# Geo3DSmart/PDANet

Hardware: AMD Instinct MI355X
Metric: scenes/sec (16384-pt ONCE, PDA-SSD forward+backward) (higher is better)
Workload: dtype f32; 1 GPU; once16k_b2_detector_fwd_bwd_adam; scenes_per_gpu=2, global_batch=2, parallelism=dp1, world_size_seen=1, cpu_affinity=GPU-local NUMA node of 0000:a7:00.0: 128 CPUs, full=False, graph_tail=False, graph_head=True

## Files before the change

include/pda_train.h:

```cpp
#ifndef PDA_TRAIN_H
#define PDA_TRAIN_H
#include "pda_pointnet2.h"

#ifdef __cplusplus
extern "C" {
#endif

int pda_grad_norm(const float *g, int64_t n, float *norm_out, float *scratch1024, pda_stream_t stream);
int pda_adam_onecycle_step(float *p, const float *g, float *m, float *v, int64_t n, float lr,
                           float beta1, float beta2, float eps, float wd, int step,
                           const float *total_norm, float max_norm, pda_stream_t stream);

int64_t pda_bn_relu_scratch_bytes(int c);
int pda_bn_relu_fwd(const float *x, const float *gamma, const float *beta, float *running_mean,
                    float *running_var, float *y, float *mean_invstd, void *scratch, int64_t rows, int c,
                    float eps, float momentum, pda_stream_t stream);
int pda_bn_relu_bwd(const float *x, const float *grad_y, const float *gamma, const float *beta,
                    const float *mean_invstd, float *grad_x, float *grad_gamma, float *grad_beta,
                    void *scratch, int64_t rows, int c, pda_stream_t stream);
int pda_bn_relu_fwd_mixed(const void *x, int x_is_bf16, const float *gamma, const float *beta, float *running_mean,
                          float *running_var, void *y, int y_is_bf16, float *mean_invstd, void *scratch,
                          int64_t rows, int c, float eps, float momentum, pda_stream_t stream);
int pda_bn_relu_bwd_mixed(const void *x, int x_is_bf16, const void *grad_y, int grad_y_is_bf16, const float *gamma,
                          const float *beta, const float *mean_invstd, void *grad_x, float *grad_gamma,
                          float *grad_beta, void *scratch, int64_t rows, int c, pda_stream_t stream);
int pda_bn_relu_max_pool_fwd(const void *x, int x_is_bf16, const float *gamma, const float *beta, float *running_mean,
                             float *running_var, float *out, uint8_t *arg, float *mean_invstd, void *scratch,
                             int64_t groups, int ns, int c, float eps, float momentum, pda_stream_t stream);
int pda_bn_relu_max_pool_bwd(const void *x, int x_is_bf16, const float *grad_out, const uint8_t *arg,
                             const float *gamma, const float *beta, const float *mean_invstd, void *grad_x,
                             float *grad_gamma, float *grad_beta, void *scratch, int64_t groups, int ns, int c,
                             pda_stream_t stream);

int64_t pda_layer_norm_scratch_bytes(int d);
int pda_layer_norm_fwd(const float *x, const float *residual, const float *gamma, const float *beta,
                       float *sum_out, float *y, float *mean_rstd, int64_t rows, int d, float eps,
                       pda_stream_t stream);
int pda_layer_norm_bwd(const float *x, const float *grad_y, const float *grad_y2, const float *gamma,
                       const float *mean_rstd, float *grad_x, float *grad_gamma, float *grad_beta,
                       void *scratch, int64_t rows, int d, pda_stream_t stream);
int pda_layer_norm_fwd_mixed(const void *x, int x_is_bf16, const float *residual, const float *gamma,
                             const float *beta, float *sum_out, float *y, uint16_t *y_bf16, float *mean_rstd,
                             int64_t rows, int d, float eps, pda_stream_t stream);
int pda_layer_norm_bwd_mixed(const float *x, const float *grad_y, const void *grad_y2, int grad_y2_is_bf16,
                             const float *gamma, const float *mean_rstd, float *grad_x, uint16_t *grad_x_bf16,
                             float *grad_gamma, float *grad_beta, void *scratch, int64_t rows, int d,
                             pda_stream_t stream);

int64_t pda_linear_wgrad_scratch_bytes(int64_t tokens, int in_features, int out_features);
int pda_linear_wgrad_form(int64_t tokens, int in_features, int out_features);
int pda_linear_wgrad(const float *x, const float *grad_out, float *grad_weight, float *grad_bias,
                     void *scratch, int64_t tokens, int in_features, int out_features, pda_stream_t stream);
int pda_linear_wgrad_bn(const float *x, const float *grad_out, float *grad_weight, float *grad_bias, void *scratch,
                        int64_t tokens, int in_features, int out_features, const float *x_mean_invstd,
                        const float *x_gamma, const float *x_beta, pda_stream_t stream);

int64_t pda_gemm_split_bn_tiles(int64_t tokens);
int pda_gemm_split_bn(const float *x, const void *wf, float *y, int64_t tokens, int k, int n_out,
                      const float *in_mean_invstd, const float *in_gamma, const float *in_beta, int stats_mode,
                      double *partial, pda_stream_t stream);
int pda_gemm_split_maxpool(const float *x, const void *wf, const float *bias, float *out, int64_t tokens, int k, int n_out,
                           int ns, int relu, pda_stream_t stream);
int pda_gemm_split_gather(const float *point_rows, const float *xyz, const float *new_xyz, const int32_t *idx,
                          const float *w1, int ldw1, const float *bias1, const void *wf, const float *bias2, float *y,
                          int b, int n, int m, int ns, int k, int n_out, int relu, pda_stream_t stream);
int pda_bn_stats_fwd(const float *x, float *running_mean, float *running_var, float *mean_invstd, void *scratch,
                     int64_t rows, int c, float eps, float momentum, pda_stream_t stream);
int pda_bn_finalize_fwd(const double *partial, int nblocks, int c, int64_t count, float eps, float momentum,
                        float *mean_invstd, float *running_mean, float *running_var, pda_stream_t stream);
int pda_bn_relu_max_pool_apply(const float *x, const float *gamma, const float *beta, const float *mean_invstd,
                               float *out, uint8_t *arg, int64_t groups, int ns, int c, pda_stream_t stream);

int64_t pda_colsum_scratch_bytes(int cols);
int pda_colsum_bf16(const uint16_t *g, float *out, void *scratch, int64_t rows, int cols, pda_stream_t stream);

int pda_assemble_tokens(const float *rppe, const float *dscale, const float *feats, const int32_t *idx,
                        const float *glob, float *out, int b, int n, int m, int nsample, int c,
                        pda_stream_t stream);
int pda_assemble_tokens_grad(const float *grad_out, const float *dscale, const float *feats, const int32_t *idx,
                             float *grad_rppe, float *grad_dscale, float *grad_feats, float *grad_glob,
                             int b, int n, int m, int nsample, int c, pda_stream_t stream);

int pda_add_max_pool(const float *a, const float *b, float *out, uint8_t *arg, int64_t groups, int seq, int d,
                     pda_stream_t stream);
int pda_max_pool_scatter(const float *grad_out, const uint8_t *arg, float *grad_x, int64_t groups, int seq,
                         int d, pda_stream_t stream);
int pda_add_max_pool_bf16(const float *a, const uint16_t *b, float *out, uint8_t *arg, int64_t groups, int seq,
                          int d, pda_stream_t stream);
int pda_max_pool_scatter_bf16(const float *grad_out, const uint8_t *arg, float *grad_x, uint16_t *grad_x_bf16,
                              int64_t groups, int seq, int d, pda_stream_t stream);

int pda_bn_relu_fwd_weighted(const float *x, const float *gamma, const float *beta, float *running_mean,
                             float *running_var, float *y, float *mean_invstd, void *scratch, int64_t rows, int c,
                             float eps, float momentum, const float *row_weight, int64_t count, pda_stream_t stream);
int pda_bn_relu_bwd_weighted(const float *x, const float *grad_y, const float *gamma, const float *beta,
                             const float *mean_invstd, float *grad_x, float *grad_gamma, float *grad_beta,
                             void *scratch, int64_t rows, int c, const float *row_weight, int64_t count,
                             pda_stream_t stream);

int pda_ragged_plan(const int32_t *idx, int32_t *cnt, int32_t *off, int32_t *rowmap, float *row_weight, int64_t groups,
                    int nsample, pda_stream_t stream);
int pda_assemble_tokens_ragged(const float *rppe, const float *dscale, const float *feats, const int32_t *idx,
                               const float *glob, const int32_t *rowmap, const int32_t *off, float *out,
                               int64_t max_tokens, int b, int n, int m, int nsample, int c, int rppe_compact,
                               pda_stream_t stream);
int pda_assemble_tokens_ragged_grad(const float *grad_out, const float *dscale, const float *feats,
                                    const int32_t *idx, const int32_t *cnt, const int32_t *off, const int32_t *rowmap,
                                    float *grad_rppe, float *grad_dscale, float *grad_feats, float *grad_glob,
                                    int64_t max_tokens, int b, int n, int m, int nsample, int c, int rppe_compact,
                                    pda_stream_t stream);
int pda_add_max_pool_ragged(const float *a, const float *b, const int32_t *cnt, const int32_t *off, float *out,
                            uint8_t *arg, int64_t groups, int d, pda_stream_t stream);
int pda_max_pool_scatter_ragged(const float *grad_out, const uint8_t *arg, const int32_t *rowmap,
                                const int32_t *off, float *grad_x, int64_t max_tokens, int64_t groups, int nsample,
                                int d, pda_stream_t stream);
int pda_group_attention_ragged_fwd(const float *qkv, const int32_t *cnt, const int32_t *off, float *out, float *lse,
                                   int64_t tokens, int64_t num_groups, int seq, int heads, int head_dim,
                                   pda_stream_t stream);
int pda_group_attention_ragged_bwd(const float *qkv, const float *grad_out, const float *lse, const int32_t *cnt,
                                   const int32_t *off, float *grad_qkv, int64_t tokens, int64_t num_groups, int seq,
                                   int heads, int head_dim, pda_stream_t stream);

int pda_densitynet_param_count(void);
int64_t pda_densitynet_scratch_bytes(void);
int pda_densitynet_fwd(const float *x, const float *params, float *y, float *stats, void *scratch,
                       float *running_mean1, float *running_var1, float *running_mean2, float *running_var2,
                       float *running_mean3, float *running_var3, int64_t n, float eps, float momentum,
                       pda_stream_t stream);
int pda_densitynet_bwd(const float *x, const float *grad_y, const float *params, const float *stats,
                       float *grad_params, void *scratch, int64_t n, float eps, pda_stream_t stream);
int pda_densitynet_fwd_unique(const float *x, const float *params, float *y, float *stats, void *scratch,
                              float *running_mean1, float *running_var1, float *running_mean2, float *running_var2,
                              float *running_mean3, float *running_var3, int64_t n, const int32_t *rowmap,
                              const float *row_weight, const int32_t *n_unique, int nsample, float eps, float momentum,
                              pda_stream_t stream);
int pda_densitynet_bwd_unique(const float *x, const float *grad_y, const float *params, const float *stats,
                              float *grad_params, void *scratch, int64_t n, const int32_t *rowmap,
                              const float *row_weight, const int32_t *n_unique, int nsample, float eps,
                              pda_stream_t stream);
#define PDA_DENSITYNET_MAX_SCALES 4
typedef struct pda_densitynet_scale {
    const float *x, *grad_y, *params;
    float *y, *stats;
    void *scratch;
    float *running[6];
    float *grad_params;
    int64_t n;
    const int32_t *rowmap;
    const float *row_weight;
    const int32_t *n_unique;
    int nsample;
    float eps, momentum;
} pda_densitynet_scale_t;
int pda_densitynet_fwd_multi(const pda_densitynet_scale_t *scales, int nscales, pda_stream_t stream);
int pda_densitynet_bwd_multi(const pda_densitynet_scale_t *scales, int nscales, pda_stream_t stream);

int pda_densitynet_eval_param_count(void);
int pda_densitynet_eval(const float *x, const float *folded, float *y, int64_t n, pda_stream_t stream);

int pda_pda_geometry(const float *xyz, const float *new_xyz, const int32_t *idx, float *rppe, float *dscale,
                     int b, int n, int m, int nsample, float radius, pda_stream_t stream);

int pda_points_in_boxes(const float *boxes, const float *pts, int32_t *box_idx_of_points, int b, int t,
                        int m, pda_stream_t stream);
int pda_assign_point_targets(const float *gt_boxes, const int32_t *in_box, const int32_t *in_ext, int64_t *labels,
                             int64_t *box_idx, float *gt_of_points, int b, int n, int t, int mode, int single_class,
                             pda_stream_t stream);
int pda_head_assign_targets(const float *points, int point_stride, int point_offset, const float *gt_boxes, const float *extra_width,
                            int64_t *labels, int64_t *box_idx, float *gt_of_points, float *box_labels, const float *mean_size,
                            int bins, int b, int n, int t, int mode, int single_class, pda_stream_t stream);
int pda_sa_gaussian_mask(const float *coords, int stride, int offset, const float *gt_of_points, const int64_t *labels,
                         float *out, int64_t points, pda_stream_t stream);

int pda_boxes_overlap_bev(const float *boxes_a, const float *boxes_b, float *ans_overlap, int num_a,
                          int num_b, pda_stream_t stream);
int pda_boxes_iou_bev(const float *boxes_a, const float *boxes_b, float *ans_iou, int num_a, int num_b,
                      pda_stream_t stream);
int64_t pda_nms_mask_words(int n);
int pda_nms_bev(const float *boxes, const int32_t *num_valid, int64_t *keep, int32_t *num_keep,
                uint64_t *mask_scratch, int b, int n, float thresh, int normal, pda_stream_t stream);

int pda_head_cls_loss(const float *preds, int row_stride, int col0, int num_class, const int64_t *labels, const float *soft,
                      int64_t n, float scale, float *out2, float *grad, pda_stream_t stream);
int pda_head_centerness(const float *centers, const float *gt, const int64_t *labels, float *out, int64_t n, pda_stream_t stream);
int pda_head_box_loss(const float *preds, const float *labels, const int64_t *cls_labels, const float *code_weights, float beta,
                      int bins, float dir_weight, float box_weight, int64_t n, float *out4, float *grad, pda_stream_t stream);
int pda_head_vote_loss(int mode, const float *origin, const float *offsets, const int64_t *key, const float *gt, int b, int boxes,
                       int num_class, float weight, int64_t n, float *out1, float *grad, pda_stream_t stream);
int pda_head_corner_loss(const float *box_preds, const float *centers, const float *cls_preds, int num_class, const float *gt,
                         const int64_t *cls_labels, const float *mean_size, int bins, float weight, int64_t n, float *out1,
                         float *grad_box, float *grad_centers, pda_stream_t stream);

int64_t pda_sa_small_train_workspace_bytes(void);
int pda_sa_small_train_supported(int c, int nsample, int c1, int c2, int c3, int64_t tokens);
int pda_sa_small_train_fwd(const float *xyz, const float *new_xyz, const float *feat_pm, const int32_t *idx,
                           const float *w1, const float *w2, const float *w3, const float *const *gamma,
                           const float *const *beta, float *const *running_mean, float *const *running_var,
                           const float *eps, const float *momentum, void *workspace, float *out, float *zmax,
                           uint8_t *arg, int b, int n, int m, int c, int nsample, int c1, int c2, int c3,
                           pda_stream_t stream);
int pda_sa_small_train_bwd(const float *xyz, const float *new_xyz, const float *feat_pm, const int32_t *idx,
                           const float *grad_out, const float *zmax, const uint8_t *arg, void *workspace, float *dz2,
                           float *dz1, float *dw1, float *dw2, float *dw3, float *const *dgamma, float *const *dbeta,
                           int b, int n, int m, int c, int nsample, int c1, int c2, int c3, pda_stream_t stream);

int64_t pda_sa_xyz_grad_scratch_bytes(int c1);
int pda_sa_point_gather(const float *point_rows, const float *xyz, const float *new_xyz, const int32_t *idx, const float *w,
                        int ldw, const float *bias, int relu, float *z, int b, int n, int m, int nsample, int c1,
                        pda_stream_t stream);
int pda_sa_xyz_grad(const float *grad_z1, const float *xyz, const float *new_xyz, const int32_t *idx, const float *w, int ldw,
                    float *dw, int lddw, float *grad_new_xyz, void *scratch, int b, int n, int m, int nsample, int c1,
                    pda_stream_t stream);

int64_t pda_input_stage_workspace_bytes(int batch, int64_t n_cap);
int pda_input_stage(const float *points, const int64_t *offsets, int64_t n_total, int batch, int c, int64_t n_cap,
                    const float *range6, int num_points, const int32_t *pick, const int32_t *perm1, const int32_t *perm2,
                    uint64_t seed, int shuffle, float *out_points, int32_t *info, void *workspace, pda_stream_t stream);
int pda_input_boxes(const float *boxes, const int64_t *box_offsets, int64_t m_total, int batch, int box_dim, int max_gt,
                    const float *range6, int min_num_corners, float *gt_boxes, int32_t *info, pda_stream_t stream);

int64_t pda_augment_workspace_bytes(int batch, int64_t n_cap, int k);
int pda_augment(const float *points, const int64_t *offsets, int64_t n_total, int batch, int c, int64_t n_cap,
                const float *boxes, const int64_t *box_offsets, int64_t m_total, const float *db_points,
                const int64_t *db_offsets, int64_t db_n_points, const float *db_boxes, const double *db_centre,
                const int32_t *db_class, int n_obj, const int32_t *cand, const int32_t *cand_group, const double *cand_dz,
                int k, const int32_t *flip, const double *angle, const float *scale, const float *remove_extra_width,
                int64_t paste_cap, float *out_points, int64_t out_cap, int64_t *out_offsets, float *out_boxes,
                int64_t out_box_cap, int64_t *out_box_offsets, int32_t *info, void *workspace, pda_stream_t stream);

int pda_augment_paste(const float *points, const int64_t *offsets, int64_t n_total, int batch, int c, int64_t n_cap,
                      const float *boxes, const int64_t *box_offsets, int64_t m_total, const float *db_points,
                      const int64_t *db_offsets, int64_t db_n_points, const float *db_boxes, const double *db_centre,
                      const int32_t *db_class, int n_obj, const int32_t *cand, const int32_t *cand_group,
                      const double *cand_dz, int k, const float *remove_extra_width, int64_t paste_cap, float *out_points,
                      int64_t out_cap, int64_t *out_offsets, float *out_boxes, int64_t out_box_cap,
                      int64_t *out_box_offsets, int32_t *info, void *workspace, pda_stream_t stream);

int64_t pda_augment_steps_workspace_bytes(int batch, int64_t n_cap, int box_slots, int n_ops);
int pda_augment_steps(const float *points, const int64_t *offsets, int64_t n_total, int batch, int c, int64_t n_cap,
                      const float *boxes, const int64_t *box_offsets, int64_t m_total, const int32_t *ops, int n_ops,
                      const double *scene_draws, const double *box_draws, int draw_cap, int box_slots,
                      const int32_t *info_in, float *out_points, int64_t out_cap, int64_t *out_offsets, float *out_boxes,
                      int64_t out_box_cap, int64_t *out_box_offsets, int32_t *info, void *workspace, pda_stream_t stream);

typedef struct pda_once_frames {
    const double *gt_boxes;
    const int32_t *gt_name;
    const int64_t *gt_offsets;
    const float *pred_boxes, *pred_score;
    const int32_t *pred_name;
    const int64_t *pred_start;
    const int32_t *pred_count;
    const int64_t *iou_start;
    int64_t n_gt_total, pred_cap, iou_cap;
    int n_frames, max_gt, max_pred;
} pda_once_frames_t;

int64_t pda_once_eval_workspace_bytes(int n_frames, int64_t n_gt_total, int n_tasks);
int pda_once_eval_iou(const pda_once_frames_t *frames, int with_heading, double *iou, int32_t *status,
                      pda_stream_t stream);
int pda_once_eval_accumulate(const pda_once_frames_t *frames, const double *iou, const uint8_t *accept, int n_classes,
                             int n_names, const double *iou_thr, int difficulty_mode, int64_t *num_valid_gt,
                             int32_t *status, void *workspace, pda_stream_t stream);
int pda_once_eval_match(const pda_once_frames_t *frames, const double *iou, const uint8_t *accept, int n_classes,
                        int n_names, const double *iou_thr, int difficulty_mode, int num_pr_points,
                        const float *sorted_scores, const int64_t *num_valid_gt, double *thresholds,
                        int64_t *n_thresholds, int64_t *counts, int32_t *status, void *workspace, pda_stream_t stream);


typedef struct pda_kitti_frames {
    const float *gt_bbox, *gt_loc;
    const double *gt_dims, *gt_ry, *gt_alpha, *gt_trunc, *gt_occ;
    const int32_t *gt_name;
    const int64_t *gt_offsets;
    const float *dt_bbox, *dt_box, *dt_alpha, *dt_score;
    const int32_t *dt_name;
    const int64_t *dt_start;
    const int32_t *dt_count;
    const int64_t *ov_start;
    const int32_t *frame_mode;
    int64_t n_gt_total, det_cap, ov_cap;
    int n_frames, max_gt, max_det;
} pda_kitti_frames_t;

int64_t pda_kitti_eval_workspace_bytes(int n_frames, int64_t n_gt_total, int64_t det_cap, int n_classes);
int pda_kitti_eval_overlaps(const pda_kitti_frames_t *frames, double *overlaps, int32_t *status, pda_stream_t stream);
int pda_kitti_eval_first_pass(const pda_kitti_frames_t *frames, const double *overlaps, int n_classes, int n_names,
                              const int8_t *gt_class, const uint8_t *dt_class, const uint8_t *dontcare,
                              const double *min_overlaps, int8_t *gt_flags, int8_t *dt_flags, int64_t *num_valid_gt,
                              int32_t *status, void *workspace, pda_stream_t stream);
int pda_kitti_eval_match(const pda_kitti_frames_t *frames, const double *overlaps, int n_classes, int n_names,
                         const int8_t *gt_class, const uint8_t *dt_class, const uint8_t *dontcare,
                         const double *min_overlaps, int compute_aos, const int8_t *gt_flags, const int8_t *dt_flags,
                         const float *sorted_scores, const int64_t *num_valid_gt, double *thresholds,
                         int64_t *n_thresholds, int64_t *counts, double *similarity, int32_t *status, void *workspace,
                         pda_stream_t stream);
int pda_kitti_eval_predictions(const float *boxes, int64_t n, int stride, int rows_per_frame, const int32_t *frame_idx,
                               const float *calib, const int32_t *image_shape, int n_frames, float *cam, float *bbox,
                               float *alpha, int32_t *status, pda_stream_t stream);

int pda_recall_record(const float *pred_boxes, const int32_t *num_pred, const float *gt_boxes, int gt_cols,
                      const float *thresh, int n_thresh, int64_t *counters, float *max_iou, int b, int k, int t,
                      pda_stream_t stream);

int64_t pda_kitti_fov_filter_workspace_bytes(int batch, int64_t n_cap);
int pda_kitti_fov_filter(const float *points, const int64_t *offsets, int64_t n_total, int batch, int c, int64_t n_cap,
                         const float *calib, const int32_t *image_shape, float *out_points, int64_t out_cap,
                         int64_t *out_offsets, int32_t *info, void *workspace, pda_stream_t stream);
int64_t pda_gt_extract_workspace_bytes(int batch, int64_t n_cap, int64_t m_total);
int pda_gt_extract_count(const float *points, const int64_t *offsets, int64_t n_total, int batch, int c, int64_t n_cap,
                         const float *boxes, const int64_t *box_offsets, int64_t m_total, int32_t *counts, int32_t *info,
                         void *workspace, pda_stream_t stream);
int pda_gt_extract_write(const float *points, const int64_t *offsets, int64_t n_total, int batch, int c, int64_t n_cap,
                         const float *boxes, const int64_t *box_offsets, int64_t m_total, const double *centre,
                         const int64_t *obj_offsets, float *obj_points, int64_t out_cap, int32_t *info, void *workspace,
                         pda_stream_t stream);

#ifdef __cplusplus
}
#endif
#endif
```

pdanet_amd/_lib.py:

```python
import ctypes
import os

_HERE = os.path.dirname(os.path.abspath(__file__))
LIB_PATH = os.environ.get("PDA_LIB_PATH") or os.path.join(_HERE, "libpda_pointnet2.so")
ABI_VERSION = 20


class DensityNetScale(ctypes.Structure):
    _fields_ = [("x", ctypes.c_void_p), ("grad_y", ctypes.c_void_p), ("params", ctypes.c_void_p), ("y", ctypes.c_void_p),
                ("stats", ctypes.c_void_p), ("scratch", ctypes.c_void_p), ("running", ctypes.c_void_p * 6),
                ("grad_params", ctypes.c_void_p), ("n", ctypes.c_int64), ("rowmap", ctypes.c_void_p),
                ("row_weight", ctypes.c_void_p), ("n_unique", ctypes.c_void_p), ("nsample", ctypes.c_int),
                ("eps", ctypes.c_float), ("momentum", ctypes.c_float)]


class OnceFrames(ctypes.Structure):
    _fields_ = [("gt_boxes", ctypes.c_void_p), ("gt_name", ctypes.c_void_p), ("gt_offsets", ctypes.c_void_p),
                ("pred_boxes", ctypes.c_void_p), ("pred_score", ctypes.c_void_p), ("pred_name", ctypes.c_void_p),
                ("pred_start", ctypes.c_void_p), ("pred_count", ctypes.c_void_p), ("iou_start", ctypes.c_void_p),
                ("n_gt_total", ctypes.c_int64), ("pred_cap", ctypes.c_int64), ("iou_cap", ctypes.c_int64),
                ("n_frames", ctypes.c_int), ("max_gt", ctypes.c_int), ("max_pred", ctypes.c_int)]


class KittiFrames(ctypes.Structure):
    _fields_ = [(n, ctypes.c_void_p) for n in ("gt_bbox", "gt_loc", "gt_dims", "gt_ry", "gt_alpha", "gt_trunc", "gt_occ",
                                               "gt_name", "gt_offsets", "dt_bbox", "dt_box", "dt_alpha", "dt_score",
                                               "dt_name", "dt_start", "dt_count", "ov_start", "frame_mode")] + \
               [("n_gt_total", ctypes.c_int64), ("det_cap", ctypes.c_int64), ("ov_cap", ctypes.c_int64),
                ("n_frames", ctypes.c_int), ("max_gt", ctypes.c_int), ("max_det", ctypes.c_int)]


PARAM_EPOCH = [0]
WEIGHT_EPOCH = [0]

_vp = ctypes.c_void_p
_i = ctypes.c_int
_f = ctypes.c_float

SIGNATURES = {
    "pda_furthest_point_sampling": [_vp, _vp, _vp, _i, _i, _i, _vp],
    "pda_furthest_point_sampling_with_dist": [_vp, _vp, _vp, _i, _i, _i, _vp],
    "pda_gather_points": [_vp, _vp, _vp, _i, _i, _i, _i, _vp],
    "pda_gather_points_grad": [_vp, _vp, _vp, _i, _i, _i, _i, _vp],
    "pda_ball_query": [_vp, _vp, _vp, _i, _i, _i, _f, _i, _vp],
    "pda_ball_query_dilated": [_vp, _vp, _vp, _i, _i, _i, _f, _f, _i, _vp],
    "pda_ellipsoid_query": [_vp, _vp, _vp, _i, _i, _i, _f, _f, _f, _i, _vp],
    "pda_ball_query_cells_scratch_bytes": [_i, _i],
    "pda_ball_query_cells": [_vp, _vp, ctypes.POINTER(_vp), _i, _i, _i, _i, ctypes.POINTER(_f), ctypes.POINTER(ctypes.c_int32),
                             _vp, ctypes.c_int64, _vp],
    "pda_ball_query_multi": [_vp, _vp, ctypes.POINTER(_vp), _i, _i, _i, _i,
                             ctypes.POINTER(_f), ctypes.POINTER(ctypes.c_int32), _vp],
    "pda_group_points": [_vp, _vp, _vp, _i, _i, _i, _i, _i, _vp],
    "pda_group_points_grad": [_vp, _vp, _vp, _i, _i, _i, _i, _i, _vp],
    "pda_group_rows": [_vp, _vp, _vp, _i, _i, _i, ctypes.c_int64, _vp],
    "pda_group_rows_grad": [_vp, _vp, _vp, _i, _i, _i, ctypes.c_int64, _vp],
    "pda_three_nn": [_vp, _vp, _vp, _vp, _i, _i, _i, _vp],
    "pda_three_interpolate": [_vp, _vp, _vp, _vp, _i, _i, _i, _i, _vp],
    "pda_three_interpolate_grad": [_vp, _vp, _vp, _vp, _i, _i, _i, _i, _vp],
    "pda_chamfer_forward": [_vp, _vp, _vp, _vp, _vp, _vp, _i, _i, _i, _vp],
    "pda_chamfer_backward": [_vp, _vp, _vp, _vp, _vp, _vp, _vp, _vp, _i, _i, _i, _vp],
    "pda_group_attention_fwd": [_vp, _vp, _vp, ctypes.c_int64, _i, _i, _i, _vp],
    "pda_group_attention_bwd": [_vp, _vp, _vp, _vp, ctypes.c_int64, _i, _i, _i, _vp],
    "pda_group_attention_fwd_bf16": [_vp, _vp, _vp, ctypes.c_int64, _i, _i, _i, _vp],
    "pda_group_attention_bwd_bf16": [_vp, _vp, _vp, _vp, ctypes.c_int64, _i, _i, _i, _vp],
    "pda_sa_mlp_maxpool": [_vp, _vp, _vp, _vp, _vp, _i, _i, _i, _i, _i, ctypes.POINTER(ctypes.c_int32),
                           ctypes.POINTER(_vp), ctypes.POINTER(_vp), ctypes.POINTER(_vp), _vp],
    "pda_linear_cols_packed_size": [_i, _i],
    "pda_linear_cols_pack": [_vp, _vp, _i, _i, _i, _i, _vp],
    "pda_linear_cols": [_vp, _vp, _vp, ctypes.c_int64, _i, _i, _vp],
    "pda_sa_gather_linear": [_vp, _vp, _vp, _vp, _vp, _vp, _i, _i, _i, _i, _i, _i, _vp],
    "pda_linear_split_packed_bytes": [_i, _i],
    "pda_linear_split_pack": [_vp, _vp, _i, _i, _i, _vp],
    "pda_linear_split_pack_both": [_vp, _vp, _vp, _i, _i, _vp],
    "pda_linear_split": [_vp, _vp, _vp, _vp, ctypes.c_int64, _i, _i, _i, _vp],
    "pda_gemm_split": [_vp, _vp, _vp, _vp, ctypes.c_int64, _i, _i, _i, _i, _vp],
    "pda_sa_mlp_packed_size": [_i, _i, _i],
    "pda_sa_mlp_pack_weights": [_vp, _vp, _i, _i, _i, _vp],
    "pda_grad_norm": [_vp, ctypes.c_int64, _vp, _vp, _vp],
    "pda_bn_relu_scratch_bytes": [_i],
    "pda_bn_relu_fwd": [_vp, _vp, _vp, _vp, _vp, _vp, _vp, _vp, ctypes.c_int64, _i, _f, _f, _vp],
    "pda_bn_relu_bwd": [_vp, _vp, _vp, _vp, _vp, _vp, _vp, _vp, _vp, ctypes.c_int64, _i, _vp],    "pda_bn_relu_fwd_mixed": [_vp, _i, _vp, _vp, _vp, _vp, _vp, _i, _vp, _vp, ctypes.c_int64, _i, _f, _f, _vp],
    "pda_bn_relu_bwd_mixed": [_vp, _i, _vp, _i, _vp, _vp, _vp, _vp, _vp, _vp, _vp, ctypes.c_int64, _i, _vp],
    "pda_bn_relu_max_pool_fwd": [_vp, _i, _vp, _vp, _vp, _vp, _vp, _vp, _vp, _vp, ctypes.c_int64, _i, _i, _f, _f, _vp],
    "pda_bn_relu_max_pool_bwd": [_vp, _i, _vp, _vp, _vp, _vp, _vp, _vp, _vp, _vp, _vp, ctypes.c_int64, _i, _i, _vp],

    "pda_layer_norm_scratch_bytes": [_i],
    "pda_layer_norm_fwd": [_vp, _vp, _vp, _vp, _vp, _vp, _vp, ctypes.c_int64, _i, _f, _vp],
    "pda_layer_norm_bwd": [_vp, _vp, _vp, _vp, _vp, _vp, _vp, _vp, _vp, ctypes.c_int64, _i, _vp],
    "pda_layer_norm_fwd_mixed": [_vp, _i, _vp, _vp, _vp, _vp, _vp, _vp, _vp, ctypes.c_int64, _i, _f, _vp],
    "pda_layer_norm_bwd_mixed": [_vp, _vp, _vp, _i, _vp, _vp, _vp, _vp, _vp, _vp, _vp, ctypes.c_int64, _i, _vp],
    "pda_linear_wgrad_scratch_bytes": [ctypes.c_int64, _i, _i],
    "pda_linear_wgrad_form": [ctypes.c_int64, _i, _i],
    "pda_linear_wgrad": [_vp, _vp, _vp, _vp, _vp, ctypes.c_int64, _i, _i, _vp],
    "pda_linear_wgrad_bn": [_vp, _vp, _vp, _vp, _vp, ctypes.c_int64, _i, _i, _vp, _vp, _vp, _vp],
    "pda_gemm_split_bn_tiles": [ctypes.c_int64],
    "pda_gemm_split_bn": [_vp, _vp, _vp, ctypes.c_int64, _i, _i, _vp, _vp, _vp, _i, _vp, _vp],
    "pda_gemm_split_maxpool": [_vp, _vp, _vp, _vp, ctypes.c_int64, _i, _i, _i, _i, _vp],
    "pda_gemm_split_gather": [_vp, _vp, _vp, _vp, _vp, _i, _vp, _vp, _vp, _vp, _i, _i, _i, _i, _i, _i, _i, _vp],
    "pda_bn_stats_fwd": [_vp, _vp, _vp, _vp, _vp, ctypes.c_int64, _i, _f, _f, _vp],
    "pda_bn_finalize_fwd": [_vp, _i, _i, ctypes.c_int64, _f, _f, _vp, _vp, _vp, _vp],
    "pda_bn_relu_max_pool_apply": [_vp, _vp, _vp, _vp, _vp, _vp, ctypes.c_int64, _i, _i, _vp],
    "pda_colsum_scratch_bytes": [_i],
    "pda_colsum_bf16": [_vp, _vp, _vp, ctypes.c_int64, _i, _vp],
    "pda_assemble_tokens": [_vp, _vp, _vp, _vp, _vp, _vp, _i, _i, _i, _i, _i, _vp],
    "pda_assemble_tokens_grad": [_vp, _vp, _vp, _vp, _vp, _vp, _vp, _vp, _i, _i, _i, _i, _i, _vp],
    "pda_add_max_pool": [_vp, _vp, _vp, _vp, ctypes.c_int64, _i, _i, _vp],
    "pda_max_pool_scatter": [_vp, _vp, _vp, ctypes.c_int64, _i, _i, _vp],
    "pda_add_max_pool_bf16": [_vp, _vp, _vp, _vp, ctypes.c_int64, _i, _i, _vp],
    "pda_max_pool_scatter_bf16": [_vp, _vp, _vp, _vp, ctypes.c_int64, _i, _i, _vp],
    "pda_ragged_plan": [_vp, _vp, _vp, _vp, _vp, ctypes.c_int64, _i, _vp],
    "pda_assemble_tokens_ragged": [_vp, _vp, _vp, _vp, _vp, _vp, _vp, _vp, ctypes.c_int64, _i, _i, _i, _i, _i, _i, _vp],
    "pda_assemble_tokens_ragged_grad": [_vp, _vp, _vp, _vp, _vp, _vp, _vp, _vp, _vp, _vp, _vp, ctypes.c_int64, _i, _i, _i, _i, _i, _i, _vp],
    "pda_bn_relu_fwd_weighted": [_vp, _vp, _vp, _vp, _vp, _vp, _vp, _vp, ctypes.c_int64, _i, _f, _f, _vp, ctypes.c_int64, _vp],
    "pda_bn_relu_bwd_weighted": [_vp, _vp, _vp, _vp, _vp, _vp, _vp, _vp, _vp, ctypes.c_int64, _i, _vp, ctypes.c_int64, _vp],
    "pda_add_max_pool_ragged": [_vp, _vp, _vp, _vp, _vp, _vp, ctypes.c_int64, _i, _vp],
    "pda_max_pool_scatter_ragged": [_vp, _vp, _vp, _vp, _vp, ctypes.c_int64, ctypes.c_int64, _i, _i, _vp],
    "pda_group_attention_ragged_fwd": [_vp, _vp, _vp, _vp, _vp, ctypes.c_int64, ctypes.c_int64, _i, _i, _i, _vp],
    "pda_group_attention_ragged_bwd": [_vp, _vp, _vp, _vp, _vp, _vp, ctypes.c_int64, ctypes.c_int64, _i, _i, _i, _vp],
    "pda_densitynet_param_count": [],
    "pda_densitynet_eval_param_count": [],
    "pda_densitynet_scratch_bytes": [],
    "pda_densitynet_fwd": [_vp, _vp, _vp, _vp, _vp, _vp, _vp, _vp, _vp, _vp, _vp, ctypes.c_int64, _f, _f, _vp],
    "pda_densitynet_bwd": [_vp, _vp, _vp, _vp, _vp, _vp, ctypes.c_int64, _f, _vp],
    "pda_densitynet_eval": [_vp, _vp, _vp, ctypes.c_int64, _vp],
    "pda_densitynet_fwd_multi": [_vp, _i, _vp],
    "pda_densitynet_bwd_multi": [_vp, _i, _vp],
    "pda_densitynet_fwd_unique": [_vp, _vp, _vp, _vp, _vp, _vp, _vp, _vp, _vp, _vp, _vp, ctypes.c_int64, _vp, _vp, _vp, _i, _f, _f, _vp],
    "pda_densitynet_bwd_unique": [_vp, _vp, _vp, _vp, _vp, _vp, ctypes.c_int64, _vp, _vp, _vp, _i, _f, _vp],
    "pda_pda_geometry": [_vp, _vp, _vp, _vp, _vp, _i, _i, _i, _i, _f, _vp],
    "pda_points_in_boxes": [_vp, _vp, _vp, _i, _i, _i, _vp],
    "pda_assign_point_targets": [_vp, _vp, _vp, _vp, _vp, _vp, _i, _i, _i, _i, _i, _vp],
    "pda_sa_gaussian_mask": [_vp, _i, _i, _vp, _vp, _vp, ctypes.c_int64, _vp],
    "pda_head_assign_targets": [_vp, _i, _i, _vp, ctypes.POINTER(ctypes.c_float), _vp, _vp, _vp, _vp, _vp, _i, _i, _i, _i, _i, _i, _vp],
    "pda_head_cls_loss": [_vp, _i, _i, _i, _vp, _vp, ctypes.c_int64, _f, _vp, _vp, _vp],
    "pda_head_centerness": [_vp, _vp, _vp, _vp, ctypes.c_int64, _vp],
    "pda_head_box_loss": [_vp, _vp, _vp, _vp, _f, _i, _f, _f, ctypes.c_int64, _vp, _vp, _vp],
    "pda_head_vote_loss": [_i, _vp, _vp, _vp, _vp, _i, _i, _i, _f, ctypes.c_int64, _vp, _vp, _vp],
    "pda_head_corner_loss": [_vp, _vp, _vp, _i, _vp, _vp, _vp, _i, _f, ctypes.c_int64, _vp, _vp, _vp, _vp],
    "pda_boxes_overlap_bev": [_vp, _vp, _vp, _i, _i, _vp],
    "pda_boxes_iou_bev": [_vp, _vp, _vp, _i, _i, _vp],
    "pda_nms_mask_words": [_i],
    "pda_nms_bev": [_vp, _vp, _vp, _vp, _vp, _i, _i, _f, _i, _vp],
    "pda_sa_small_train_workspace_bytes": [],
    "pda_sa_small_train_supported": [_i, _i, _i, _i, _i, ctypes.c_int64],
    "pda_sa_small_train_fwd": [_vp] * 7 + [ctypes.POINTER(_vp)] * 4 + [ctypes.POINTER(_f)] * 2 + [_vp] * 4 + [_i] * 8 + [_vp],
    "pda_sa_small_train_bwd": [_vp] * 13 + [ctypes.POINTER(_vp)] * 2 + [_i] * 8 + [_vp],
    "pda_sa_xyz_grad_scratch_bytes": [_i],
    "pda_sa_point_gather": [_vp, _vp, _vp, _vp, _vp, _i, _vp, _i, _vp, _i, _i, _i, _i, _i, _vp],
    "pda_sa_xyz_grad": [_vp, _vp, _vp, _vp, _vp, _i, _vp, _i, _vp, _vp, _i, _i, _i, _i, _i, _vp],
    "pda_adam_onecycle_step": [_vp, _vp, _vp, _vp, ctypes.c_int64, _f, _f, _f, _f, _f, _i, _vp, _f, _vp],
    "pda_input_stage_workspace_bytes": [_i, ctypes.c_int64],
    "pda_input_stage": [_vp, _vp, ctypes.c_int64, _i, _i, ctypes.c_int64, ctypes.POINTER(_f), _i, _vp, _vp, _vp,
                        ctypes.c_uint64, _i, _vp, _vp, _vp, _vp],
    "pda_input_boxes": [_vp, _vp, ctypes.c_int64, _i, _i, _i, ctypes.POINTER(_f), _i, _vp, _vp, _vp],
    "pda_augment_workspace_bytes": [_i, ctypes.c_int64, _i],
    "pda_augment": [_vp, _vp, ctypes.c_int64, _i, _i, ctypes.c_int64, _vp, _vp, ctypes.c_int64, _vp, _vp, ctypes.c_int64, _vp,
                    _vp, _vp, _i, _vp, _vp, _vp, _i, _vp, _vp, _vp, ctypes.POINTER(_f), ctypes.c_int64, _vp, ctypes.c_int64,
                    _vp, _vp, ctypes.c_int64, _vp, _vp, _vp, _vp],
    "pda_augment_paste": [_vp, _vp, ctypes.c_int64, _i, _i, ctypes.c_int64, _vp, _vp, ctypes.c_int64, _vp, _vp, ctypes.c_int64, _vp,
                          _vp, _vp, _i, _vp, _vp, _vp, _i, ctypes.POINTER(_f), ctypes.c_int64, _vp, ctypes.c_int64, _vp, _vp,
                          ctypes.c_int64, _vp, _vp, _vp, _vp],
    "pda_augment_steps_workspace_bytes": [_i, ctypes.c_int64, _i, _i],
    "pda_augment_steps": [_vp, _vp, ctypes.c_int64, _i, _i, ctypes.c_int64, _vp, _vp, ctypes.c_int64,
                          ctypes.POINTER(ctypes.c_int32), _i, _vp, _vp, _i, _i, _vp, _vp, ctypes.c_int64, _vp, _vp,
                          ctypes.c_int64, _vp, _vp, _vp, _vp],
    "pda_once_eval_workspace_bytes": [_i, ctypes.c_int64, _i],
    "pda_once_eval_iou": [ctypes.POINTER(OnceFrames), _i, _vp, _vp, _vp],
    "pda_once_eval_accumulate": [ctypes.POINTER(OnceFrames), _vp, _vp, _i, _i, ctypes.POINTER(ctypes.c_double), _i, _vp, _vp,
                                 _vp, _vp],
    "pda_once_eval_match": [ctypes.POINTER(OnceFrames), _vp, _vp, _i, _i, ctypes.POINTER(ctypes.c_double), _i, _i, _vp, _vp,
                            _vp, _vp, _vp, _vp, _vp, _vp],
    "pda_kitti_eval_workspace_bytes": [_i, ctypes.c_int64, ctypes.c_int64, _i],
    "pda_kitti_eval_overlaps": [ctypes.POINTER(KittiFrames), _vp, _vp, _vp],
    "pda_kitti_eval_first_pass": [ctypes.POINTER(KittiFrames), _vp, _i, _i, _vp, _vp, _vp, ctypes.POINTER(ctypes.c_double),
                                  _vp, _vp, _vp, _vp, _vp, _vp],
    "pda_kitti_eval_match": [ctypes.POINTER(KittiFrames), _vp, _i, _i, _vp, _vp, _vp, ctypes.POINTER(ctypes.c_double), _i,
                             _vp, _vp, _vp, _vp, _vp, _vp, _vp, _vp, _vp, _vp, _vp],
    "pda_kitti_eval_predictions": [_vp, ctypes.c_int64, _i, _i, _vp, _vp, _vp, _i, _vp, _vp, _vp, _vp, _vp],
    "pda_recall_record": [_vp, _vp, _vp, _i, ctypes.POINTER(_f), _i, _vp, _vp, _i, _i, _i, _vp],
    "pda_kitti_fov_filter_workspace_bytes": [_i, ctypes.c_int64],
    "pda_kitti_fov_filter": [_vp, _vp, ctypes.c_int64, _i, _i, ctypes.c_int64, _vp, _vp, _vp, ctypes.c_int64, _vp, _vp, _vp, _vp],
    "pda_gt_extract_workspace_bytes": [_i, ctypes.c_int64, ctypes.c_int64],
    "pda_gt_extract_count": [_vp, _vp, ctypes.c_int64, _i, _i, ctypes.c_int64, _vp, _vp, ctypes.c_int64, _vp, _vp, _vp, _vp],
    "pda_gt_extract_write": [_vp, _vp, ctypes.c_int64, _i, _i, ctypes.c_int64, _vp, _vp, ctypes.c_int64, _vp, _vp, _vp,
                             ctypes.c_int64, _vp, _vp, _vp],
    "pda_stack_ball_query": [_vp, _vp, _vp, _vp, _vp, _i, _i, _f, _i, _vp],
    "pda_stack_group_points": [_vp, _vp, _vp, _vp, _vp, _i, _i, _i, _i, _vp],
    "pda_stack_group_points_grad": [_vp, _vp, _vp, _vp, _vp, _i, _i, _i, _i, _i, _vp],
    "pda_stack_furthest_point_sampling": [_vp, _vp, _vp, _vp, _vp, _i, _vp],
    "pda_stack_three_nn": [_vp, _vp, _vp, _vp, _vp, _vp, _i, _i, _vp],
    "pda_stack_three_interpolate": [_vp, _vp, _vp, _vp, _i, _i, _vp],
    "pda_stack_three_interpolate_grad": [_vp, _vp, _vp, _vp, _i, _i, _vp],
}
INFO_SYMBOLS = ["pda_abi_version", "pda_last_error", "pda_fp_contract_mode", "pda_opt_n_threads",
                "pda_fps_coop_timeouts", "pda_debug_fps_spin_limit", "pda_debug_fps_exchange_nonzero"]

_LIB = None


class PdaError(RuntimeError):
    pass


def load():
    global _LIB
    if _LIB is not None:
        return _LIB
    import torch
    if not os.path.exists(LIB_PATH):
        raise PdaError(
            "%s not found: build it with `python -m pdanet_amd.build` (hipcc, gfx950). "
            "pdanet_amd has no fallback path." % LIB_PATH)
    lib = ctypes.CDLL(LIB_PATH)
    for name, argtypes in SIGNATURES.items():
        fn = getattr(lib, name)
        fn.argtypes = argtypes
        fn.restype = _i
    lib.pda_nms_mask_words.restype = ctypes.c_int64
    lib.pda_ball_query_cells_scratch_bytes.restype = ctypes.c_int64
    lib.pda_bn_relu_scratch_bytes.restype = ctypes.c_int64
    lib.pda_layer_norm_scratch_bytes.restype = ctypes.c_int64
    lib.pda_linear_wgrad_scratch_bytes.restype = ctypes.c_int64
    lib.pda_linear_split_packed_bytes.restype = ctypes.c_int64
    lib.pda_colsum_scratch_bytes.restype = ctypes.c_int64
    lib.pda_gemm_split_bn_tiles.restype = ctypes.c_int64
    lib.pda_densitynet_scratch_bytes.restype = ctypes.c_int64
    lib.pda_sa_small_train_workspace_bytes.restype = ctypes.c_int64
    lib.pda_sa_xyz_grad_scratch_bytes.restype = ctypes.c_int64
    lib.pda_input_stage_workspace_bytes.restype = ctypes.c_int64
    lib.pda_augment_workspace_bytes.restype = ctypes.c_int64
    lib.pda_augment_steps_workspace_bytes.restype = ctypes.c_int64
    lib.pda_once_eval_workspace_bytes.restype = ctypes.c_int64
    lib.pda_kitti_eval_workspace_bytes.restype = ctypes.c_int64
    lib.pda_kitti_fov_filter_workspace_bytes.restype = ctypes.c_int64
    lib.pda_gt_extract_workspace_bytes.restype = ctypes.c_int64
    lib.pda_abi_version.restype = _i
    lib.pda_last_error.restype = ctypes.c_char_p
    lib.pda_fp_contract_mode.restype = _i
    lib.pda_opt_n_threads.argtypes = [_i]
    lib.pda_opt_n_threads.restype = _i
    lib.pda_fps_coop_timeouts.argtypes = [ctypes.POINTER(ctypes.c_ulonglong), _i]
    lib.pda_fps_coop_timeouts.restype = _i
    lib.pda_debug_fps_spin_limit.argtypes = [_i]
    lib.pda_debug_fps_spin_limit.restype = _i
    lib.pda_debug_fps_exchange_nonzero.argtypes = []
    lib.pda_debug_fps_exchange_nonzero.restype = ctypes.c_longlong
    if lib.pda_abi_version() != ABI_VERSION:
        raise PdaError("libpda_pointnet2.so ABI %d != binding ABI %d: rebuild"
                       % (lib.pda_abi_version(), ABI_VERSION))
    _LIB = lib
    return lib


def check(status, what):
    if status != 0:
        msg = load().pda_last_error().decode("utf-8", "replace")
        raise PdaError("%s failed with status %d: %s" % (what, status, msg))
```

pdanet_amd/csrc/bn_relu.hip:

```cpp
#include "pda_common.h"

namespace pda {

constexpr int BN_BLOCKS = 512;

struct BnShape {
    int64_t rows;
    int c, cg, rpb;
    int ns;
    const float* roww;
    int64_t count;
};

__device__ __forceinline__ float4 pooled_grad(const float* __restrict__ gout, const uint8_t* __restrict__ arg, int64_t r,
                                              int col, const BnShape& s) {
    const int64_t g = r / s.ns;
    const int t = (int)(r - g * s.ns);
    const float4 v = reinterpret_cast<const float4*>(gout)[g * s.cg + col];
    const uchar4 k = reinterpret_cast<const uchar4*>(arg)[g * s.cg + col];
    return make_float4(k.x == t ? v.x : 0.f, k.y == t ? v.y : 0.f, k.z == t ? v.z : 0.f, k.w == t ? v.w : 0.f);
}

__device__ __forceinline__ void block_reduce_cols(double (&a)[4], double (&b)[4], double* lds, int cg, int rpb, double* out_a,
                                                  double* out_b) {
    const int tid = threadIdx.x;
    double* la = lds;
    double* lb = lds + 256 * 4;
#pragma unroll
    for (int k = 0; k < 4; ++k) { la[tid * 4 + k] = a[k]; lb[tid * 4 + k] = b[k]; }
    __syncthreads();
    if (tid < cg) {
        double sa[4] = {0, 0, 0, 0}, sb[4] = {0, 0, 0, 0};
        for (int r = 0; r < rpb; ++r)
#pragma unroll
            for (int k = 0; k < 4; ++k) { sa[k] += la[(r * cg + tid) * 4 + k]; sb[k] += lb[(r * cg + tid) * 4 + k]; }
#pragma unroll
        for (int k = 0; k < 4; ++k) { out_a[tid * 4 + k] = sa[k]; out_b[tid * 4 + k] = sb[k]; }
    }
}

template <bool BWD, typename TX, typename TD, bool POOL = false>
__global__ __launch_bounds__(256) void bn_reduce_kernel(const TX* __restrict__ x, const TD* __restrict__ dy,
                                                        const float* __restrict__ mean_invstd, const float* __restrict__ gamma,
                                                        const float* __restrict__ beta, double* __restrict__ partial, BnShape s,
                                                        const uint8_t* __restrict__ arg = nullptr) {
    __shared__ double lds[2 * 256 * 4];
    const int tid = threadIdx.x;
    double a[4] = {0, 0, 0, 0}, b[4] = {0, 0, 0, 0};
    if (s.cg <= 256) {
        const int col = tid % s.cg, r0 = tid / s.cg;
        float4 mu = make_float4(0, 0, 0, 0), is = mu, g = mu, be = mu;
        if (BWD) {
            mu = reinterpret_cast<const float4*>(mean_invstd)[col];
            is = reinterpret_cast<const float4*>(mean_invstd + s.c)[col];
            g = reinterpret_cast<const float4*>(gamma)[col];
            be = reinterpret_cast<const float4*>(beta)[col];
        }
        const int64_t stride = (int64_t)gridDim.x * s.rpb;
        auto row = [&](int64_t r, const float4& v, const float4& d) {
            if (!BWD) {
                const double w = s.roww ? (double)s.roww[r] : 1.0;
                a[0] += w * v.x; a[1] += w * v.y; a[2] += w * v.z; a[3] += w * v.w;
                b[0] += w * ((double)v.x * v.x); b[1] += w * ((double)v.y * v.y); b[2] += w * ((double)v.z * v.z); b[3] += w * ((double)v.w * v.w);
            } else {
                const float xh[4] = {(v.x - mu.x) * is.x, (v.y - mu.y) * is.y, (v.z - mu.z) * is.z, (v.w - mu.w) * is.w};
                const float gg[4] = {g.x, g.y, g.z, g.w}, bb[4] = {be.x, be.y, be.z, be.w}, dd[4] = {d.x, d.y, d.z, d.w};
#pragma unroll
                for (int k = 0; k < 4; ++k) {
                    const float dyh = (xh[k] * gg[k] + bb[k] > 0.f) ? dd[k] : 0.f;
                    a[k] += dyh;
                    b[k] += (double)dyh * xh[k];
                }
            }
        };
        auto grad = [&](int64_t r) -> float4 {
            if constexpr (!BWD) return make_float4(0, 0, 0, 0);
            else if constexpr (POOL) return pooled_grad(reinterpret_cast<const float*>(dy), arg, r, col, s);
            else return load4(dy + r * s.c + 4 * col);
        };
        constexpr int U = BWD ? 1 : 4;
        int64_t r = (int64_t)blockIdx.x * s.rpb + r0;
        for (; r + (U - 1) * stride < s.rows; r += U * stride) {
            float4 v[U], d[U];
#pragma unroll
            for (int u = 0; u < U; ++u) { v[u] = load4(x + (r + u * stride) * s.c + 4 * col); d[u] = grad(r + u * stride); }
#pragma unroll
            for (int u = 0; u < U; ++u) row(r + u * stride, v[u], d[u]);
        }
        for (; r < s.rows; r += stride) row(r, load4(x + r * s.c + 4 * col), grad(r));
    }
    double* pa = partial + (size_t)blockIdx.x * 2 * s.c;
    block_reduce_cols(a, b, lds, s.cg, s.rpb, pa, pa + s.c);
}

__device__ __forceinline__ bool sum_partials(const double* __restrict__ partial, int nblocks, int c, double& s1, double& s2, int& ch) {
    __shared__ double red[2][16][32];
    const int cl = threadIdx.x & 31, part = threadIdx.x >> 5;
    ch = blockIdx.x * 32 + cl;
    double a = 0, b = 0;
    if (ch < c) {
        double va[16], vb[16];
        for (int k0 = part; k0 < nblocks; k0 += 16 * 16) {
#pragma unroll
            for (int u = 0; u < 16; ++u) {
                const int k = k0 + 16 * u;
                va[u] = k < nblocks ? partial[(size_t)k * 2 * c + ch] : 0.0;
                vb[u] = k < nblocks ? partial[(size_t)k * 2 * c + c + ch] : 0.0;
            }
#pragma unroll
            for (int u = 0; u < 16; ++u) { a += va[u]; b += vb[u]; }
        }
    }
    red[0][part][cl] = a; red[1][part][cl] = b;
    __syncthreads();
    if (part != 0 || ch >= c) return false;
    s1 = 0; s2 = 0;
#pragma unroll
    for (int p = 0; p < 16; ++p) { s1 += red[0][p][cl]; s2 += red[1][p][cl]; }
    return true;
}

__global__ __launch_bounds__(512) void bn_finalize_fwd_kernel(const double* __restrict__ partial, int nblocks, int c, int64_t rows,
                                                               float eps, float momentum, float* __restrict__ mean_invstd,
                                                               float* __restrict__ running_mean, float* __restrict__ running_var) {
    double s1, s2;
    int ch;
    if (!sum_partials(partial, nblocks, c, s1, s2, ch)) return;
    const double mean = s1 / (double)rows;
    double var = s2 / (double)rows - mean * mean;
    var = var < 0 ? 0 : var;
    mean_invstd[ch] = (float)mean;
    mean_invstd[c + ch] = (float)(1.0 / sqrt(var + (double)eps));
    if (running_mean) {
        const double unbiased = rows > 1 ? var * ((double)rows / (double)(rows - 1)) : var;
        running_mean[ch] = (float)((1.0 - momentum) * running_mean[ch] + momentum * mean);
        running_var[ch] = (float)((1.0 - momentum) * running_var[ch] + momentum * unbiased);
    }
}

__global__ __launch_bounds__(512) void bn_finalize_bwd_kernel(const double* __restrict__ partial, int nblocks, int c, int64_t rows,
                                                               float* __restrict__ dgamma, float* __restrict__ dbeta,
                                                               float* __restrict__ sums) {
    double s1, s2;
    int ch;
    if (!sum_partials(partial, nblocks, c, s1, s2, ch)) return;
    dbeta[ch] = (float)s1;
    dgamma[ch] = (float)s2;
    sums[ch] = (float)(s1 / (double)rows);
    sums[c + ch] = (float)(s2 / (double)rows);
}

template <bool BWD, typename TX, typename TD, typename TO, bool POOL = false>
__global__ __launch_bounds__(256) void bn_apply_kernel(const TX* __restrict__ x, const TD* __restrict__ dy,
                                                       const float* __restrict__ mean_invstd, const float* __restrict__ gamma,
                                                       const float* __restrict__ beta, const float* __restrict__ sums,
                                                       TO* __restrict__ out, BnShape s, const uint8_t* __restrict__ arg = nullptr) {
    const int tid = threadIdx.x;
    const int col = tid % s.cg, r0 = tid / s.cg;
    const float4 mu = reinterpret_cast<const float4*>(mean_invstd)[col], is = reinterpret_cast<const float4*>(mean_invstd + s.c)[col];
    const float4 g = reinterpret_cast<const float4*>(gamma)[col], be = reinterpret_cast<const float4*>(beta)[col];
    float4 m1 = make_float4(0, 0, 0, 0), m2 = m1;
    if (BWD) { m1 = reinterpret_cast<const float4*>(sums)[col]; m2 = reinterpret_cast<const float4*>(sums + s.c)[col]; }
    const float muv[4] = {mu.x, mu.y, mu.z, mu.w}, isv[4] = {is.x, is.y, is.z, is.w}, gv[4] = {g.x, g.y, g.z, g.w},
                bv[4] = {be.x, be.y, be.z, be.w}, m1v[4] = {m1.x, m1.y, m1.z, m1.w}, m2v[4] = {m2.x, m2.y, m2.z, m2.w};
    const int64_t stride = (int64_t)gridDim.x * s.rpb;
    auto row = [&](int64_t r, const float4& v, const float4& d) {
        const float xv[4] = {v.x, v.y, v.z, v.w};
        float o[4];
        if (!BWD) {
#pragma unroll
            for (int k = 0; k < 4; ++k) o[k] = fmaxf((xv[k] - muv[k]) * isv[k] * gv[k] + bv[k], 0.f);
        } else {
            const float dv[4] = {d.x, d.y, d.z, d.w};
            const float w = s.roww ? s.roww[r] : 1.f;
#pragma unroll
            for (int k = 0; k < 4; ++k) {
                const float xh = (xv[k] - muv[k]) * isv[k];
                const float dyh = (xh * gv[k] + bv[k] > 0.f) ? dv[k] : 0.f;
                o[k] = gv[k] * isv[k] * (dyh - w * (m1v[k] + xh * m2v[k]));
            }
        }
        store4(out + r * s.c + 4 * col, make_float4(o[0], o[1], o[2], o[3]));
    };
    auto grad = [&](int64_t r) -> float4 {
        if constexpr (!BWD) return make_float4(0, 0, 0, 0);
        else if constexpr (POOL) return pooled_grad(reinterpret_cast<const float*>(dy), arg, r, col, s);
        else return load4(dy + r * s.c + 4 * col);
    };
    constexpr int U = (BWD && !POOL) ? 1 : 4;
    const int64_t last = s.rows - 1;
    int64_t r = (int64_t)blockIdx.x * s.rpb + r0;
    for (; r + (U - 1) * stride < s.rows; r += U * stride) {
        float4 v[U], d[U];
#pragma unroll
        for (int u = 0; u < U; ++u) { const int64_t q = last - (r + u * stride); v[u] = load4(x + q * s.c + 4 * col); d[u] = grad(q); }
#pragma unroll
        for (int u = 0; u < U; ++u) row(last - (r + u * stride), v[u], d[u]);
    }
    for (; r < s.rows; r += stride) { const int64_t q = last - r; row(q, load4(x + q * s.c + 4 * col), grad(q)); }
}

template <typename TX>
__global__ __launch_bounds__(256) void bn_apply_pool_kernel(const TX* __restrict__ x, const float* __restrict__ mean_invstd,
                                                            const float* __restrict__ gamma, const float* __restrict__ beta,
                                                            float* __restrict__ out, uint8_t* __restrict__ arg, int64_t groups,
                                                            BnShape s) {
    const int64_t e = (int64_t)blockIdx.x * 256 + threadIdx.x;
    if (e >= groups * s.cg) return;
    const int64_t g = e / s.cg;
    const int col = (int)(e - g * s.cg);
    const float4 mu = reinterpret_cast<const float4*>(mean_invstd)[col], is = reinterpret_cast<const float4*>(mean_invstd + s.c)[col];
    const float4 gm = reinterpret_cast<const float4*>(gamma)[col], be = reinterpret_cast<const float4*>(beta)[col];
    float4 best = make_float4(-1.f, -1.f, -1.f, -1.f);
    uchar4 bi = make_uchar4(0, 0, 0, 0);
    const TX* px = x + (size_t)g * s.ns * s.c + 4 * col;
    for (int t = 0; t < s.ns; ++t) {
        const float4 v = load4(px + (size_t)t * s.c);
        const float y0 = fmaxf((v.x - mu.x) * is.x * gm.x + be.x, 0.f), y1 = fmaxf((v.y - mu.y) * is.y * gm.y + be.y, 0.f);
        const float y2 = fmaxf((v.z - mu.z) * is.z * gm.z + be.z, 0.f), y3 = fmaxf((v.w - mu.w) * is.w * gm.w + be.w, 0.f);
        if (y0 > best.x) { best.x = y0; bi.x = (uint8_t)t; }
        if (y1 > best.y) { best.y = y1; bi.y = (uint8_t)t; }
        if (y2 > best.z) { best.z = y2; bi.z = (uint8_t)t; }
        if (y3 > best.w) { best.w = y3; bi.w = (uint8_t)t; }
    }
    reinterpret_cast<float4*>(out)[e] = best;
    reinterpret_cast<uchar4*>(arg)[e] = bi;
}

static int bn_shape(int64_t rows, int c, BnShape& s, const char* what) {
    PDA_REQUIRE(rows >= 1, "%s: rows = %lld", what, (long long)rows);
    PDA_REQUIRE(c >= 4 && c <= 1024 && (c & (c - 1)) == 0, "%s: C = %d is not a power of two in [4, 1024]", what, c);
    s.rows = rows; s.c = c; s.cg = c / 4; s.rpb = 256 / s.cg; s.ns = 1;
    s.roww = nullptr; s.count = rows;
    return PDA_OK;
}

static int bn_grid(const BnShape& s) {
    const int64_t steps = divup64(s.rows, s.rpb);
    return (int)(steps < BN_BLOCKS ? steps : BN_BLOCKS);
}

}

PDA_API int64_t pda_bn_relu_scratch_bytes(int c) {
    const int64_t cc = c > 0 ? c : 0;
    return (int64_t)pda::BN_BLOCKS * 2 * cc * (int64_t)sizeof(double) + 2 * cc * (int64_t)sizeof(float);
}

namespace pda {

template <typename T> static bool bn_aligned(const T* p) { return ((uintptr_t)p & (4 * sizeof(T) - 1)) == 0; }

template <typename TX, typename TY>
static int launch_bn_relu_fwd(const TX* x, const float* gamma, const float* beta, float* running_mean, float* running_var, TY* y,
                              float* mean_invstd, void* scratch, int64_t rows, int c, float eps, float momentum, hipStream_t st,
                              const char* what, const float* roww = nullptr, int64_t count = 0) {
    BnShape s;
    if (int rc = bn_shape(rows, c, s, what)) return rc;
    if (roww) { PDA_REQUIRE(count >= rows, "%s: count = %lld < rows", what, (long long)count); s.roww = roww; s.count = count; }
    PDA_REQUIRE(x && gamma && beta && y && mean_invstd && scratch, "%s: null pointer", what);
    PDA_REQUIRE((running_mean == nullptr) == (running_var == nullptr), "%s: running_mean/var must come together", what);
    PDA_REQUIRE(bn_aligned(x) && bn_aligned(y) && (((uintptr_t)gamma | (uintptr_t)beta | (uintptr_t)mean_invstd) & 15) == 0,
                "%s: pointers must be 16-byte aligned (8 for bf16 tensors)", what);
    const int grid = bn_grid(s);
    hipLaunchKernelGGL((bn_reduce_kernel<false, TX, float>), dim3(grid), dim3(256), 0, st, x, (const float*)nullptr, (const float*)nullptr,
                       (const float*)nullptr, (const float*)nullptr, (double*)scratch, s);
    hipLaunchKernelGGL(bn_finalize_fwd_kernel, dim3(divup(c, 32)), dim3(512), 0, st, (const double*)scratch, grid, c, s.count, eps, momentum,
                       mean_invstd, running_mean, running_var);
    hipLaunchKernelGGL((bn_apply_kernel<false, TX, float, TY>), dim3(grid), dim3(256), 0, st, x, (const float*)nullptr, mean_invstd, gamma, beta,
                       (const float*)nullptr, y, s);
    return check_launch(what);
}

template <typename TX, typename TD>
static int launch_bn_relu_bwd(const TX* x, const TD* grad_y, const float* gamma, const float* beta, const float* mean_invstd, TX* grad_x,
                              float* grad_gamma, float* grad_beta, void* scratch, int64_t rows, int c, hipStream_t st, const char* what,
                              const float* roww = nullptr, int64_t count = 0) {
    BnShape s;
    if (int rc = bn_shape(rows, c, s, what)) return rc;
    if (roww) { PDA_REQUIRE(count >= rows, "%s: count = %lld < rows", what, (long long)count); s.roww = roww; s.count = count; }
    PDA_REQUIRE(x && grad_y && gamma && beta && mean_invstd && grad_x && grad_gamma && grad_beta && scratch, "%s: null pointer", what);
    PDA_REQUIRE(bn_aligned(x) && bn_aligned(grad_y) && bn_aligned(grad_x) && (((uintptr_t)gamma | (uintptr_t)beta | (uintptr_t)mean_invstd) & 15) == 0,
                "%s: pointers must be 16-byte aligned (8 for bf16 tensors)", what);
    const int grid = bn_grid(s);
    float* sums = reinterpret_cast<float*>(reinterpret_cast<double*>(scratch) + (size_t)BN_BLOCKS * 2 * c);
    hipLaunchKernelGGL((bn_reduce_kernel<true, TX, TD>), dim3(grid), dim3(256), 0, st, x, grad_y, mean_invstd, gamma, beta, (double*)scratch, s);
    hipLaunchKernelGGL(bn_finalize_bwd_kernel, dim3(divup(c, 32)), dim3(512), 0, st, (const double*)scratch, grid, c, s.count, grad_gamma, grad_beta,
                       sums);
    hipLaunchKernelGGL((bn_apply_kernel<true, TX, TD, TX>), dim3(grid), dim3(256), 0, st, x, grad_y, mean_invstd, gamma, beta, sums, grad_x, s);
    return check_launch(what);
}

template <typename TX>
static int launch_bn_relu_pool_fwd(const TX* x, const float* gamma, const float* beta, float* running_mean, float* running_var, float* out,
                                   uint8_t* arg, float* mean_invstd, void* scratch, int64_t groups, int ns, int c, float eps,
                                   float momentum, hipStream_t st, const char* what) {
    PDA_REQUIRE(groups >= 1 && ns >= 1 && ns <= 255, "%s: groups=%lld ns=%d (1..255)", what, (long long)groups, ns);
    BnShape s;
    if (int rc = bn_shape(groups * ns, c, s, what)) return rc;
    s.ns = ns;
    PDA_REQUIRE(x && gamma && beta && out && arg && mean_invstd && scratch, "%s: null pointer", what);
    PDA_REQUIRE((running_mean == nullptr) == (running_var == nullptr), "%s: running_mean/var must come together", what);
    PDA_REQUIRE(bn_aligned(x) && (((uintptr_t)out | (uintptr_t)gamma | (uintptr_t)beta | (uintptr_t)mean_invstd) & 15) == 0 &&
                    ((uintptr_t)arg & 3) == 0, "%s: alignment", what);
    const int grid = bn_grid(s);
    hipLaunchKernelGGL((bn_reduce_kernel<false, TX, float>), dim3(grid), dim3(256), 0, st, x, (const float*)nullptr, (const float*)nullptr,
                       (const float*)nullptr, (const float*)nullptr, (double*)scratch, s, (const uint8_t*)nullptr);
    hipLaunchKernelGGL(bn_finalize_fwd_kernel, dim3(divup(c, 32)), dim3(512), 0, st, (const double*)scratch, grid, c, s.rows, eps, momentum,
                       mean_invstd, running_mean, running_var);
    hipLaunchKernelGGL(bn_apply_pool_kernel<TX>, dim3((unsigned)divup64(groups * s.cg, 256)), dim3(256), 0, st, x, mean_invstd, gamma, beta, out,
                       arg, groups, s);
    return check_launch(what);
}

template <typename TX>
static int launch_bn_relu_pool_bwd(const TX* x, const float* grad_out, const uint8_t* arg, const float* gamma, const float* beta,
                                   const float* mean_invstd, TX* grad_x, float* grad_gamma, float* grad_beta, void* scratch, int64_t groups,
                                   int ns, int c, hipStream_t st, const char* what) {
    PDA_REQUIRE(groups >= 1 && ns >= 1 && ns <= 255, "%s: groups=%lld ns=%d (1..255)", what, (long long)groups, ns);
    BnShape s;
    if (int rc = bn_shape(groups * ns, c, s, what)) return rc;
    s.ns = ns;
    PDA_REQUIRE(x && grad_out && arg && gamma && beta && mean_invstd && grad_x && grad_gamma && grad_beta && scratch, "%s: null pointer", what);
    PDA_REQUIRE(bn_aligned(x) && bn_aligned(grad_x) && (((uintptr_t)grad_out | (uintptr_t)gamma | (uintptr_t)beta | (uintptr_t)mean_invstd) & 15) == 0 &&
                    ((uintptr_t)arg & 3) == 0, "%s: alignment", what);
    const int grid = bn_grid(s);
    float* sums = reinterpret_cast<float*>(reinterpret_cast<double*>(scratch) + (size_t)BN_BLOCKS * 2 * c);
    hipLaunchKernelGGL((bn_reduce_kernel<true, TX, float, true>), dim3(grid), dim3(256), 0, st, x, grad_out, mean_invstd, gamma, beta,
                       (double*)scratch, s, arg);
    hipLaunchKernelGGL(bn_finalize_bwd_kernel, dim3(divup(c, 32)), dim3(512), 0, st, (const double*)scratch, grid, c, s.rows, grad_gamma, grad_beta,
                       sums);
    hipLaunchKernelGGL((bn_apply_kernel<true, TX, float, TX, true>), dim3(grid), dim3(256), 0, st, x, grad_out, mean_invstd, gamma, beta, sums,
                       grad_x, s, arg);
    return check_launch(what);
}

}

PDA_API int pda_bn_relu_fwd(const float* x, const float* gamma, const float* beta, float* running_mean, float* running_var,
                            float* y, float* mean_invstd, void* scratch, int64_t rows, int c, float eps, float momentum,
                            pda_stream_t stream) {
    return pda::launch_bn_relu_fwd<float, float>(x, gamma, beta, running_mean, running_var, y, mean_invstd, scratch, rows, c, eps, momentum,
                                                 (hipStream_t)stream, "pda_bn_relu_fwd");
}

PDA_API int pda_bn_relu_bwd(const float* x, const float* grad_y, const float* gamma, const float* beta, const float* mean_invstd,
                            float* grad_x, float* grad_gamma, float* grad_beta, void* scratch, int64_t rows, int c,
                            pda_stream_t stream) {
    return pda::launch_bn_relu_bwd<float, float>(x, grad_y, gamma, beta, mean_invstd, grad_x, grad_gamma, grad_beta, scratch, rows, c,
                                                 (hipStream_t)stream, "pda_bn_relu_bwd");
}

PDA_API int pda_bn_relu_fwd_weighted(const float* x, const float* gamma, const float* beta, float* running_mean, float* running_var,
                                     float* y, float* mean_invstd, void* scratch, int64_t rows, int c, float eps, float momentum,
                                     const float* row_weight, int64_t count, pda_stream_t stream) {
    PDA_REQUIRE(row_weight != nullptr, "pda_bn_relu_fwd_weighted: null pointer");
    return pda::launch_bn_relu_fwd<float, float>(x, gamma, beta, running_mean, running_var, y, mean_invstd, scratch, rows, c, eps, momentum,
                                                 (hipStream_t)stream, "pda_bn_relu_fwd_weighted", row_weight, count);
}

PDA_API int pda_bn_relu_bwd_weighted(const float* x, const float* grad_y, const float* gamma, const float* beta, const float* mean_invstd,
                                     float* grad_x, float* grad_gamma, float* grad_beta, void* scratch, int64_t rows, int c,
                                     const float* row_weight, int64_t count, pda_stream_t stream) {
    PDA_REQUIRE(row_weight != nullptr, "pda_bn_relu_bwd_weighted: null pointer");
    return pda::launch_bn_relu_bwd<float, float>(x, grad_y, gamma, beta, mean_invstd, grad_x, grad_gamma, grad_beta, scratch, rows, c,
                                                 (hipStream_t)stream, "pda_bn_relu_bwd_weighted", row_weight, count);
}

PDA_API int pda_bn_relu_fwd_mixed(const void* x, int x_is_bf16, const float* gamma, const float* beta, float* running_mean,
                                  float* running_var, void* y, int y_is_bf16, float* mean_invstd, void* scratch, int64_t rows, int c,
                                  float eps, float momentum, pda_stream_t stream) {
    using pda::bf16_t;
    hipStream_t st = (hipStream_t)stream;
    const char* what = "pda_bn_relu_fwd_mixed";
#define PDA_BN_FWD(TX, TY) pda::launch_bn_relu_fwd<TX, TY>((const TX*)x, gamma, beta, running_mean, running_var, (TY*)y, mean_invstd, scratch, rows, c, eps, momentum, st, what)
    if (x_is_bf16) return y_is_bf16 ? PDA_BN_FWD(bf16_t, bf16_t) : PDA_BN_FWD(bf16_t, float);
    return y_is_bf16 ? PDA_BN_FWD(float, bf16_t) : PDA_BN_FWD(float, float);
#undef PDA_BN_FWD
}

PDA_API int pda_bn_relu_bwd_mixed(const void* x, int x_is_bf16, const void* grad_y, int grad_y_is_bf16, const float* gamma,
                                  const float* beta, const float* mean_invstd, void* grad_x, float* grad_gamma, float* grad_beta,
                                  void* scratch, int64_t rows, int c, pda_stream_t stream) {
    using pda::bf16_t;
    hipStream_t st = (hipStream_t)stream;
    const char* what = "pda_bn_relu_bwd_mixed";
#define PDA_BN_BWD(TX, TD) pda::launch_bn_relu_bwd<TX, TD>((const TX*)x, (const TD*)grad_y, gamma, beta, mean_invstd, (TX*)grad_x, grad_gamma, grad_beta, scratch, rows, c, st, what)
    if (x_is_bf16) return grad_y_is_bf16 ? PDA_BN_BWD(bf16_t, bf16_t) : PDA_BN_BWD(bf16_t, float);
    return grad_y_is_bf16 ? PDA_BN_BWD(float, bf16_t) : PDA_BN_BWD(float, float);
#undef PDA_BN_BWD
}

PDA_API int pda_bn_relu_max_pool_fwd(const void* x, int x_is_bf16, const float* gamma, const float* beta, float* running_mean,
                                     float* running_var, float* out, uint8_t* arg, float* mean_invstd, void* scratch, int64_t groups,
                                     int ns, int c, float eps, float momentum, pda_stream_t stream) {
    const char* what = "pda_bn_relu_max_pool_fwd";
    if (x_is_bf16)
        return pda::launch_bn_relu_pool_fwd<pda::bf16_t>((const pda::bf16_t*)x, gamma, beta, running_mean, running_var, out, arg, mean_invstd,
                                                         scratch, groups, ns, c, eps, momentum, (hipStream_t)stream, what);
    return pda::launch_bn_relu_pool_fwd<float>((const float*)x, gamma, beta, running_mean, running_var, out, arg, mean_invstd, scratch, groups,
                                               ns, c, eps, momentum, (hipStream_t)stream, what);
}

PDA_API int pda_bn_relu_max_pool_bwd(const void* x, int x_is_bf16, const float* grad_out, const uint8_t* arg, const float* gamma,
                                     const float* beta, const float* mean_invstd, void* grad_x, float* grad_gamma, float* grad_beta,
                                     void* scratch, int64_t groups, int ns, int c, pda_stream_t stream) {
    const char* what = "pda_bn_relu_max_pool_bwd";
    if (x_is_bf16)
        return pda::launch_bn_relu_pool_bwd<pda::bf16_t>((const pda::bf16_t*)x, grad_out, arg, gamma, beta, mean_invstd, (pda::bf16_t*)grad_x,
                                                         grad_gamma, grad_beta, scratch, groups, ns, c, (hipStream_t)stream, what);
    return pda::launch_bn_relu_pool_bwd<float>((const float*)x, grad_out, arg, gamma, beta, mean_invstd, (float*)grad_x, grad_gamma, grad_beta,
                                               scratch, groups, ns, c, (hipStream_t)stream, what);
}

PDA_API int pda_bn_stats_fwd(const float* x, float* running_mean, float* running_var, float* mean_invstd, void* scratch, int64_t rows, int c,
                             float eps, float momentum, pda_stream_t stream) {
    const char* what = "pda_bn_stats_fwd";
    pda::BnShape s;
    if (int rc = pda::bn_shape(rows, c, s, what)) return rc;
    PDA_REQUIRE(x && mean_invstd && scratch && pda::bn_aligned(x) && ((uintptr_t)mean_invstd & 15) == 0, "%s: null or misaligned pointer", what);
    PDA_REQUIRE((running_mean == nullptr) == (running_var == nullptr), "%s: running_mean/var must come together", what);
    const int grid = pda::bn_grid(s);
    hipStream_t st = (hipStream_t)stream;
    hipLaunchKernelGGL((pda::bn_reduce_kernel<false, float, float>), dim3(grid), dim3(256), 0, st, x, (const float*)nullptr, (const float*)nullptr,
                       (const float*)nullptr, (const float*)nullptr, (double*)scratch, s);
    hipLaunchKernelGGL(pda::bn_finalize_fwd_kernel, dim3(pda::divup(c, 32)), dim3(512), 0, st, (const double*)scratch, grid, c, s.count, eps, momentum,
                       mean_invstd, running_mean, running_var);
    return pda::check_launch(what);
}

PDA_API int pda_bn_finalize_fwd(const double* partial, int nblocks, int c, int64_t count, float eps, float momentum, float* mean_invstd,
                                float* running_mean, float* running_var, pda_stream_t stream) {
    PDA_REQUIRE(partial && mean_invstd && nblocks >= 1 && c >= 1 && count >= 1, "pda_bn_finalize_fwd: bad argument");
    PDA_REQUIRE((running_mean == nullptr) == (running_var == nullptr), "pda_bn_finalize_fwd: running_mean/var must come together");
    hipLaunchKernelGGL(pda::bn_finalize_fwd_kernel, dim3(pda::divup(c, 32)), dim3(512), 0, (hipStream_t)stream, partial, nblocks, c, count, eps,
                       momentum, mean_invstd, running_mean, running_var);
    return pda::check_launch("pda_bn_finalize_fwd");
}

PDA_API int pda_bn_relu_max_pool_apply(const float* x, const float* gamma, const float* beta, const float* mean_invstd, float* out, uint8_t* arg,
                                       int64_t groups, int ns, int c, pda_stream_t stream) {
    const char* what = "pda_bn_relu_max_pool_apply";
    PDA_REQUIRE(groups >= 1 && ns >= 1 && ns <= 255, "%s: groups=%lld ns=%d (1..255)", what, (long long)groups, ns);
    pda::BnShape s;
    if (int rc = pda::bn_shape(groups * ns, c, s, what)) return rc;
    s.ns = ns;
    PDA_REQUIRE(x && gamma && beta && out && arg && mean_invstd, "%s: null pointer", what);
    PDA_REQUIRE(pda::bn_aligned(x) && (((uintptr_t)out | (uintptr_t)gamma | (uintptr_t)beta | (uintptr_t)mean_invstd) & 15) == 0 &&
                    ((uintptr_t)arg & 3) == 0, "%s: alignment", what);
    hipLaunchKernelGGL(pda::bn_apply_pool_kernel<float>, dim3((unsigned)pda::divup64(groups * s.cg, 256)), dim3(256), 0, (hipStream_t)stream, x,
                       mean_invstd, gamma, beta, out, arg, groups, s);
    return pda::check_launch(what);
}
```

pdanet_amd/csrc/sa_xyz_grad.hip:

```cpp
#include "pda_common.h"

namespace pda {

constexpr int XG_BLOCKS = 512;
constexpr int XG_THREADS = 256;
constexpr int XG_MAXC = 4;

template <int CPT>
__global__ __launch_bounds__(XG_THREADS) void sa_xyz_grad_kernel(const float* __restrict__ g, const float* __restrict__ xyz,
                                                                 const float* __restrict__ new_xyz, const int32_t* __restrict__ idx,
                                                                 const float* __restrict__ w, int ldw, float* __restrict__ partial,
                                                                 float* __restrict__ grad_new, int n, int m, int ns, int c1, int64_t groups) {
    __shared__ float red[XG_THREADS / 64][3];
    const int tid = threadIdx.x;
    float accw[CPT][3], wx[CPT][3];
#pragma unroll
    for (int q = 0; q < CPT; ++q) {
        const int o = tid + q * XG_THREADS;
#pragma unroll
        for (int d = 0; d < 3; ++d) { accw[q][d] = 0.f; wx[q][d] = o < c1 ? w[(size_t)o * ldw + d] : 0.f; }
    }
    for (int64_t grp = blockIdx.x; grp < groups; grp += gridDim.x) {
        const int bs = (int)(grp / m);
        const float* ct = new_xyz + grp * 3;
        const float cx = ct[0], cy = ct[1], cz = ct[2];
        const float* pts = xyz + (size_t)bs * n * 3;
        const int32_t* ids = idx + grp * ns;
        const float* grow = g + grp * ns * (int64_t)c1;
        float gs[CPT];
#pragma unroll
        for (int q = 0; q < CPT; ++q) gs[q] = 0.f;
        for (int s0 = 0; s0 < ns; s0 += 8) {
            float gv[8][CPT], dx[8], dy[8], dz[8];
#pragma unroll
            for (int u = 0; u < 8; ++u) {
                const int s = s0 + u < ns ? s0 + u : ns - 1;
                const float* pt = pts + (size_t)ids[s] * 3;
                dx[u] = pt[0] - cx; dy[u] = pt[1] - cy; dz[u] = pt[2] - cz;
#pragma unroll
                for (int q = 0; q < CPT; ++q) {
                    const int o = tid + q * XG_THREADS;
                    gv[u][q] = (s0 + u < ns && o < c1) ? grow[(int64_t)s * c1 + o] : 0.f;
                }
            }
#pragma unroll
            for (int u = 0; u < 8; ++u)
#pragma unroll
                for (int q = 0; q < CPT; ++q) {
                    accw[q][0] = __builtin_fmaf(gv[u][q], dx[u], accw[q][0]);
                    accw[q][1] = __builtin_fmaf(gv[u][q], dy[u], accw[q][1]);
                    accw[q][2] = __builtin_fmaf(gv[u][q], dz[u], accw[q][2]);
                    gs[q] += gv[u][q];
                }
        }
        if (grad_new) {
            float v[3] = {0.f, 0.f, 0.f};
#pragma unroll
            for (int q = 0; q < CPT; ++q)
#pragma unroll
                for (int d = 0; d < 3; ++d) v[d] = __builtin_fmaf(gs[q], wx[q][d], v[d]);
#pragma unroll
            for (int d = 0; d < 3; ++d) {
#pragma unroll
                for (int o = 32; o >= 1; o >>= 1) v[d] += __shfl_xor(v[d], o);
            }
            __syncthreads();
            if (lane_id() == 0) { red[wave_id()][0] = v[0]; red[wave_id()][1] = v[1]; red[wave_id()][2] = v[2]; }
            __syncthreads();
            if (tid < 3) grad_new[grp * 3 + tid] = -((red[0][tid] + red[1][tid]) + (red[2][tid] + red[3][tid]));
        }
    }
#pragma unroll
    for (int q = 0; q < CPT; ++q) {
        const int o = tid + q * XG_THREADS;
        if (o < c1) {
            float* p = partial + ((size_t)blockIdx.x * c1 + o) * 3;
            p[0] = accw[q][0]; p[1] = accw[q][1]; p[2] = accw[q][2];
        }
    }
}

__global__ __launch_bounds__(256) void sa_xyz_grad_reduce_kernel(const float* __restrict__ partial, int nblocks, int c1, float* __restrict__ dw, int lddw) {
    __shared__ double red[16][16];
    const int el = threadIdx.x & 15, part = threadIdx.x >> 4;
    const int e = blockIdx.x * 16 + el;
    const bool ok = e < c1 * 3;
    double a = 0.0;
    if (ok)
        for (int k = part; k < nblocks; k += 16) a += (double)partial[(size_t)k * c1 * 3 + e];
    red[part][el] = a;
    __syncthreads();
    if (part == 0 && ok) {
        double t = 0.0;
#pragma unroll
        for (int q = 0; q < 16; ++q) t += red[q][el];
        dw[(size_t)(e / 3) * lddw + e % 3] = (float)t;
    }
}

__global__ __launch_bounds__(256) void sa_point_gather_kernel(const float* __restrict__ prow, const float* __restrict__ xyz,
                                                              const float* __restrict__ new_xyz, const int32_t* __restrict__ idx,
                                                              const float* __restrict__ w, int ldw, const float* __restrict__ bias,
                                                              int relu, float* __restrict__ z, int n, int m, int ns, int c1,
                                                              int64_t tokens) {
    const int cq = c1 >> 2;
    const int q = threadIdx.x % cq;
    float wx[4], wy[4], wz[4];
#pragma unroll
    for (int k = 0; k < 4; ++k) {
        const float* wr = w + (size_t)(4 * q + k) * ldw;
        wx[k] = wr[0]; wy[k] = wr[1]; wz[k] = wr[2];
    }
    float bq[4] = {0.f, 0.f, 0.f, 0.f};
    if (bias) { const float4 b4 = *reinterpret_cast<const float4*>(bias + 4 * q); bq[0] = b4.x; bq[1] = b4.y; bq[2] = b4.z; bq[3] = b4.w; }
    const int tpb = 256 / cq;
    for (int64_t tok = (int64_t)blockIdx.x * tpb + threadIdx.x / cq; tok < tokens; tok += (int64_t)gridDim.x * tpb) {
        const int64_t grp = tok / ns;
        const int bs = (int)(grp / m);
        const int id = idx[tok];
        const float* pt = xyz + ((size_t)bs * n + id) * 3;
        const float* ct = new_xyz + grp * 3;
        const float dx = pt[0] - ct[0], dy = pt[1] - ct[1], dz = pt[2] - ct[2];
        const float4 p4 = *reinterpret_cast<const float4*>(prow + ((size_t)bs * n + id) * c1 + 4 * q);
        const float pv[4] = {p4.x, p4.y, p4.z, p4.w};
        float o[4];
#pragma unroll
        for (int k = 0; k < 4; ++k) {
            o[k] = __builtin_fmaf(wz[k], dz, __builtin_fmaf(wy[k], dy, __builtin_fmaf(wx[k], dx, pv[k]))) + bq[k];
            o[k] = relu ? fmaxf(o[k], 0.f) : o[k];
        }
        *reinterpret_cast<float4*>(z + tok * c1 + 4 * q) = make_float4(o[0], o[1], o[2], o[3]);
    }
}

}

PDA_API int pda_sa_point_gather(const float* point_rows, const float* xyz, const float* new_xyz, const int32_t* idx, const float* w, int ldw,
                                const float* bias, int relu, float* z, int b, int n, int m, int ns, int c1, pda_stream_t stream) {
    using namespace pda;
    PDA_REQUIRE(b >= 0 && n >= 1 && m >= 0 && ns >= 1 && c1 >= 4 && (c1 & 3) == 0 && ldw >= 3, "pda_sa_point_gather: bad size");
    const int64_t tokens = (int64_t)b * m * ns;
    if (tokens == 0) return PDA_OK;
    PDA_REQUIRE(point_rows && xyz && new_xyz && idx && w && z && (((uintptr_t)point_rows | (uintptr_t)z | (uintptr_t)bias) & 15) == 0,
                "pda_sa_point_gather: null or misaligned pointer");
    if (256 % (c1 >> 2) != 0) {
        set_error("pda_sa_point_gather: c1 = %d (c1 / 4 must divide 256)", c1);
        return PDA_ERR_UNSUPPORTED;
    }
    const int64_t total = tokens * (c1 >> 2);
    const int blocks = (int)(divup64(total, 256) < 8192 ? divup64(total, 256) : 8192);
    hipLaunchKernelGGL(sa_point_gather_kernel, dim3(blocks), dim3(256), 0, (hipStream_t)stream, point_rows, xyz, new_xyz, idx, w, ldw, bias, relu, z,
                       n, m, ns, c1, tokens);
    return check_launch("pda_sa_point_gather");
}

PDA_API int64_t pda_sa_xyz_grad_scratch_bytes(int c1) { return c1 > 0 ? (int64_t)pda::XG_BLOCKS * c1 * 3 * sizeof(float) : 0; }

PDA_API int pda_sa_xyz_grad(const float* grad_z1, const float* xyz, const float* new_xyz, const int32_t* idx, const float* w, int ldw,
                            float* dw, int lddw, float* grad_new_xyz, void* scratch, int b, int n, int m, int ns, int c1,
                            pda_stream_t stream) {
    using namespace pda;
    PDA_REQUIRE(b >= 0 && n >= 1 && m >= 0 && ns >= 1 && c1 >= 1 && ldw >= 3 && lddw >= 3, "pda_sa_xyz_grad: bad size");
    const int64_t groups = (int64_t)b * m;
    if (groups == 0) return PDA_OK;
    PDA_REQUIRE(grad_z1 && xyz && new_xyz && idx && w && dw && scratch, "pda_sa_xyz_grad: null pointer");
    if (c1 > XG_THREADS * XG_MAXC) {
        set_error("pda_sa_xyz_grad: c1 = %d > %d", c1, XG_THREADS * XG_MAXC);
        return PDA_ERR_UNSUPPORTED;
    }
    const hipStream_t s = (hipStream_t)stream;
    const int blocks = (int)(groups < XG_BLOCKS ? groups : XG_BLOCKS);
    float* partial = (float*)scratch;
    const int cpt = divup(c1, XG_THREADS);
#define PDA_XG(CPT) hipLaunchKernelGGL((sa_xyz_grad_kernel<CPT>), dim3(blocks), dim3(XG_THREADS), 0, s, grad_z1, xyz, new_xyz, idx, w, ldw, \
                                       partial, grad_new_xyz, n, m, ns, c1, groups)
    if (cpt == 1) PDA_XG(1); else if (cpt == 2) PDA_XG(2); else PDA_XG(4);
#undef PDA_XG
    hipLaunchKernelGGL(sa_xyz_grad_reduce_kernel, dim3(divup(c1 * 3, 16)), dim3(256), 0, s, (const float*)partial, blocks, c1, dw, lddw);
    return check_launch("pda_sa_xyz_grad");
}
```

pdanet_amd/pointnet2_batch_cuda.py:

```python
import ctypes

import functools

import torch

from . import _lib


def _chk(t, name, dtype):
    if not isinstance(t, torch.Tensor):
        raise TypeError("%s must be a torch.Tensor" % name)
    if not t.is_cuda:
        raise RuntimeError("%s must be a CUDA(HIP) tensor -- there is no CPU path" % name)
    if not t.is_contiguous():
        raise RuntimeError("%s must be contiguous" % name)
    if t.dtype != dtype:
        raise RuntimeError("%s must be %s, got %s" % (name, dtype, t.dtype))
    return t.data_ptr()


def _numel_ok(t, n, name):
    if t.numel() < n:
        raise RuntimeError("%s has %d elements, the sizes passed need %d" % (name, t.numel(), n))

# ... 138 lines not shown
    return 1


def farthest_point_sampling_wrapper(b, n, m, xyz, temp, idx):
    _numel_ok(xyz, b * n * 3, "xyz"); _numel_ok(temp, b * n, "temp"); _numel_ok(idx, b * m, "idx")
    _call("pda_furthest_point_sampling", xyz, _chk(xyz, "xyz", F32), _chk(temp, "temp", F32),
          _chk(idx, "idx", I32), b, n, m)
    return 1


def furthest_point_sampling_with_dist_wrapper(b, n, m, dist, temp, idx):
    _numel_ok(dist, b * n * n, "dist"); _numel_ok(temp, b * n, "temp"); _numel_ok(idx, b * m, "idx")
    _call("pda_furthest_point_sampling_with_dist", dist, _chk(dist, "dist", F32),
          _chk(temp, "temp", F32), _chk(idx, "idx", I32), b, n, m)
    return 2


def three_nn_wrapper(b, n, m, unknown, known, dist2, idx):
    _numel_ok(unknown, b * n * 3, "unknown"); _numel_ok(known, b * m * 3, "known")
    _numel_ok(dist2, b * n * 3, "dist2"); _numel_ok(idx, b * n * 3, "idx")
    _call("pda_three_nn", unknown, _chk(unknown, "unknown", F32), _chk(known, "known", F32),
          _chk(dist2, "dist2", F32), _chk(idx, "idx", I32), b, n, m)


def three_interpolate_wrapper(b, c, m, n, points, idx, weight, out):
    _numel_ok(points, b * c * m, "points"); _numel_ok(idx, b * n * 3, "idx")
    _numel_ok(weight, b * n * 3, "weight"); _numel_ok(out, b * c * n, "out")
    _call("pda_three_interpolate", points, _chk(points, "points", F32), _chk(idx, "idx", I32),
          _chk(weight, "weight", F32), _chk(out, "out", F32), b, c, m, n)


def three_interpolate_grad_wrapper(b, c, n, m, grad_out, idx, weight, grad_points):
    _numel_ok(grad_out, b * c * n, "grad_out"); _numel_ok(idx, b * n * 3, "idx")
    _numel_ok(weight, b * n * 3, "weight"); _numel_ok(grad_points, b * c * m, "grad_points")
    _call("pda_three_interpolate_grad", grad_out, _chk(grad_out, "grad_out", F32),
          _chk(idx, "idx", I32), _chk(weight, "weight", F32),
          _chk(grad_points, "grad_points", F32), b, c, n, m)


def chamfer_forward(xyz1, xyz2, dist1, dist2, idx1, idx2):
    b, n, _ = xyz1.shape
    m = xyz2.shape[1]
    _numel_ok(dist1, b * n, "dist1"); _numel_ok(dist2, b * m, "dist2")
    _numel_ok(idx1, b * n, "idx1"); _numel_ok(idx2, b * m, "idx2")
    _call("pda_chamfer_forward", xyz1, _chk(xyz1, "xyz1", F32), _chk(xyz2, "xyz2", F32), _chk(dist1, "dist1", F32),
          _chk(dist2, "dist2", F32), _chk(idx1, "idx1", I32), _chk(idx2, "idx2", I32), b, n, m)
    return 1


def chamfer_backward(xyz1, xyz2, gradxyz1, gradxyz2, graddist1, graddist2, idx1, idx2):
    b, n, _ = xyz1.shape
    m = xyz2.shape[1]
    _call("pda_chamfer_backward", xyz1, _chk(xyz1, "xyz1", F32), _chk(xyz2, "xyz2", F32),
          _chk(gradxyz1, "gradxyz1", F32), _chk(gradxyz2, "gradxyz2", F32), _chk(graddist1, "graddist1", F32),
          _chk(graddist2, "graddist2", F32), _chk(idx1, "idx1", I32), _chk(idx2, "idx2", I32), b, n, m)
    return 1


def group_attention_fwd(qkv, out, lse, num_groups, seq, heads, head_dim):
    _numel_ok(qkv, num_groups * seq * 3 * heads * head_dim, "qkv")
    _numel_ok(out, num_groups * seq * heads * head_dim, "out"); _numel_ok(lse, num_groups * heads * seq, "lse")
    io, sfx = (torch.bfloat16, "_bf16") if qkv.dtype == torch.bfloat16 else (F32, "")
    _call("pda_group_attention_fwd" + sfx, qkv, _chk(qkv, "qkv", io), _chk(out, "out", io), _chk(lse, "lse", F32),
          num_groups, seq, heads, head_dim)
    return 1


def group_attention_bwd(qkv, grad_out, lse, grad_qkv, num_groups, seq, heads, head_dim):
    _numel_ok(qkv, num_groups * seq * 3 * heads * head_dim, "qkv"); _numel_ok(grad_qkv, qkv.numel(), "grad_qkv")
    _numel_ok(grad_out, num_groups * seq * heads * head_dim, "grad_out"); _numel_ok(lse, num_groups * heads * seq, "lse")
    io, sfx = (torch.bfloat16, "_bf16") if qkv.dtype == torch.bfloat16 else (F32, "")
    _call("pda_group_attention_bwd" + sfx, qkv, _chk(qkv, "qkv", io), _chk(grad_out, "grad_out", io),
          _chk(lse, "lse", F32), _chk(grad_qkv, "grad_qkv", io), num_groups, seq, heads, head_dim)
    return 1


@functools.lru_cache(maxsize=None)
def bn_relu_scratch_bytes(c):
    return int(_lib.load().pda_bn_relu_scratch_bytes(int(c)))


def _io(t, name):
    if t.dtype == torch.bfloat16:
        return _chk(t, name, torch.bfloat16), 1
    return _chk(t, name, F32), 0


def _buffers_written(running):
    if running is not None:
        _lib.PARAM_EPOCH[0] += 1


def bn_relu_fwd(x, gamma, beta, running_mean, running_var, y, mean_invstd, scratch, rows, c, eps, momentum):
    _numel_ok(x, rows * c, "x"); _numel_ok(y, rows * c, "y"); _numel_ok(mean_invstd, 2 * c, "mean_invstd")
    rm = None if running_mean is None else _chk(running_mean, "running_mean", F32)
    rv = None if running_var is None else _chk(running_var, "running_var", F32)
    _buffers_written(rm)
    if x.dtype == F32 and y.dtype == F32:
        _call("pda_bn_relu_fwd", x, _chk(x, "x", F32), _chk(gamma, "gamma", F32), _chk(beta, "beta", F32), rm, rv,
              _chk(y, "y", F32), _chk(mean_invstd, "mean_invstd", F32), _chk(scratch, "scratch", torch.uint8), rows, c,
              float(eps), float(momentum))
        return 1
    (xp, xb), (yp, yb) = _io(x, "x"), _io(y, "y")
    _call("pda_bn_relu_fwd_mixed", x, xp, xb, _chk(gamma, "gamma", F32), _chk(beta, "beta", F32), rm, rv, yp, yb,
          _chk(mean_invstd, "mean_invstd", F32), _chk(scratch, "scratch", torch.uint8), rows, c, float(eps), float(momentum))
    return 1


def bn_relu_bwd(x, grad_y, gamma, beta, mean_invstd, grad_x, grad_gamma, grad_beta, scratch, rows, c):
    _numel_ok(x, rows * c, "x"); _numel_ok(grad_y, rows * c, "grad_y"); _numel_ok(grad_x, rows * c, "grad_x")
    if x.dtype == F32 and grad_y.dtype == F32:
        _call("pda_bn_relu_bwd", x, _chk(x, "x", F32), _chk(grad_y, "grad_y", F32), _chk(gamma, "gamma", F32),
              _chk(beta, "beta", F32), _chk(mean_invstd, "mean_invstd", F32), _chk(grad_x, "grad_x", F32),
              _chk(grad_gamma, "grad_gamma", F32), _chk(grad_beta, "grad_beta", F32), _chk(scratch, "scratch", torch.uint8), rows, c)
        return 1
    (xp, xb), (gp, gb) = _io(x, "x"), _io(grad_y, "grad_y")
    _call("pda_bn_relu_bwd_mixed", x, xp, xb, gp, gb, _chk(gamma, "gamma", F32), _chk(beta, "beta", F32),
          _chk(mean_invstd, "mean_invstd", F32), _chk(grad_x, "grad_x", x.dtype), _chk(grad_gamma, "grad_gamma", F32),
          _chk(grad_beta, "grad_beta", F32), _chk(scratch, "scratch", torch.uint8), rows, c)
    return 1


def bn_relu_max_pool_fwd(x, gamma, beta, running_mean, running_var, out, arg, mean_invstd, scratch, groups, ns, c, eps, momentum):
    _numel_ok(x, groups * ns * c, "x"); _numel_ok(out, groups * c, "out"); _numel_ok(arg, groups * c, "arg"); _numel_ok(mean_invstd, 2 * c, "mean_invstd")
    rm = None if running_mean is None else _chk(running_mean, "running_mean", F32)
    rv = None if running_var is None else _chk(running_var, "running_var", F32)
    _buffers_written(rm)
    xp, xb = _io(x, "x")
    _call("pda_bn_relu_max_pool_fwd", x, xp, xb, _chk(gamma, "gamma", F32), _chk(beta, "beta", F32), rm, rv, _chk(out, "out", F32),
          _chk(arg, "arg", torch.uint8), _chk(mean_invstd, "mean_invstd", F32), _chk(scratch, "scratch", torch.uint8), groups, ns, c,
          float(eps), float(momentum))
    return 1


def bn_relu_max_pool_bwd(x, grad_out, arg, gamma, beta, mean_invstd, grad_x, grad_gamma, grad_beta, scratch, groups, ns, c):
    _numel_ok(x, groups * ns * c, "x"); _numel_ok(grad_out, groups * c, "grad_out"); _numel_ok(arg, groups * c, "arg")
    _numel_ok(grad_x, groups * ns * c, "grad_x")
    xp, xb = _io(x, "x")
    _call("pda_bn_relu_max_pool_bwd", x, xp, xb, _chk(grad_out, "grad_out", F32), _chk(arg, "arg", torch.uint8), _chk(gamma, "gamma", F32),
          _chk(beta, "beta", F32), _chk(mean_invstd, "mean_invstd", F32), _chk(grad_x, "grad_x", x.dtype), _chk(grad_gamma, "grad_gamma", F32),
          _chk(grad_beta, "grad_beta", F32), _chk(scratch, "scratch", torch.uint8), groups, ns, c)
    return 1


@functools.lru_cache(maxsize=None)
def layer_norm_scratch_bytes(d):
    return int(_lib.load().pda_layer_norm_scratch_bytes(int(d)))


BF16 = torch.bfloat16


def layer_norm_fwd(x, residual, gamma, beta, sum_out, y, mean_rstd, rows, d, eps, y_bf16=None):
    _numel_ok(x, rows * d, "x"); _numel_ok(mean_rstd, rows * 2, "mean_rstd")
    res = None if residual is None else _chk(residual, "residual", F32)
    so = None if sum_out is None else _chk(sum_out, "sum_out", F32)
    if x.dtype == F32 and y_bf16 is None:
        _numel_ok(y, rows * d, "y")
        _call("pda_layer_norm_fwd", x, _chk(x, "x", F32), res, _chk(gamma, "gamma", F32), _chk(beta, "beta", F32), so,
              _chk(y, "y", F32), _chk(mean_rstd, "mean_rstd", F32), rows, d, float(eps))
        return 1
    yp = yb = None
    if y is not None:
        _numel_ok(y, rows * d, "y"); yp = _chk(y, "y", F32)
    if y_bf16 is not None:
        _numel_ok(y_bf16, rows * d, "y_bf16"); yb = _chk(y_bf16, "y_bf16", BF16)
    _call("pda_layer_norm_fwd_mixed", x, _chk(x, "x", x.dtype if x.dtype == BF16 else F32), int(x.dtype == BF16), res,
          _chk(gamma, "gamma", F32), _chk(beta, "beta", F32), so, yp, yb, _chk(mean_rstd, "mean_rstd", F32), rows, d, float(eps))
    return 1


def layer_norm_bwd(x, grad_y, gamma, mean_rstd, grad_x, grad_gamma, grad_beta, scratch, rows, d, grad_y2=None, grad_x_bf16=None):
    _numel_ok(x, rows * d, "x"); _numel_ok(grad_y, rows * d, "grad_y"); _numel_ok(grad_x, rows * d, "grad_x")
    g2 = None
    if grad_y2 is not None:
        _numel_ok(grad_y2, rows * d, "grad_y2")
        g2 = _chk(grad_y2, "grad_y2", BF16 if grad_y2.dtype == BF16 else F32)
    if grad_x_bf16 is not None or (grad_y2 is not None and grad_y2.dtype == BF16):
        gxb = None
        if grad_x_bf16 is not None:
            _numel_ok(grad_x_bf16, rows * d, "grad_x_bf16"); gxb = _chk(grad_x_bf16, "grad_x_bf16", BF16)
        _call("pda_layer_norm_bwd_mixed", x, _chk(x, "x", F32), _chk(grad_y, "grad_y", F32), g2,
              int(grad_y2 is not None and grad_y2.dtype == BF16), _chk(gamma, "gamma", F32), _chk(mean_rstd, "mean_rstd", F32),
              _chk(grad_x, "grad_x", F32), gxb, _chk(grad_gamma, "grad_gamma", F32), _chk(grad_beta, "grad_beta", F32),
              _chk(scratch, "scratch", torch.uint8), rows, d)
        return 1
    _call("pda_layer_norm_bwd", x, _chk(x, "x", F32), _chk(grad_y, "grad_y", F32), g2, _chk(gamma, "gamma", F32),
          _chk(mean_rstd, "mean_rstd", F32), _chk(grad_x, "grad_x", F32), _chk(grad_gamma, "grad_gamma", F32),
          _chk(grad_beta, "grad_beta", F32), _chk(scratch, "scratch", torch.uint8), rows, d)
    return 1


_WGRAD_SCRATCH_BYTES = {}


def _wgrad_scratch_bytes(tokens, in_features, out_features):
    key = (tokens, in_features, out_features)
    nbytes = _WGRAD_SCRATCH_BYTES.get(key)
    if nbytes is None:
        if len(_WGRAD_SCRATCH_BYTES) >= 4096:
            _WGRAD_SCRATCH_BYTES.clear()
        nbytes = _WGRAD_SCRATCH_BYTES[key] = int(_lib.load().pda_linear_wgrad_scratch_bytes(tokens, in_features, out_features))
    return nbytes


@functools.lru_cache(maxsize=None)
def _split_packed_bytes(n_out, k):
    return int(_lib.load().pda_linear_split_packed_bytes(n_out, k))


@functools.lru_cache(maxsize=None)
def _cols_packed_size(n_out, k):
    return int(_lib.load().pda_linear_cols_packed_size(n_out, k))


def linear_wgrad(x, grad_out, grad_weight, grad_bias, tokens, in_features, out_features):
    _numel_ok(x, tokens * in_features, "x"); _numel_ok(grad_out, tokens * out_features, "grad_out")
    _numel_ok(grad_weight, in_features * out_features, "grad_weight")
    nbytes = _wgrad_scratch_bytes(tokens, in_features, out_features)
    scratch = torch.empty((nbytes,), dtype=torch.uint8, device=x.device)
    gb = None if grad_bias is None else _chk(grad_bias, "grad_bias", F32)
    _call("pda_linear_wgrad", x, _chk(x, "x", F32), _chk(grad_out, "grad_out", F32), _chk(grad_weight, "grad_weight", F32),
          gb, _chk(scratch, "scratch", torch.uint8), tokens, in_features, out_features)
    return 1


def linear_wgrad_bn(x, grad_out, grad_weight, tokens, in_features, out_features, x_mean_invstd, x_gamma, x_beta):
    _numel_ok(x, tokens * in_features, "x"); _numel_ok(grad_out, tokens * out_features, "grad_out")
    _numel_ok(grad_weight, in_features * out_features, "grad_weight"); _numel_ok(x_mean_invstd, 2 * in_features, "x_mean_invstd")
    _numel_ok(x_gamma, in_features, "x_gamma"); _numel_ok(x_beta, in_features, "x_beta")
    nbytes = _wgrad_scratch_bytes(tokens, in_features, out_features)
    scratch = torch.empty((nbytes,), dtype=torch.uint8, device=x.device)
    _call("pda_linear_wgrad_bn", x, _chk(x, "x", F32), _chk(grad_out, "grad_out", F32), _chk(grad_weight, "grad_weight", F32), None,
          _chk(scratch, "scratch", torch.uint8), tokens, in_features, out_features, _chk(x_mean_invstd, "x_mean_invstd", F32),
          _chk(x_gamma, "x_gamma", F32), _chk(x_beta, "x_beta", F32))
    return 1


def gemm_split_bn_tiles(tokens):
    return (int(tokens) + 255) // 256


def gemm_split_bn(x, wf, y, tokens, k, n_out, in_bn=None, stats_mode=0, partial=None):
    _numel_ok(x, tokens * k, "x"); _numel_ok(y, tokens * n_out, "y")
    _numel_ok(wf, _split_packed_bytes(int(n_out), int(k)), "wf")
    ib = (None, None, None)
    if in_bn is not None:
        _numel_ok(in_bn[0], 2 * k, "in_mean_invstd"); _numel_ok(in_bn[1], k, "in_gamma"); _numel_ok(in_bn[2], k, "in_beta")
        ib = tuple(_chk(t, "in_bn", F32) for t in in_bn)
    if stats_mode:
        _numel_ok(partial, gemm_split_bn_tiles(tokens) * 2 * n_out, "partial")
    _call("pda_gemm_split_bn", x, _chk(x, "x", F32), _chk(wf, "wf", torch.uint8), _chk(y, "y", F32), tokens, k, n_out, ib[0], ib[1], ib[2],
          int(stats_mode), None if partial is None else _chk(partial, "partial", torch.float64))
    return 1


def gemm_split_maxpool(x, wf, bias, out, tokens, k, n_out, ns, relu=True):
    _numel_ok(x, tokens * k, "x"); _numel_ok(out, (tokens // ns) * n_out, "out")
    _numel_ok(wf, _split_packed_bytes(int(n_out), int(k)), "wf")
    if bias is not None:
        _numel_ok(bias, n_out, "bias")
    _call("pda_gemm_split_maxpool", x, _chk(x, "x", F32), _chk(wf, "wf", torch.uint8), None if bias is None else _chk(bias, "bias", F32),
          _chk(out, "out", F32), tokens, k, n_out, ns, 1 if relu else 0)
    return 1


def gemm_split_gather(point_rows, xyz, new_xyz, idx, w1, bias1, wf, bias2, y, b, n, m, ns, k, n_out, relu=True):
    t = b * m * ns
    _numel_ok(point_rows, b * n * k, "point_rows"); _numel_ok(xyz, b * n * 3, "xyz"); _numel_ok(new_xyz, b * m * 3, "new_xyz")
    _numel_ok(idx, t, "idx"); _numel_ok(y, t * n_out, "y"); _numel_ok(wf, _split_packed_bytes(int(n_out), int(k)), "wf")
    if w1.dim() != 2 or w1.shape[0] != k or w1.shape[1] < 3:
        raise RuntimeError("w1 must be (k, 3 + c)")
    _call("pda_gemm_split_gather", y, _chk(point_rows, "point_rows", F32), _chk(xyz, "xyz", F32), _chk(new_xyz, "new_xyz", F32),
          _chk(idx, "idx", I32), _chk(w1, "w1", F32), int(w1.shape[1]), None if bias1 is None else _chk(bias1, "bias1", F32),
          _chk(wf, "wf", torch.uint8), None if bias2 is None else _chk(bias2, "bias2", F32), _chk(y, "y", F32), b, n, m, ns, k, n_out,
          1 if relu else 0)
    return 1


def bn_stats_fwd(x, running_mean, running_var, mean_invstd, scratch, rows, c, eps, momentum):
    _numel_ok(x, rows * c, "x"); _numel_ok(mean_invstd, 2 * c, "mean_invstd")
    rm = None if running_mean is None else _chk(running_mean, "running_mean", F32)
    rv = None if running_var is None else _chk(running_var, "running_var", F32)
    _buffers_written(rm)
    _call("pda_bn_stats_fwd", x, _chk(x, "x", F32), rm, rv, _chk(mean_invstd, "mean_invstd", F32), _chk(scratch, "scratch", torch.uint8),
          rows, c, float(eps), float(momentum))
    return 1


def bn_finalize_fwd(partial, nblocks, c, count, eps, momentum, mean_invstd, running_mean, running_var):
    _numel_ok(partial, nblocks * 2 * c, "partial"); _numel_ok(mean_invstd, 2 * c, "mean_invstd")
    rm = None if running_mean is None else _chk(running_mean, "running_mean", F32)
    rv = None if running_var is None else _chk(running_var, "running_var", F32)
    _buffers_written(rm)
    _call("pda_bn_finalize_fwd", partial, _chk(partial, "partial", torch.float64), nblocks, c, count, float(eps), float(momentum),
          _chk(mean_invstd, "mean_invstd", F32), rm, rv)
    return 1


def bn_relu_max_pool_apply(x, gamma, beta, mean_invstd, out, arg, groups, ns, c):
    _numel_ok(x, groups * ns * c, "x"); _numel_ok(out, groups * c, "out"); _numel_ok(arg, groups * c, "arg"); _numel_ok(mean_invstd, 2 * c, "mean_invstd")
    _call("pda_bn_relu_max_pool_apply", x, _chk(x, "x", F32), _chk(gamma, "gamma", F32), _chk(beta, "beta", F32),
          _chk(mean_invstd, "mean_invstd", F32), _chk(out, "out", F32), _chk(arg, "arg", torch.uint8), groups, ns, c)
    return 1


def colsum_bf16(g, out, rows, cols):
    _numel_ok(g, rows * cols, "g"); _numel_ok(out, cols, "out")
    scratch = torch.empty((int(_lib.load().pda_colsum_scratch_bytes(cols)),), dtype=torch.uint8, device=g.device)
    _call("pda_colsum_bf16", g, _chk(g, "g", torch.bfloat16), _chk(out, "out", F32), _chk(scratch, "scratch", torch.uint8), rows, cols)
    return 1


@functools.lru_cache(maxsize=None)
def densitynet_sizes():
    lib = _lib.load()
    return int(lib.pda_densitynet_param_count()), int(lib.pda_densitynet_scratch_bytes())


def densitynet_eval(x, folded, y, n):
    _numel_ok(x, n, "x"); _numel_ok(y, n, "y"); _numel_ok(folded, int(_lib.load().pda_densitynet_eval_param_count()), "folded")
    _call("pda_densitynet_eval", x, _chk(x, "x", F32), _chk(folded, "folded", F32), _chk(y, "y", F32), n)
    return 1


def densitynet_fwd(x, params, y, stats, scratch, running, n, eps, momentum):
    _numel_ok(x, n, "x"); _numel_ok(y, n, "y")
    r = [None] * 6 if running is None else [_chk(t, "running", F32) for t in running]
    _buffers_written(running)
    _call("pda_densitynet_fwd", x, _chk(x, "x", F32), _chk(params, "params", F32), _chk(y, "y", F32), _chk(stats, "stats", F32),
          _chk(scratch, "scratch", torch.uint8), *r, n, float(eps), float(momentum))
    return 1


def densitynet_bwd(x, grad_y, params, stats, grad_params, scratch, n, eps):
    _numel_ok(x, n, "x"); _numel_ok(grad_y, n, "grad_y")
    _call("pda_densitynet_bwd", x, _chk(x, "x", F32), _chk(grad_y, "grad_y", F32), _chk(params, "params", F32),
          _chk(stats, "stats", F32), _chk(grad_params, "grad_params", F32), _chk(scratch, "scratch", torch.uint8), n, float(eps))
    return 1


def _unique_rows(rowmap, roww, off, groups, n, nsample):
    assert groups * nsample == n and off.numel() >= groups + 1 and off.dtype == I32 and off.is_contiguous()
    _numel_ok(rowmap, 0, "rowmap"); _numel_ok(roww, 0, "row_weight")
    return _chk(rowmap, "rowmap", I32), _chk(roww, "row_weight", F32), off.data_ptr() + 4 * groups


def densitynet_fwd_unique(x, params, y, stats, scratch, running, n, rowmap, roww, off, groups, nsample, eps, momentum):
    _numel_ok(x, n, "x"); _numel_ok(y, n, "y")
    r = [None] * 6 if running is None else [_chk(t, "running", F32) for t in running]
    _buffers_written(running)
    rm, rw, nu = _unique_rows(rowmap, roww, off, groups, n, nsample)
    _call("pda_densitynet_fwd_unique", x, _chk(x, "x", F32), _chk(params, "params", F32), _chk(y, "y", F32), _chk(stats, "stats", F32),
          _chk(scratch, "scratch", torch.uint8), *r, n, rm, rw, nu, nsample, float(eps), float(momentum))
    return 1


def densitynet_bwd_unique(x, grad_y, params, stats, grad_params, scratch, n, rowmap, roww, off, groups, nsample, eps):
    _numel_ok(x, n, "x"); _numel_ok(grad_y, n, "grad_y")
    rm, rw, nu = _unique_rows(rowmap, roww, off, groups, n, nsample)
    _call("pda_densitynet_bwd_unique", x, _chk(x, "x", F32), _chk(grad_y, "grad_y", F32), _chk(params, "params", F32),
          _chk(stats, "stats", F32), _chk(grad_params, "grad_params", F32), _chk(scratch, "scratch", torch.uint8), n, rm, rw, nu,
          nsample, float(eps))
    return 1


def densitynet_multi(problems, backward=False):
    arr = (_lib.DensityNetScale * len(problems))()
    for S, p in zip(arr, problems):
        n = int(p["n"])
        _numel_ok(p["x"], n, "x")
        S.x = _chk(p["x"], "x", F32); S.params = _chk(p["params"], "params", F32); S.stats = _chk(p["stats"], "stats", F32)
        S.scratch = _chk(p["scratch"], "scratch", torch.uint8)
        S.n, S.nsample, S.eps, S.momentum = n, 1, float(p["eps"]), float(p.get("momentum") or 0.0)
        if backward:
            _numel_ok(p["grad_y"], n, "grad_y")
            S.grad_y = _chk(p["grad_y"], "grad_y", F32); S.grad_params = _chk(p["grad_params"], "grad_params", F32)
        else:
            _numel_ok(p["y"], n, "y")
            S.y = _chk(p["y"], "y", F32)
            if p.get("running") is not None:
                _buffers_written(p["running"])
                for k, t in enumerate(p["running"]):
                    S.running[k] = _chk(t, "running", F32)
        if p.get("rowmap") is not None:
            S.rowmap, S.row_weight, S.n_unique = _unique_rows(p["rowmap"], p["roww"], p["off"], p["groups"], n, p["nsample"])
            S.nsample = int(p["nsample"])
    _call("pda_densitynet_bwd_multi" if backward else "pda_densitynet_fwd_multi", problems[0]["x"], ctypes.addressof(arr), len(problems))
    return 1


def pda_geometry(xyz, new_xyz, idx, rppe, dscale, b, n, m, nsample, radius):
    _numel_ok(xyz, b * n * 3, "xyz"); _numel_ok(new_xyz, b * m * 3, "new_xyz"); _numel_ok(idx, b * m * nsample, "idx")
    _numel_ok(rppe, b * m * nsample * 12, "rppe"); _numel_ok(dscale, b * m * nsample, "dscale")
    _call("pda_pda_geometry", xyz, _chk(xyz, "xyz", F32), _chk(new_xyz, "new_xyz", F32), _chk(idx, "idx", I32),
          _chk(rppe, "rppe", F32), _chk(dscale, "dscale", F32), b, n, m, nsample, float(radius))
    return 1


def add_max_pool(a, b, out, arg, groups, seq, d):
    _numel_ok(a, groups * seq * d, "a"); _numel_ok(b, groups * seq * d, "b"); _numel_ok(out, groups * d, "out"); _numel_ok(arg, groups * d, "arg")
    io, sfx = (BF16, "_bf16") if b.dtype == BF16 else (F32, "")
    _call("pda_add_max_pool" + sfx, a, _chk(a, "a", F32), _chk(b, "b", io), _chk(out, "out", F32), _chk(arg, "arg", torch.uint8), groups, seq, d)
    return 1


def max_pool_scatter(grad_out, arg, grad_x, groups, seq, d, grad_x_bf16=None):
    _numel_ok(grad_out, groups * d, "grad_out"); _numel_ok(arg, groups * d, "arg"); _numel_ok(grad_x, groups * seq * d, "grad_x")
    if grad_x_bf16 is not None:
        _numel_ok(grad_x_bf16, groups * seq * d, "grad_x_bf16")
        _call("pda_max_pool_scatter_bf16", grad_out, _chk(grad_out, "grad_out", F32), _chk(arg, "arg", torch.uint8), _chk(grad_x, "grad_x", F32),
              _chk(grad_x_bf16, "grad_x_bf16", BF16), groups, seq, d)
        return 1
    _call("pda_max_pool_scatter", grad_out, _chk(grad_out, "grad_out", F32), _chk(arg, "arg", torch.uint8), _chk(grad_x, "grad_x", F32),
          groups, seq, d)
    return 1


def assemble_tokens(rppe, dscale, feats, idx, glob, out, b, n, m, nsample, c):
    t = b * m * nsample
    _numel_ok(rppe, t * c, "rppe"); _numel_ok(dscale, t, "dscale"); _numel_ok(feats, b * n * c, "feats"); _numel_ok(idx, t, "idx")
    _numel_ok(glob, b * m * c, "glob"); _numel_ok(out, t * 4 * c, "out")
    _call("pda_assemble_tokens", rppe, _chk(rppe, "rppe", F32), _chk(dscale, "dscale", F32), _chk(feats, "feats", F32),
          _chk(idx, "idx", I32), _chk(glob, "glob", F32), _chk(out, "out", F32), b, n, m, nsample, c)
    return 1


def assemble_tokens_grad(grad_out, dscale, feats, idx, grad_rppe, grad_dscale, grad_feats, grad_glob, b, n, m, nsample, c):
    t = b * m * nsample
    _numel_ok(grad_out, t * 4 * c, "grad_out"); _numel_ok(grad_rppe, t * c, "grad_rppe"); _numel_ok(grad_dscale, t, "grad_dscale")
    _numel_ok(grad_feats, b * n * c, "grad_feats"); _numel_ok(grad_glob, b * m * c, "grad_glob")
    _call("pda_assemble_tokens_grad", grad_out, _chk(grad_out, "grad_out", F32), _chk(dscale, "dscale", F32), _chk(feats, "feats", F32),
          _chk(idx, "idx", I32), _chk(grad_rppe, "grad_rppe", F32), _chk(grad_dscale, "grad_dscale", F32),
          _chk(grad_feats, "grad_feats", F32), _chk(grad_glob, "grad_glob", F32), b, n, m, nsample, c)
    return 1


def ragged_plan(idx, cnt, off, rowmap, groups, nsample, roww=None):
    _numel_ok(idx, groups * nsample, "idx"); _numel_ok(cnt, groups, "cnt"); _numel_ok(off, groups + 1, "off")
    _numel_ok(rowmap, groups * nsample, "rowmap")
    if roww is not None:
        _numel_ok(roww, groups * nsample, "roww")
    _call("pda_ragged_plan", idx, _chk(idx, "idx", I32), _chk(cnt, "cnt", I32), _chk(off, "off", I32), _chk(rowmap, "rowmap", I32),
          None if roww is None else _chk(roww, "roww", F32), groups, nsample)
    return 1


def bn_relu_fwd_weighted(x, gamma, beta, running_mean, running_var, y, mean_invstd, scratch, rows, c, eps, momentum, roww, count):
    _numel_ok(x, rows * c, "x"); _numel_ok(y, rows * c, "y"); _numel_ok(mean_invstd, 2 * c, "mean_invstd"); _numel_ok(roww, rows, "roww")
    rm = None if running_mean is None else _chk(running_mean, "running_mean", F32)
    rv = None if running_var is None else _chk(running_var, "running_var", F32)
    _buffers_written(rm)
    _call("pda_bn_relu_fwd_weighted", x, _chk(x, "x", F32), _chk(gamma, "gamma", F32), _chk(beta, "beta", F32), rm, rv, _chk(y, "y", F32),
          _chk(mean_invstd, "mean_invstd", F32), _chk(scratch, "scratch", torch.uint8), rows, c, float(eps), float(momentum),
          _chk(roww, "roww", F32), int(count))
    return 1


def bn_relu_bwd_weighted(x, grad_y, gamma, beta, mean_invstd, grad_x, grad_gamma, grad_beta, scratch, rows, c, roww, count):
    _numel_ok(x, rows * c, "x"); _numel_ok(grad_y, rows * c, "grad_y"); _numel_ok(grad_x, rows * c, "grad_x"); _numel_ok(roww, rows, "roww")
    _call("pda_bn_relu_bwd_weighted", x, _chk(x, "x", F32), _chk(grad_y, "grad_y", F32), _chk(gamma, "gamma", F32), _chk(beta, "beta", F32),
          _chk(mean_invstd, "mean_invstd", F32), _chk(grad_x, "grad_x", F32), _chk(grad_gamma, "grad_gamma", F32),
          _chk(grad_beta, "grad_beta", F32), _chk(scratch, "scratch", torch.uint8), rows, c, _chk(roww, "roww", F32), int(count))
    return 1


def assemble_tokens_ragged(rppe, dscale, feats, idx, glob, rowmap, off, out, tokens, b, n, m, nsample, c, rppe_compact=False):
    t = b * m * nsample
    _numel_ok(rppe, (tokens if rppe_compact else t) * c, "rppe"); _numel_ok(dscale, t, "dscale"); _numel_ok(feats, b * n * c, "feats"); _numel_ok(idx, t, "idx")
    _numel_ok(glob, b * m * c, "glob"); _numel_ok(out, tokens * 4 * c, "out"); _numel_ok(rowmap, tokens, "rowmap"); _numel_ok(off, b * m + 1, "off")
    _call("pda_assemble_tokens_ragged", rppe, _chk(rppe, "rppe", F32), _chk(dscale, "dscale", F32), _chk(feats, "feats", F32),
          _chk(idx, "idx", I32), _chk(glob, "glob", F32), _chk(rowmap, "rowmap", I32), _chk(off, "off", I32), _chk(out, "out", F32),
          tokens, b, n, m, nsample, c, 1 if rppe_compact else 0)
    return 1


def assemble_tokens_ragged_grad(grad_out, dscale, feats, idx, cnt, off, grad_rppe, grad_dscale, grad_feats, grad_glob, tokens, b, n, m, nsample, c,
                                rppe_compact=False, rowmap=None):
    t = b * m * nsample
    if rowmap is not None:
        _numel_ok(rowmap, tokens, "rowmap")
    _numel_ok(grad_out, tokens * 4 * c, "grad_out"); _numel_ok(grad_rppe, (tokens if rppe_compact else t) * c, "grad_rppe"); _numel_ok(grad_dscale, t, "grad_dscale")
    _numel_ok(grad_feats, b * n * c, "grad_feats"); _numel_ok(grad_glob, b * m * c, "grad_glob"); _numel_ok(cnt, b * m, "cnt"); _numel_ok(off, b * m + 1, "off")
    _call("pda_assemble_tokens_ragged_grad", grad_out, _chk(grad_out, "grad_out", F32), _chk(dscale, "dscale", F32), _chk(feats, "feats", F32),
          _chk(idx, "idx", I32), _chk(cnt, "cnt", I32), _chk(off, "off", I32), None if rowmap is None else _chk(rowmap, "rowmap", I32),
          _chk(grad_rppe, "grad_rppe", F32), _chk(grad_dscale, "grad_dscale", F32), _chk(grad_feats, "grad_feats", F32),
          _chk(grad_glob, "grad_glob", F32), tokens, b, n, m, nsample, c, 1 if rppe_compact else 0)
    return 1


def add_max_pool_ragged(a, b, cnt, off, out, arg, tokens, groups, d):
    _numel_ok(a, tokens * d, "a"); _numel_ok(b, tokens * d, "b"); _numel_ok(out, groups * d, "out"); _numel_ok(arg, groups * d, "arg")
    _numel_ok(cnt, groups, "cnt"); _numel_ok(off, groups + 1, "off")
    _call("pda_add_max_pool_ragged", a, _chk(a, "a", F32), _chk(b, "b", F32), _chk(cnt, "cnt", I32), _chk(off, "off", I32),
          _chk(out, "out", F32), _chk(arg, "arg", torch.uint8), groups, d)
    return 1


def max_pool_scatter_ragged(grad_out, arg, rowmap, off, grad_x, tokens, groups, nsample, d):
    _numel_ok(grad_out, groups * d, "grad_out"); _numel_ok(arg, groups * d, "arg"); _numel_ok(grad_x, tokens * d, "grad_x")
    _numel_ok(rowmap, tokens, "rowmap"); _numel_ok(off, groups + 1, "off")
    _call("pda_max_pool_scatter_ragged", grad_out, _chk(grad_out, "grad_out", F32), _chk(arg, "arg", torch.uint8),
          _chk(rowmap, "rowmap", I32), _chk(off, "off", I32), _chk(grad_x, "grad_x", F32), tokens, groups, nsample, d)
    return 1


def group_attention_ragged_fwd(qkv, cnt, off, out, lse, tokens, num_groups, seq, heads, head_dim):
    _numel_ok(qkv, tokens * 3 * heads * head_dim, "qkv"); _numel_ok(out, tokens * heads * head_dim, "out")
    _numel_ok(lse, num_groups * heads * seq, "lse"); _numel_ok(cnt, num_groups, "cnt"); _numel_ok(off, num_groups + 1, "off")
    _call("pda_group_attention_ragged_fwd", qkv, _chk(qkv, "qkv", F32), _chk(cnt, "cnt", I32), _chk(off, "off", I32),
          _chk(out, "out", F32), _chk(lse, "lse", F32), tokens, num_groups, seq, heads, head_dim)
    return 1


def group_attention_ragged_bwd(qkv, grad_out, lse, cnt, off, grad_qkv, tokens, num_groups, seq, heads, head_dim):
    _numel_ok(qkv, tokens * 3 * heads * head_dim, "qkv"); _numel_ok(grad_qkv, tokens * 3 * heads * head_dim, "grad_qkv")
    _numel_ok(grad_out, tokens * heads * head_dim, "grad_out"); _numel_ok(lse, num_groups * heads * seq, "lse")
    _call("pda_group_attention_ragged_bwd", qkv, _chk(qkv, "qkv", F32), _chk(grad_out, "grad_out", F32), _chk(lse, "lse", F32),
          _chk(cnt, "cnt", I32), _chk(off, "off", I32), _chk(grad_qkv, "grad_qkv", F32), tokens, num_groups, seq, heads, head_dim)
    return 1


def linear_cols_pack(w, n_out, k, transposed_source=False, gather_order=False):
    lib = _lib.load()
    wf = torch.empty((_cols_packed_size(int(n_out), int(k)),), dtype=F32, device=w.device)
    _numel_ok(w, n_out * k, "w")
    _call("pda_linear_cols_pack", w, _chk(w, "w", F32), _chk(wf, "wf", F32), n_out, k, 1 if transposed_source else 0,
          1 if gather_order else 0)
    return wf


def linear_cols(x, wf, y, tokens, k, n_out):
    _numel_ok(x, tokens * k, "x"); _numel_ok(y, tokens * n_out, "y")
    _numel_ok(wf, _cols_packed_size(int(n_out), int(k)), "wf")
    _call("pda_linear_cols", x, _chk(x, "x", F32), _chk(wf, "wf", F32), _chk(y, "y", F32), tokens, k, n_out)
    return 1


def linear_split_pack(w, n_out, k, transposed_source=False):
    lib = _lib.load()
    wf = torch.empty((_split_packed_bytes(int(n_out), int(k)),), dtype=torch.uint8, device=w.device)
    _numel_ok(w, n_out * k, "w")
    _call("pda_linear_split_pack", w, _chk(w, "w", F32), _chk(wf, "wf", torch.uint8), n_out, k, 1 if transposed_source else 0)
    return wf


def linear_split_pack_both(w, n_out, k):
    wf = torch.empty((_split_packed_bytes(int(n_out), int(k)),), dtype=torch.uint8, device=w.device)
    wft = torch.empty((_split_packed_bytes(int(k), int(n_out)),), dtype=torch.uint8, device=w.device)
    _numel_ok(w, n_out * k, "w")
    _call("pda_linear_split_pack_both", w, _chk(w, "w", F32), _chk(wf, "wf", torch.uint8), _chk(wft, "wft", torch.uint8), n_out, k)
    return wf, wft


def linear_split(x, wf, bias, y, tokens, k, n_out, relu=False):
    _numel_ok(x, tokens * k, "x"); _numel_ok(y, tokens * n_out, "y")
    _numel_ok(wf, _split_packed_bytes(int(n_out), int(k)), "wf")
    if bias is not None:
        _numel_ok(bias, n_out, "bias")
    _call("pda_linear_split", x, _chk(x, "x", F32), _chk(wf, "wf", torch.uint8), None if bias is None else _chk(bias, "bias", F32),
          _chk(y, "y", F32), tokens, k, n_out, 1 if relu else 0)
    return 1


def gemm_split(x, wf, bias, y, tokens, k, n_out, relu=False, accumulate=False):
    _numel_ok(x, tokens * k, "x"); _numel_ok(y, tokens * n_out, "y")
    _numel_ok(wf, _split_packed_bytes(int(n_out), int(k)), "wf")
    if bias is not None:
        _numel_ok(bias, n_out, "bias")
    _call("pda_gemm_split", x, _chk(x, "x", F32), _chk(wf, "wf", torch.uint8), None if bias is None else _chk(bias, "bias", F32),
          _chk(y, "y", F32), tokens, k, n_out, 1 if relu else 0, 1 if accumulate else 0)
    return 1


def sa_gather_linear(xyz, new_xyz, feats_pm, idx, wf, y, b, n, m, c, nsample, n_out):
    _numel_ok(xyz, b * n * 3, "xyz"); _numel_ok(new_xyz, b * m * 3, "new_xyz"); _numel_ok(feats_pm, b * n * c, "feats_pm")
    _numel_ok(idx, b * m * nsample, "idx"); _numel_ok(y, b * m * nsample * n_out, "y")
    _numel_ok(wf, _cols_packed_size(int(n_out), 3 + int(c)), "wf")
    _call("pda_sa_gather_linear", xyz, _chk(xyz, "xyz", F32), _chk(new_xyz, "new_xyz", F32), _chk(feats_pm, "feats_pm", F32),
          _chk(idx, "idx", I32), _chk(wf, "wf", F32), _chk(y, "y", F32), b, n, m, c, nsample, n_out)
    return 1


@functools.lru_cache(maxsize=None)
def sa_small_train_workspace_bytes():
    return int(_lib.load().pda_sa_small_train_workspace_bytes())


@functools.lru_cache(maxsize=None)
def sa_small_train_supported(c, ns, c1, c2, c3, tokens):
    return bool(_lib.load().pda_sa_small_train_supported(int(c), int(ns), int(c1), int(c2), int(c3), int(tokens)))


def _ptr_array(ptrs):
    return (ctypes.c_void_p * len(ptrs))(*ptrs)


def sa_small_train_fwd(xyz, new_xyz, feat_pm, idx, weights, gammas, betas, running_means, running_vars, eps, momentum,
                       workspace, out, zmax, arg, b, n, m, c, ns):
    c1, c2, c3 = (int(w.shape[0]) for w in weights)
    tokens = b * m * ns
    _numel_ok(xyz, b * n * 3, "xyz"); _numel_ok(new_xyz, b * m * 3, "new_xyz"); _numel_ok(idx, tokens, "idx")
    _numel_ok(out, b * m * c3, "out"); _numel_ok(zmax, b * m * c3, "zmax"); _numel_ok(arg, b * m * c3, "arg")
    _numel_ok(workspace, sa_small_train_workspace_bytes(), "workspace")
    assert weights[0].shape[1] == 3 + c and weights[1].shape[1] == c1 and weights[2].shape[1] == c2
    if feat_pm is not None:
        _numel_ok(feat_pm, b * n * c, "feat_pm")
    rm = [None if t is None else _chk(t, "running_mean", F32) for t in running_means]
    rv = [None if t is None else _chk(t, "running_var", F32) for t in running_vars]
    _buffers_written(rm[0] or rm[1] or rm[2])
    _call("pda_sa_small_train_fwd", xyz, _chk(xyz, "xyz", F32), _chk(new_xyz, "new_xyz", F32),
          None if feat_pm is None else _chk(feat_pm, "feat_pm", F32), _chk(idx, "idx", I32),
          _chk(weights[0], "w1", F32), _chk(weights[1], "w2", F32), _chk(weights[2], "w3", F32),
          _ptr_array([_chk(t, "gamma", F32) for t in gammas]), _ptr_array([_chk(t, "beta", F32) for t in betas]),
          _ptr_array(rm), _ptr_array(rv), (ctypes.c_float * 3)(*[float(e) for e in eps]),
          (ctypes.c_float * 3)(*[float(x) for x in momentum]), _chk(workspace, "workspace", torch.uint8),
          _chk(out, "out", F32), _chk(zmax, "zmax", F32), _chk(arg, "arg", torch.uint8), b, n, m, c, ns, c1, c2, c3)
    return 1


def sa_small_train_bwd(xyz, new_xyz, feat_pm, idx, grad_out, zmax, arg, workspace, dz2, dz1, dws, dgammas, dbetas, b, n, m, c, ns):
    c1, c2, c3 = (int(w.shape[0]) for w in dws)
    tokens = b * m * ns
    _numel_ok(grad_out, b * m * c3, "grad_out"); _numel_ok(dz2, tokens * c2, "dz2"); _numel_ok(dz1, tokens * c1, "dz1")
    _numel_ok(workspace, sa_small_train_workspace_bytes(), "workspace")
    _call("pda_sa_small_train_bwd", xyz, _chk(xyz, "xyz", F32), _chk(new_xyz, "new_xyz", F32),
          None if feat_pm is None else _chk(feat_pm, "feat_pm", F32), _chk(idx, "idx", I32), _chk(grad_out, "grad_out", F32),
          _chk(zmax, "zmax", F32), _chk(arg, "arg", torch.uint8), _chk(workspace, "workspace", torch.uint8),
          _chk(dz2, "dz2", F32), _chk(dz1, "dz1", F32), _chk(dws[0], "dw1", F32), _chk(dws[1], "dw2", F32), _chk(dws[2], "dw3", F32),
          _ptr_array([_chk(t, "dgamma", F32) for t in dgammas]), _ptr_array([_chk(t, "dbeta", F32) for t in dbetas]),
          b, n, m, c, ns, c1, c2, c3)
    return 1


@functools.lru_cache(maxsize=None)
def sa_xyz_grad_scratch_bytes(c1):
    return int(_lib.load().pda_sa_xyz_grad_scratch_bytes(int(c1)))


def sa_xyz_grad(grad_z1, xyz, new_xyz, idx, w, dw, grad_new_xyz, b, n, m, ns, c1):
    _numel_ok(grad_z1, b * m * ns * c1, "grad_z1"); _numel_ok(idx, b * m * ns, "idx")
    _numel_ok(xyz, b * n * 3, "xyz"); _numel_ok(new_xyz, b * m * 3, "new_xyz")
    assert w.shape[0] == c1 and dw.shape == w.shape and w.shape[1] >= 3
    scratch = torch.empty((sa_xyz_grad_scratch_bytes(c1),), dtype=torch.uint8, device=xyz.device)
    _call("pda_sa_xyz_grad", xyz, _chk(grad_z1, "grad_z1", F32), _chk(xyz, "xyz", F32), _chk(new_xyz, "new_xyz", F32),
          _chk(idx, "idx", I32), _chk(w, "w", F32), int(w.shape[1]), _chk(dw, "dw", F32), int(dw.shape[1]),
          None if grad_new_xyz is None else _chk(grad_new_xyz, "grad_new_xyz", F32), _chk(scratch, "scratch", torch.uint8),
          b, n, m, ns, c1)
    return 1


def sa_point_gather(point_rows, xyz, new_xyz, idx, w, z, b, n, m, ns, c1, bias=None, relu=False):
    _numel_ok(point_rows, b * n * c1, "point_rows"); _numel_ok(z, b * m * ns * c1, "z"); _numel_ok(idx, b * m * ns, "idx")
    _numel_ok(xyz, b * n * 3, "xyz"); _numel_ok(new_xyz, b * m * 3, "new_xyz")
    assert w.shape[0] == c1 and w.shape[1] >= 3
    _call("pda_sa_point_gather", xyz, _chk(point_rows, "point_rows", F32), _chk(xyz, "xyz", F32), _chk(new_xyz, "new_xyz", F32),
          _chk(idx, "idx", I32), _chk(w, "w", F32), int(w.shape[1]), None if bias is None else _chk(bias, "bias", F32),
          1 if relu else 0, _chk(z, "z", F32), b, n, m, ns, c1)
    return 1
```

pdanet_amd/pointnet2_utils.py:

```python
import weakref
from typing import List, Tuple

import os

import torch
import torch.nn as nn
from torch.autograd import Function

from . import _lib
from . import pointnet2_batch_cuda as pointnet2

_fwd = torch.amp.custom_fwd(device_type="cuda", cast_inputs=torch.float32)
_bwd = torch.amp.custom_bwd(device_type="cuda")


class FarthestPointSampling(Function):

    @staticmethod
    @_fwd
    def forward(ctx, xyz: torch.Tensor, npoint: int) -> torch.Tensor:
        assert xyz.is_contiguous()
        B, N, _ = xyz.size()
        output = torch.empty((B, npoint), dtype=torch.int32, device=xyz.device)
        temp = torch.full((B, N), 1e10, dtype=torch.float32, device=xyz.device)
# ... 835 lines not shown
        d_a = torch.mm(ds_g, _b16p(out_w)) if bf16 else _gemm_nn(d_s, out_w)
        gwo, gbo = _wgrad(a_s, ds_g, out_w, True, bf16)
        del ds_g
        dqkv = torch.empty_like(qkv)
        pointnet2.group_attention_bwd(qkv, d_a.view(G, S, D), lse, dqkv, G, S, heads, hd)
        del d_a
        dqkv2 = dqkv.view(T, 3 * D)
        gwi, gbi = _wgrad(src1_s, dqkv2, in_w, True, bf16)
        d_src1 = _mm_nn(dqkv2, in_w, True, acc=d_s) if bf16 else _gemm_nn(dqkv2, in_w, acc=d_s)
        del dqkv, dqkv2
        d_x = torch.empty_like(x)
        gn1w, gn1b = torch.empty_like(n1w), torch.empty_like(n1w)
        pointnet2.layer_norm_bwd(x, d_src1, n1w, st1, d_x, gn1w, gn1b, scratch, T, D)
        return d_x, gn1w, gn1b, gwi, gbi, gwo, gbo, gn2w, gn2b, gw1, gb1, gw2, gb2, None, None, None, None


def transformer_block(tr, x, pool=False):
    at = tr.self_attn
    return TransformerBlock.apply(x, tr.norm1.weight, tr.norm1.bias, at.in_proj_weight, at.in_proj_bias, at.out_proj.weight,
                                  at.out_proj.bias, tr.norm2.weight, tr.norm2.bias, tr.linear1.weight, tr.linear1.bias,
                                  tr.linear2.weight, tr.linear2.bias, at.num_heads, tr.norm1.eps, tr.norm2.eps, pool)


SA_MFMA_TRAIN = True
SA_MFMA_EVENTS = None


def _sa_timed(flops, fn, pipe="f32"):
    ev = SA_MFMA_EVENTS
    if ev is None or torch.cuda.is_current_stream_capturing():
        return fn()
    e0, e1 = torch.cuda.Event(enable_timing=True), torch.cuda.Event(enable_timing=True)
    e0.record()
    fn()
    e1.record()
    ev.append((e0, e1, flops, pipe))




def _lin_cols(x2, weight, y, T, k, n_out, transposed):
    if SPLIT_GEMM:
        wf = _split_planes(weight, transposed)
        if _rows_in_registers(T, k, n_out):
            _sa_timed(2.0 * T * k * n_out, lambda: pointnet2.linear_split(x2, wf, None, y, T, k, n_out), "bf16x6")
        else:
            _sa_timed(2.0 * T * k * n_out, lambda: pointnet2.gemm_split(x2, wf, None, y, T, k, n_out), "bf16x6")
    else:
        wf = pointnet2.linear_cols_pack(weight, n_out, k, transposed_source=transposed)
        _sa_timed(2.0 * T * k * n_out, lambda: pointnet2.linear_cols(x2, wf, y, T, k, n_out))


class LinearColsMFMA(Function):

    @staticmethod
    def supported(x, weight):
        n_out, k = weight.shape
        return (SA_MFMA_TRAIN and x.is_cuda and x.dtype == torch.float32 and weight.dtype == torch.float32 and k in (256, 512)
                and n_out % 128 == 0 and n_out <= 1024 and x.shape[-1] == k and not torch.is_autocast_enabled() and not DENSE_BF16)

    @staticmethod
    def forward(ctx, x, weight):
        n_out, k = weight.shape
        x2 = x.contiguous().view(-1, k)
        T = x2.shape[0]
        y = torch.empty((T, n_out), dtype=torch.float32, device=x.device)
        _lin_cols(x2, weight.contiguous(), y, T, k, n_out, False)
        ctx.save_for_backward(x2, weight)
        ctx.x_shape = x.shape
        return y.view(*x.shape[:-1], n_out)

    @staticmethod
    def backward(ctx, grad_out):
        x2, weight = ctx.saved_tensors
        n_out, k = weight.shape
        g2 = grad_out.contiguous().view(-1, n_out)
        T = g2.shape[0]
        gx = gw = None
        if ctx.needs_input_grad[0]:
            if n_out in (256, 512) and k % 128 == 0:
                gx = torch.empty((T, k), dtype=torch.float32, device=g2.device)
                _lin_cols(g2, weight.contiguous(), gx, T, n_out, k, True)
            else:
                gx = _gemm_nn(g2, weight)
            gx = gx.view(ctx.x_shape)
        if ctx.needs_input_grad[1]:
            gw = _wgrad(x2, g2, weight, False)[0]
        return gx, gw


class SaGatherLinear(Function):

    @staticmethod
    def supported(xyz, feats_pm, weight):
        return (SA_MFMA_TRAIN and xyz.is_cuda and feats_pm is not None and feats_pm.dtype == torch.float32 and feats_pm.shape[-1] == 256
                and weight.shape[1] == 259 and weight.shape[0] % 128 == 0 and weight.shape[0] <= 1024
                and not torch.is_autocast_enabled() and not DENSE_BF16)

    @staticmethod
    def forward(ctx, xyz, new_xyz, feats_pm, idx, weight):
        B, N, _ = xyz.shape
        M, ns = idx.shape[1], idx.shape[2]
        C, n_out = feats_pm.shape[-1], weight.shape[0]
        xyz, new_xyz, feats_pm = xyz.contiguous(), new_xyz.contiguous(), feats_pm.contiguous()
        y = torch.empty((B, M, ns, n_out), dtype=torch.float32, device=xyz.device)
        wf = pointnet2.linear_cols_pack(weight.contiguous(), n_out, 3 + C, gather_order=True)
        _sa_timed(2.0 * B * M * ns * (3 + C) * n_out,
                  lambda: pointnet2.sa_gather_linear(xyz, new_xyz, feats_pm, idx, wf, y, B, N, M, C, ns, n_out))
        ctx.save_for_backward(xyz, new_xyz, feats_pm, idx, weight)
        return y

    @staticmethod
    def backward(ctx, grad_out):
        xyz, new_xyz, feats_pm, idx, weight = ctx.saved_tensors
        B, M, ns = idx.shape
        n_out, C, N = weight.shape[0], feats_pm.shape[-1], xyz.shape[1]
        g2 = grad_out.contiguous().view(-1, n_out)
        T = g2.shape[0]
        g_new = g_feats = gw = None
        with torch.no_grad():
            if ctx.needs_input_grad[4] or ctx.needs_input_grad[1]:
                gw = torch.empty_like(weight)
                g_new = torch.empty_like(new_xyz) if ctx.needs_input_grad[1] else None
                pointnet2.sa_xyz_grad(g2, xyz, new_xyz, idx, weight.contiguous(), gw, g_new, B, N, M, ns, n_out)
            if ctx.needs_input_grad[4]:
                gf_in = group_rows(feats_pm, idx).view(T, C)
                gw[:, 3:] = _wgrad(gf_in, g2, torch.empty((n_out, C), dtype=weight.dtype, device=weight.device), False)[0]
                del gf_in
            else:
                gw = None
            if ctx.needs_input_grad[2]:
                gxf = _gemm_nn(g2, weight[:, 3:].contiguous())
                g_feats = torch.zeros_like(feats_pm)
                pointnet2.group_rows_grad(B, feats_pm.shape[1], C, M * ns, gxf, idx, g_feats)
        return None, g_new, g_feats, None, gw


SA_POINT_LINEAR = os.environ.get("PDA_SA_POINT_LINEAR", "1") != "0"


class SaPointLinear(Function):

    @staticmethod
    def supported(xyz, feats_pm, weight):
        return (SA_POINT_LINEAR and SPLIT_GEMM and SaGatherLinear.supported(xyz, feats_pm, weight) and weight.shape[0] in (128, 256, 512, 1024)
                and feats_pm.shape[0] * feats_pm.shape[1] >= SPLIT_GEMM_MIN_TOKENS)

    @staticmethod
    def forward(ctx, xyz, new_xyz, feats_pm, idx, weight):
        B, N, _ = xyz.shape
        M, ns = idx.shape[1], idx.shape[2]
        C, n_out = feats_pm.shape[-1], weight.shape[0]
        xyz, new_xyz, feats_pm, idx = xyz.contiguous(), new_xyz.contiguous(), feats_pm.contiguous(), idx.contiguous()
        w = weight.detach().contiguous()
        w_f = w[:, 3:].contiguous()
        rows = _gemm_nt(feats_pm.view(B * N, C), w_f)
        z = torch.empty((B, M, ns, n_out), dtype=torch.float32, device=xyz.device)
        pointnet2.sa_point_gather(rows, xyz, new_xyz, idx, w, z, B, N, M, ns, n_out)
        ctx.save_for_backward(xyz, new_xyz, feats_pm, idx, weight)
        return z

    @staticmethod
    def backward(ctx, grad_out):
        xyz, new_xyz, feats_pm, idx, weight = ctx.saved_tensors
        B, M, ns = idx.shape
        n_out, C, N = weight.shape[0], feats_pm.shape[-1], xyz.shape[1]
        g2 = grad_out.contiguous().view(-1, n_out)
        g_new = g_feats = gw = None
        with torch.no_grad():
            w = weight.contiguous()
            if ctx.needs_input_grad[4] or ctx.needs_input_grad[1]:
                gw = torch.empty_like(weight)
                g_new = torch.empty_like(new_xyz) if ctx.needs_input_grad[1] else None
                pointnet2.sa_xyz_grad(g2, xyz, new_xyz, idx, w, gw, g_new, B, N, M, ns, n_out)
            if ctx.needs_input_grad[4] or ctx.needs_input_grad[2]:
                g_pts = torch.zeros((B, N, n_out), dtype=torch.float32, device=g2.device)
                pointnet2.group_rows_grad(B, N, n_out, M * ns, g2, idx, g_pts)
                g_pts = g_pts.view(B * N, n_out)
                if ctx.needs_input_grad[4]:
                    gw[:, 3:] = _wgrad(feats_pm.view(B * N, C), g_pts, torch.empty((n_out, C), dtype=weight.dtype, device=weight.device), False)[0]
                if ctx.needs_input_grad[2]:
                    g_feats = _gemm_nn(g_pts, w[:, 3:].contiguous()).view(B, N, C)
            if not ctx.needs_input_grad[4]:
                gw = None
        return None, g_new, g_feats, None, gw


SA_WIDE_INFER_SPLIT = os.environ.get("PDA_SA_WIDE_INFER_SPLIT", "1") != "0"
SA_WIDE_INFER_GATHER_IN_GEMM = os.environ.get("PDA_SA_WIDE_INFER_GATHER_IN_GEMM", "1") != "0"


def sa_wide_scale_infer(xyz, new_xyz, feats_pm, idx, folded):
    (w1, b1), (w2, b2), (w3, b3) = folded
    B, N, _ = xyz.shape
    M, ns = idx.shape[1], idx.shape[2]
    C = feats_pm.shape[-1]
    T = B * M * ns
    c1, c2, c3 = w1.shape[0], w2.shape[0], w3.shape[0]
    if not (SA_WIDE_INFER_SPLIT and SPLIT_GEMM and not DENSE_BF16 and w1.shape[1] == 3 + C and C % 32 == 0 and c1 in (128, 256, 512, 1024)
            and c1 % 32 == 0 and c2 % 128 == 0 and c3 % 128 == 0 and B * N >= SPLIT_GEMM_MIN_TOKENS and T >= SPLIT_GEMM_MIN_TOKENS):
        return None
    out = []

    def run():
        rows = _gemm_nt(feats_pm.reshape(B * N, C), w1[:, 3:].contiguous())
        if SA_WIDE_INFER_GATHER_IN_GEMM and c1 % 32 == 0 and c1 <= 1024:
            y2 = torch.empty((T, c2), dtype=torch.float32, device=xyz.device)
            pointnet2.gemm_split_gather(rows, xyz.contiguous(), new_xyz.contiguous(), idx.contiguous(), w1.contiguous(), b1.detach().contiguous(),
                                        _split_planes(w2), b2.detach().contiguous(), y2, B, N, M, ns, c1, c2, relu=True)
        else:
            y1 = torch.empty((T, c1), dtype=torch.float32, device=xyz.device)
            pointnet2.sa_point_gather(rows, xyz.contiguous(), new_xyz.contiguous(), idx.contiguous(), w1, y1, B, N, M, ns, c1, bias=b1, relu=True)
            y2 = _gemm_nt(y1, w2, b2, relu=True)
            del y1
        if ns in (16, 32, 64) and c2 % 32 == 0:
            pooled = torch.empty((B, M, c3), dtype=torch.float32, device=xyz.device)
            pointnet2.gemm_split_maxpool(y2, _split_planes(w3), b3.detach().contiguous(), pooled, T, c2, c3, ns, relu=True)
            out.append(pooled)
            return
        y3 = _gemm_nt(y2, w3, b3, relu=True)
        del y2
        out.append(y3.view(B, M, ns, c3).amax(dim=2))
    _sa_timed(2.0 * T * (c1 * c2 + c2 * c3), run, "bf16x6_infer")
    return out[0]


SA_SMALL_TRAIN = True
FUSED_WIDE_CHAIN_OK = True


class SaSmallChainTrain(Function):

    @staticmethod
    def supported(xyz, new_xyz, feats_pm, idx, mlp):
        layers = list(mlp)
        if not (SA_SMALL_TRAIN and len(layers) == 9 and xyz.is_cuda and xyz.dtype == torch.float32 and not DENSE_BF16
                and not torch.is_autocast_enabled() and not xyz.requires_grad and not new_xyz.requires_grad
                and (feats_pm is None or (feats_pm.dtype == torch.float32 and not feats_pm.requires_grad))):
            return False
        for k in range(3):
            conv, bn, act = layers[3 * k:3 * k + 3]
            if not (isinstance(conv, nn.Conv2d) and conv.bias is None and conv.kernel_size == (1, 1) and isinstance(bn, nn.BatchNorm2d)
                    and isinstance(act, nn.ReLU) and bn.training and bn.affine and bn.momentum is not None
                    and conv.weight.dtype == torch.float32):
                return False
        c = 0 if feats_pm is None else feats_pm.shape[-1]
        c1, c2, c3 = (layers[3 * k].out_channels for k in range(3))
        return layers[0].in_channels == 3 + c and pointnet2.sa_small_train_supported(c, idx.shape[2], c1, c2, c3, idx.numel())

    @staticmethod
    def forward(ctx, xyz, new_xyz, feats_pm, idx, w1, w2, w3, g1, b1, g2, b2, g3, b3, bns):
        B, N, _ = xyz.shape
        M, ns = idx.shape[1], idx.shape[2]
        c = 0 if feats_pm is None else feats_pm.shape[-1]
        c3 = w3.shape[0]
        dev = xyz.device
        xyz, new_xyz, idx = xyz.contiguous(), new_xyz.contiguous(), idx.contiguous()
        feats_pm = None if feats_pm is None else feats_pm.contiguous()
        ws = torch.empty((pointnet2.sa_small_train_workspace_bytes(),), dtype=torch.uint8, device=dev)
        out = torch.empty((B, M, c3), dtype=torch.float32, device=dev)
        zmax = torch.empty((B, M, c3), dtype=torch.float32, device=dev)
        arg = torch.empty((B, M, c3), dtype=torch.uint8, device=dev)
        track = [bn.track_running_stats for bn in bns]
        macs = w1.numel() + w2.numel() + w3.numel()
        _sa_timed(2.0 * B * M * ns * macs, lambda: pointnet2.sa_small_train_fwd(
            xyz, new_xyz, feats_pm, idx, (w1.contiguous(), w2.contiguous(), w3.contiguous()), (g1, g2, g3), (b1, b2, b3),
            [bn.running_mean if t else None for bn, t in zip(bns, track)],
            [bn.running_var if t else None for bn, t in zip(bns, track)],
            [bn.eps for bn in bns], [bn.momentum for bn in bns], ws, out, zmax, arg, B, N, M, c, ns), "f32_recompute")
        ctx.save_for_backward(xyz, new_xyz, feats_pm, idx, zmax, arg, ws, w1, w2, w3)
        ctx.dims = (B, N, M, c, ns)
        return out

    @staticmethod
    def backward(ctx, grad_out):
        xyz, new_xyz, feats_pm, idx, zmax, arg, ws, w1, w2, w3 = ctx.saved_tensors
        B, N, M, c, ns = ctx.dims
        tokens = B * M * ns
        dev = xyz.device
        dz2 = torch.empty((tokens, w2.shape[0]), dtype=torch.float32, device=dev)
        dz1 = torch.empty((tokens, w1.shape[0]), dtype=torch.float32, device=dev)
        dws = [torch.empty(w.shape, dtype=torch.float32, device=dev) for w in (w1, w2, w3)]
        dgs = [torch.empty((w.shape[0],), dtype=torch.float32, device=dev) for w in (w1, w2, w3)]
        dbs = [torch.empty((w.shape[0],), dtype=torch.float32, device=dev) for w in (w1, w2, w3)]
        gout = grad_out.contiguous().float()
        macs = w1.numel() + w2.numel() + w3.numel()
        _sa_timed(2.0 * tokens * (2 * macs - w1.numel()), lambda: pointnet2.sa_small_train_bwd(
            xyz, new_xyz, feats_pm, idx, gout, zmax, arg, ws, dz2, dz1, dws, dgs, dbs, B, N, M, c, ns), "f32_recompute")
        return (None, None, None, None, dws[0], dws[1], dws[2], dgs[0], dbs[0], dgs[1], dbs[1], dgs[2], dbs[2], None)


def sa_small_chain_train(xyz, new_xyz, feats_pm, idx, mlp):
    layers = list(mlp)
    convs, bns = [layers[0], layers[3], layers[6]], [layers[1], layers[4], layers[7]]
    for bn in bns:
        bump_bn_counter(bn)
    return SaSmallChainTrain.apply(xyz, new_xyz, feats_pm, idx, convs[0].weight.flatten(1), convs[1].weight.flatten(1),
                                   convs[2].weight.flatten(1), bns[0].weight, bns[0].bias, bns[1].weight, bns[1].bias,
                                   bns[2].weight, bns[2].bias, bns)


SA_WIDE_CHAIN = os.environ.get("PDA_SA_WIDE_CHAIN", "1") != "0"
WIDE_CHAIN_DGRAD_FIRST = os.environ.get("PDA_WIDE_CHAIN_DGRAD_FIRST", "1") != "0"
SA_WIDE_CHAIN_MIN_TOKENS = int(os.environ.get("PDA_SA_WIDE_CHAIN_MIN_TOKENS", "32768"))


class SaWideChainTrain(Function):

    @staticmethod
    def supported(xyz, new_xyz, feats_pm, idx, mlp):
        layers = list(mlp)
        if not (SA_WIDE_CHAIN and FUSED_WIDE_CHAIN_OK and len(layers) == 9 and feats_pm is not None and idx is not None):
            return False
        convs, bns = [layers[0], layers[3], layers[6]], [layers[1], layers[4], layers[7]]
        if not (all(isinstance(c, nn.Conv2d) and c.bias is None and c.weight.dtype == torch.float32 for c in convs)
                and all(isinstance(b, nn.BatchNorm2d) and b.affine and b.training and b.momentum is not None for b in bns)
                and all(isinstance(layers[k], nn.ReLU) for k in (2, 5, 8))):
            return False
        w1 = convs[0].weight.flatten(1)
        if not SaPointLinear.supported(xyz, feats_pm, w1):
            return False
        c1, c2, c3 = (c.weight.shape[0] for c in convs)
        T = idx.shape[0] * idx.shape[1] * idx.shape[2]
        if not (c1 % 256 == 0 and c2 % 256 == 0 and c3 % 256 == 0 and max(c1, c2, c3) <= 1024 and 1 <= idx.shape[2] <= 255
                and T >= SA_WIDE_CHAIN_MIN_TOKENS and not DENSE_BF16 and not torch.is_autocast_enabled()):
            return False
        lib = _lib.load()
        return int(lib.pda_linear_wgrad_form(T, c1, c2)) == 2 and int(lib.pda_linear_wgrad_form(T, c2, c3)) == 2

    @staticmethod
    def forward(ctx, xyz, new_xyz, feats_pm, idx, w1, w2, w3, g1, b1, g2, b2, g3, b3, bns):
        B, N, _ = xyz.shape
        M, ns = idx.shape[1], idx.shape[2]
        C, c1, c2, c3 = feats_pm.shape[-1], w1.shape[0], w2.shape[0], w3.shape[0]
        T = B * M * ns
        dev = xyz.device
        xyz, new_xyz, feats_pm, idx = xyz.contiguous(), new_xyz.contiguous(), feats_pm.contiguous(), idx.contiguous()
        gs = [t.detach().contiguous() for t in (g1, g2, g3)]
        bs = [t.detach().contiguous() for t in (b1, b2, b3)]
        stats = [(bn.running_mean, bn.running_var) if bn.track_running_stats else (None, None) for bn in bns]
        w1d = w1.detach().contiguous()
        rows = _gemm_nt(feats_pm.view(B * N, C), w1d[:, 3:].contiguous())
        z1 = torch.empty((T, c1), dtype=torch.float32, device=dev)
        pointnet2.sa_point_gather(rows, xyz, new_xyz, idx, w1d, z1, B, N, M, ns, c1)
        mi1 = torch.empty((2 * c1,), dtype=torch.float32, device=dev)
        scratch = torch.empty((pointnet2.bn_relu_scratch_bytes(c1),), dtype=torch.uint8, device=dev)
        pointnet2.bn_stats_fwd(z1, stats[0][0], stats[0][1], mi1, scratch, T, c1, bns[0].eps, bns[0].momentum)
        tiles = pointnet2.gemm_split_bn_tiles(T)

        def layer(z_in, mi_in, k, w, n_out, bn, st, gi, bi):
            z = torch.empty((T, n_out), dtype=torch.float32, device=dev)
            part = torch.empty((tiles * 2 * n_out,), dtype=torch.float64, device=dev)
            wf = _split_planes(w)
            _sa_timed(2.0 * T * k * n_out, lambda: pointnet2.gemm_split_bn(z_in, wf, z, T, k, n_out, in_bn=(mi_in, gi, bi), stats_mode=1,
                                                                           partial=part), "bf16x6")
            mi = torch.empty((2 * n_out,), dtype=torch.float32, device=dev)
            pointnet2.bn_finalize_fwd(part, tiles, n_out, T, bn.eps, bn.momentum, mi, st[0], st[1])
            return z, mi
        z2, mi2 = layer(z1, mi1, c1, w2, c2, bns[1], stats[1], gs[0], bs[0])
        z3, mi3 = layer(z2, mi2, c2, w3, c3, bns[2], stats[2], gs[1], bs[1])
        out = torch.empty((B, M, c3), dtype=torch.float32, device=dev)
        arg = torch.empty((B, M, c3), dtype=torch.uint8, device=dev)
        pointnet2.bn_relu_max_pool_apply(z3, gs[2], bs[2], mi3, out, arg, B * M, ns, c3)
        ctx.save_for_backward(xyz, new_xyz, feats_pm, idx, w1, w2, w3, g1, b1, g2, b2, g3, b3, z1, z2, z3, mi1, mi2, mi3, arg)
        return out

    @staticmethod
    def backward(ctx, grad_out):
        xyz, new_xyz, feats_pm, idx, w1, w2, w3, g1, b1, g2, b2, g3, b3, z1, z2, z3, mi1, mi2, mi3, arg = ctx.saved_tensors
        B, M, ns = idx.shape
        N, C = xyz.shape[1], feats_pm.shape[-1]
        c1, c2, c3 = w1.shape[0], w2.shape[0], w3.shape[0]
        T = B * M * ns
        dev = xyz.device
        tiles = pointnet2.gemm_split_bn_tiles(T)
        with torch.no_grad():
            g1c, b1c, g2c, b2c, g3c, b3c = (t.contiguous() for t in (g1, b1, g2, b2, g3, b3))
            gz3 = torch.empty((T, c3), dtype=torch.float32, device=dev)
            dg3, db3 = torch.empty_like(g3c), torch.empty_like(b3c)
            scratch = torch.empty((pointnet2.bn_relu_scratch_bytes(c3),), dtype=torch.uint8, device=dev)
            pointnet2.bn_relu_max_pool_bwd(z3, grad_out.contiguous().float(), arg, g3c, b3c, mi3, gz3, dg3, db3, scratch, B * M, ns, c3)

            def layer(gz, w, z_in, mi_in, gi, bi, k_in, n_out):
                dw = torch.empty((n_out, k_in), dtype=torch.float32, device=dev)
                ga = torch.empty((T, k_in), dtype=torch.float32, device=dev)
                if WIDE_CHAIN_DGRAD_FIRST:
                    _lin_cols(gz, w, ga, T, n_out, k_in, True)
                    pointnet2.linear_wgrad_bn(z_in, gz, dw, T, k_in, n_out, mi_in, gi, bi)
                else:
                    pointnet2.linear_wgrad_bn(z_in, gz, dw, T, k_in, n_out, mi_in, gi, bi)
                    _lin_cols(gz, w, ga, T, n_out, k_in, True)
                dg, db = torch.empty_like(gi), torch.empty_like(bi)
                scratch = torch.empty((pointnet2.bn_relu_scratch_bytes(k_in),), dtype=torch.uint8, device=dev)
                pointnet2.bn_relu_bwd(z_in, ga, gi, bi, mi_in, ga, dg, db, scratch, T, k_in)
                return dw, ga, dg, db
            dw3, gz2, dg2, db2 = layer(gz3, w3, z2, mi2, g2c, b2c, c2, c3)
            del gz3
            dw2, gz1, dg1, db1 = layer(gz2, w2, z1, mi1, g1c, b1c, c1, c2)
            del gz2
            w1c = w1.contiguous()
            dw1 = torch.empty_like(w1c)
            g_new = torch.empty_like(new_xyz) if ctx.needs_input_grad[1] else None
            pointnet2.sa_xyz_grad(gz1, xyz, new_xyz, idx, w1c, dw1, g_new, B, N, M, ns, c1)
            g_pts = torch.zeros((B, N, c1), dtype=torch.float32, device=dev)
            pointnet2.group_rows_grad(B, N, c1, M * ns, gz1, idx, g_pts)
            g_pts = g_pts.view(B * N, c1)
            dw1[:, 3:] = _wgrad(feats_pm.view(B * N, C), g_pts, torch.empty((c1, C), dtype=torch.float32, device=dev), False)[0]
            g_feats = _gemm_nn(g_pts, w1c[:, 3:].contiguous()).view(B, N, C) if ctx.needs_input_grad[2] else None
        return None, g_new, g_feats, None, dw1, dw2, dw3, dg1, db1, dg2, db2, dg3, db3, None


def sa_wide_chain_train(xyz, new_xyz, feats_pm, idx, mlp):
    layers = list(mlp)
    convs, bns = [layers[0], layers[3], layers[6]], [layers[1], layers[4], layers[7]]
    for bn in bns:
        bump_bn_counter(bn)
    return SaWideChainTrain.apply(xyz, new_xyz, feats_pm, idx, convs[0].weight.flatten(1), convs[1].weight.flatten(1),
                                  convs[2].weight.flatten(1), bns[0].weight, bns[0].bias, bns[1].weight, bns[1].bias,
                                  bns[2].weight, bns[2].bias, bns)


RAGGED_TOKENS = True
RAGGED_MAX_FRACTION = 0.85


class RaggedPlan:
    __slots__ = ("cnt", "off", "rowmap", "roww", "tokens", "groups", "nsample")

    def __init__(self, cnt, off, rowmap, roww, tokens, groups, nsample):
        self.cnt, self.off, self.rowmap, self.roww = cnt, off, rowmap, roww
        self.tokens, self.groups, self.nsample = tokens, groups, nsample

    @property
    def fraction(self):
        return self.tokens / float(self.groups * self.nsample)


def ragged_plan_parts(idxs):
    parts = []
    for idx in idxs:
        G, ns = idx.shape[0] * idx.shape[1], idx.shape[2]
        cnt = torch.empty((G,), dtype=torch.int32, device=idx.device)
        off = torch.empty((G + 1,), dtype=torch.int32, device=idx.device)
        rowmap = torch.empty((G * ns,), dtype=torch.int32, device=idx.device)
        roww = torch.empty((G * ns,), dtype=torch.float32, device=idx.device)
        pointnet2.ragged_plan(idx, cnt, off, rowmap, G, ns, roww)
        parts.append((cnt, off, rowmap, roww, G, ns))
    return parts, torch.stack([p[1][-1] for p in parts])


def ragged_plans_from(parts, totals):
    return [RaggedPlan(c, o, r[:u], w[:u], int(u), G, ns) for (c, o, r, w, G, ns), u in zip(parts, totals)]


def ragged_plans(idxs):
    parts, totals = ragged_plan_parts(idxs)
    return ragged_plans_from(parts, totals.tolist())


ASSEMBLE_BWD_TOKEN_PARALLEL = os.environ.get("PDA_ASSEMBLE_BWD_TOKEN_PARALLEL", "1") != "0"


class AssembleTokensRagged(Function):

    @staticmethod
    def forward(ctx, rppe, dscale, feats_pm, idx, glob, plan):
        B, M, ns = idx.shape
        C, N = feats_pm.shape[-1], feats_pm.shape[1]
        compact = rppe.dim() == 2
        rppe, dscale, feats_pm, glob = rppe.contiguous(), dscale.contiguous(), feats_pm.contiguous(), glob.contiguous()
        out = torch.empty((plan.tokens, 4 * C), dtype=torch.float32, device=rppe.device)
        pointnet2.assemble_tokens_ragged(rppe, dscale, feats_pm, idx, glob, plan.rowmap, plan.off, out, plan.tokens, B, N, M, ns, C,
                                         rppe_compact=compact)
        ctx.save_for_backward(dscale, feats_pm, idx, plan.cnt, plan.off, plan.rowmap)
        ctx.dims = (B, N, M, ns, C, plan.tokens, compact)
        return out

    @staticmethod
    def backward(ctx, grad_out):
        dscale, feats_pm, idx, cnt, off, rowmap = ctx.saved_tensors
        B, N, M, ns, C, U, compact = ctx.dims
        dev = grad_out.device
        g_rppe = torch.empty((U, C) if compact else (B, M, ns, C), dtype=torch.float32, device=dev)
        g_ds = torch.empty_like(dscale)
        g_feats = torch.zeros((B, N, C), dtype=torch.float32, device=dev)
        g_glob = torch.empty((B, M, C), dtype=torch.float32, device=dev)
        pointnet2.assemble_tokens_ragged_grad(grad_out.contiguous(), dscale, feats_pm, idx, cnt, off, g_rppe, g_ds, g_feats, g_glob,
                                              U, B, N, M, ns, C, rppe_compact=compact,
                                              rowmap=rowmap if ASSEMBLE_BWD_TOKEN_PARALLEL else None)
        return g_rppe, g_ds, g_feats, None, g_glob, None


RAGGED_POSITION_MLP = True


class BatchNormReLUWeighted(Function):

    @staticmethod
    def forward(ctx, x, weight, bias, running_mean, running_var, eps, momentum, roww, count):
        x = x.contiguous()
        rows, c = x.shape
        y = torch.empty_like(x)
        stats = torch.empty((2 * c,), dtype=torch.float32, device=x.device)
        scratch = torch.empty((pointnet2.bn_relu_scratch_bytes(c),), dtype=torch.uint8, device=x.device)
        pointnet2.bn_relu_fwd_weighted(x, weight, bias, running_mean, running_var, y, stats, scratch, rows, c, eps, momentum, roww, count)
        ctx.save_for_backward(x, weight, bias, stats, roww)
        ctx.count = count
        return y

    @staticmethod
    def backward(ctx, grad_y):
        x, weight, bias, stats, roww = ctx.saved_tensors
        rows, c = x.shape
        gx = torch.empty_like(x)
        gw, gb = torch.empty_like(weight), torch.empty_like(bias)
        scratch = torch.empty((pointnet2.bn_relu_scratch_bytes(c),), dtype=torch.uint8, device=x.device)
        pointnet2.bn_relu_bwd_weighted(x, grad_y.contiguous(), weight, bias, stats, gx, gw, gb, scratch, rows, c, roww, ctx.count)
        return gx, gw, gb, None, None, None, None, None, None


def position_mlp_ragged_supported(layers, rppe):
    layers = list(layers)
    ok = (RAGGED_POSITION_MLP and rppe.is_cuda and rppe.dtype == torch.float32 and len(layers) == 6 and torch.is_grad_enabled()
          and not DENSE_BF16 and not torch.is_autocast_enabled())
    if not ok:
        return False
    for conv, bn in ((layers[0], layers[1]), (layers[3], layers[4])):
        c = conv.weight.shape[0]
        if (conv.bias is not None or not bn.training or not bn.affine or bn.momentum is None or c < 4 or c > 1024
                or (c & (c - 1)) != 0):
            return False
    return True


def position_mlp_ragged(layers, rppe, plan):
    layers = list(layers)
    x = rppe.reshape(-1, rppe.shape[-1]).index_select(0, plan.rowmap)
    count = plan.groups * plan.nsample
    for conv, bn in ((layers[0], layers[1]), (layers[3], layers[4])):
        x = linear(x, conv.weight.flatten(1), None)
        rm, rv = (bn.running_mean, bn.running_var) if bn.track_running_stats else (None, None)
        bump_bn_counter(bn)
        x = BatchNormReLUWeighted.apply(x, bn.weight, bn.bias, rm, rv, bn.eps, bn.momentum, plan.roww, count)
    return x


def _wgrad_ragged(x2d, g2d, weight, want_bias):
    n_out, n_in = weight.shape
    tokens = x2d.shape[0]
    if (LINEAR_WGRAD_KERNEL and tokens >= 4096 and (min(n_out, n_in) >= 64 or max(n_out, n_in) <= 64) and n_out % 4 == 0
            and n_in % 4 == 0 and x2d.dtype == torch.float32 and g2d.dtype == torch.float32):
        gw = torch.empty_like(weight)
        gb = torch.empty((n_out,), dtype=torch.float32, device=x2d.device) if want_bias else None
        pointnet2.linear_wgrad(x2d.contiguous(), g2d.contiguous(), gw, gb, tokens, n_in, n_out)
        return gw, gb
    return g2d.t().mm(x2d), (g2d.sum(0) if want_bias else None)


class RaggedTransformerBlock(Function):

    @staticmethod
    def supported(d, heads, nsample, x):
        return (RAGGED_TOKENS and x.is_cuda and x.dtype == torch.float32 and d in (256, 512, 1024) and d % heads == 0
                and nsample in GroupAttention.SUPPORTED_SEQ and d // heads in GroupAttention.SUPPORTED_HD
                and not torch.is_autocast_enabled() and not DENSE_BF16)

    @staticmethod
    def forward(ctx, x, plan, n1w, n1b, in_w, in_b, out_w, out_b, n2w, n2b, w1, b1, w2, b2, heads, eps1, eps2):
        x = x.contiguous()
        U, D = x.shape
        G, S, hd = plan.groups, plan.nsample, D // heads
        dev = x.device
        f32 = dict(dtype=torch.float32, device=dev)
        src1, ssum, src2 = torch.empty_like(x), torch.empty_like(x), torch.empty_like(x)
        st1, st2 = torch.empty((U, 2), **f32), torch.empty((U, 2), **f32)
        lse = torch.empty((G, heads, S), **f32)
        pointnet2.layer_norm_fwd(x, None, n1w, n1b, None, src1, st1, U, D, eps1)
        qkv = _gemm_nt(src1, in_w, in_b)
        a = torch.empty((U, D), **f32)
        pointnet2.group_attention_ragged_fwd(qkv, plan.cnt, plan.off, a, lse, U, G, S, heads, hd)
        proj = _gemm_nt(a, out_w, out_b)
        pointnet2.layer_norm_fwd(proj, src1, n2w, n2b, ssum, src2, st2, U, D, eps2)
        del proj
        h = _gemm_nt(src2, w1, b1, relu=True)
        ffn = _gemm_nt(h, w2, b2)
        y = torch.empty((G, D), **f32)
        arg = torch.empty((G, D), dtype=torch.uint8, device=dev)
        pointnet2.add_max_pool_ragged(src2, ffn, plan.cnt, plan.off, y, arg, U, G, D)
        ctx.save_for_backward(x, st1, src1, qkv, lse, a, ssum, st2, src2, h, n1w, in_w, out_w, n2w, w1, w2, arg,
                              plan.cnt, plan.off, plan.rowmap)
        ctx.heads, ctx.dims = heads, (G, S)
        return y

    @staticmethod
    def backward(ctx, dy):
        x, st1, src1, qkv, lse, a, ssum, st2, src2, h, n1w, in_w, out_w, n2w, w1, w2, arg, cnt, off, rowmap = ctx.saved_tensors
        U, D = x.shape
        G, S = ctx.dims
        heads = ctx.heads
        hd = D // heads
        dev = x.device
        f32 = dict(dtype=torch.float32, device=dev)
        dy2 = torch.empty((U, D), **f32)
        pointnet2.max_pool_scatter_ragged(dy.contiguous(), arg, rowmap, off, dy2, U, G, S, D)
        d_h = _gemm_nn(dy2, w2)
        gw2, gb2 = _wgrad_ragged(h, dy2, w2, True)
        d_h = torch.ops.aten.threshold_backward(d_h, h, 0)
        gw1, gb1 = _wgrad_ragged(src2, d_h, w1, True)
        d_lin1 = _gemm_nn(d_h, w1)
        del d_h
        d_s = torch.empty((U, D), **f32)
        gn2w, gn2b = torch.empty_like(n2w), torch.empty_like(n2w)
        scratch = torch.empty((pointnet2.layer_norm_scratch_bytes(D),), dtype=torch.uint8, device=dev)
        pointnet2.layer_norm_bwd(ssum, dy2, n2w, st2, d_s, gn2w, gn2b, scratch, U, D, grad_y2=d_lin1)
        del d_lin1
        d_a = _gemm_nn(d_s, out_w)
        gwo, gbo = _wgrad_ragged(a, d_s, out_w, True)
        dqkv = torch.empty_like(qkv)
        pointnet2.group_attention_ragged_bwd(qkv, d_a, lse, cnt, off, dqkv, U, G, S, heads, hd)
        del d_a
        gwi, gbi = _wgrad_ragged(src1, dqkv, in_w, True)
        d_src1 = _gemm_nn(dqkv, in_w, acc=d_s)
        del dqkv
        d_x = torch.empty_like(x)
        gn1w, gn1b = torch.empty_like(n1w), torch.empty_like(n1w)
        pointnet2.layer_norm_bwd(x, d_src1, n1w, st1, d_x, gn1w, gn1b, scratch, U, D)
        return d_x, None, gn1w, gn1b, gwi, gbi, gwo, gbo, gn2w, gn2b, gw1, gb1, gw2, gb2, None, None, None


def ragged_transformer_block(tr, x, plan):
    at = tr.self_attn
    return RaggedTransformerBlock.apply(x, plan, tr.norm1.weight, tr.norm1.bias, at.in_proj_weight, at.in_proj_bias,
                                        at.out_proj.weight, at.out_proj.bias, tr.norm2.weight, tr.norm2.bias,
                                        tr.linear1.weight, tr.linear1.bias, tr.linear2.weight, tr.linear2.bias,
                                        at.num_heads, tr.norm1.eps, tr.norm2.eps)


class LayerNormResidual(Function):

    @staticmethod
    def supported(x, d):
        return x.is_cuda and x.dtype == torch.float32 and x.shape[-1] == d and d in (256, 512, 1024) and x.numel() > 0

    @staticmethod
    def forward(ctx, x, residual, weight, bias, eps):
        x = x.contiguous()
        d = x.shape[-1]
        rows = x.numel() // d
        y = torch.empty_like(x)
        stats = torch.empty((rows, 2), dtype=torch.float32, device=x.device)
        if residual is not None:
            s = torch.empty_like(x)
            pointnet2.layer_norm_fwd(x, residual.contiguous(), weight, bias, s, y, stats, rows, d, eps)
        else:
            s = x
            pointnet2.layer_norm_fwd(x, None, weight, bias, None, y, stats, rows, d, eps)
        ctx.save_for_backward(s, weight, stats)
        ctx.has_residual = residual is not None
        return y

    @staticmethod
    def backward(ctx, grad_y):
        s, weight, stats = ctx.saved_tensors
        d = s.shape[-1]
        rows = s.numel() // d
        gx = torch.empty_like(s)
        gw, gb = torch.empty_like(weight), torch.empty_like(weight)
        scratch = torch.empty((pointnet2.layer_norm_scratch_bytes(d),), dtype=torch.uint8, device=s.device)
        pointnet2.layer_norm_bwd(s, grad_y.contiguous(), weight, stats, gx, gw, gb, scratch, rows, d)
        return gx, (gx if ctx.has_residual else None), gw, gb, None


def layer_norm(x, ln, residual=None):
    return LayerNormResidual.apply(x, residual, ln.weight, ln.bias, ln.eps)


class BallQuery(Function):

    @staticmethod
    @_fwd
    def forward(ctx, radius: float, nsample: int, xyz: torch.Tensor, new_xyz: torch.Tensor) -> torch.Tensor:
        assert new_xyz.is_contiguous()
        assert xyz.is_contiguous()
        B, N, _ = xyz.size()
        npoint = new_xyz.size(1)
        idx = torch.zeros((B, npoint, nsample), dtype=torch.int32, device=xyz.device)
        pointnet2.ball_query_wrapper(B, N, npoint, radius, nsample, new_xyz, xyz, idx)
        ctx.mark_non_differentiable(idx)
        return idx

    @staticmethod
    def backward(ctx, a=None):
        return None, None, None, None


ball_query = BallQuery.apply


class BallQueryDilated(Function):

    @staticmethod
    @_fwd
    def forward(ctx, max_radius: float, min_radius: float, nsample: int, xyz: torch.Tensor,
                new_xyz: torch.Tensor) -> torch.Tensor:
        assert new_xyz.is_contiguous()
        assert xyz.is_contiguous()
        B, N, _ = xyz.size()
        npoint = new_xyz.size(1)
# ... 158 lines not shown
```

Measured before the change: 121.1 scenes/s.

## Fuse SA wide-chain passes: gather+BN stats, zmax pool backward, fused tail backward

Adds a gather kernel that computes layer-1 BN statistics while producing z1, so a separate stats pass over z1 is no longer needed. The forward max-pool also saves the pre-BN value at each argmax (zmax), so the backward BN reduction can run over only the B*M pooled rows instead of all T tokens. In backward, the layer-1 BN-ReLU apply is folded into the xyz-gradient and row-scatter kernel (sa_wide_tail_bwd), removing another full pass over z1/grad tensors. The cost is an extra saved zmax buffer, plus heavier kernels carrying more registers and scatter work. The new path is gated by PDA_SA_WIDE_PASSES, which is on by default.

```diff
diff --git a/include/pda_train.h b/include/pda_train.h
--- a/include/pda_train.h
+++ b/include/pda_train.h
@@ -70,6 +70,13 @@
                         float *mean_invstd, float *running_mean, float *running_var, pda_stream_t stream);
 int pda_bn_relu_max_pool_apply(const float *x, const float *gamma, const float *beta, const float *mean_invstd,
                                float *out, uint8_t *arg, int64_t groups, int ns, int c, pda_stream_t stream);
+int pda_bn_relu_max_pool_apply_zmax(const float *x, const float *gamma, const float *beta, const float *mean_invstd,
+                                    float *out, uint8_t *arg, float *zmax, int64_t groups, int ns, int c,
+                                    pda_stream_t stream);
+int pda_bn_relu_max_pool_bwd_zmax(const float *x, const float *grad_out, const uint8_t *arg, const float *zmax,
+                                  const float *gamma, const float *beta, const float *mean_invstd, float *grad_x,
+                                  float *grad_gamma, float *grad_beta, void *scratch, int64_t groups, int ns, int c,
+                                  pda_stream_t stream);
 
 int64_t pda_colsum_scratch_bytes(int cols);
 int pda_colsum_bf16(const uint16_t *g, float *out, void *scratch, int64_t rows, int cols, pda_stream_t stream);
@@ -211,6 +218,15 @@
 int pda_sa_xyz_grad(const float *grad_z1, const float *xyz, const float *new_xyz, const int32_t *idx, const float *w, int ldw,
                     float *dw, int lddw, float *grad_new_xyz, void *scratch, int b, int n, int m, int nsample, int c1,
                     pda_stream_t stream);
+int pda_sa_point_gather_stats(const float *point_rows, const float *xyz, const float *new_xyz, const int32_t *idx,
+                              const float *w, int ldw, float *z, float *running_mean, float *running_var,
+                              float *mean_invstd, void *scratch, int b, int n, int m, int nsample, int c1, float eps,
+                              float momentum, pda_stream_t stream);
+int pda_sa_wide_tail_bwd(const float *z1, const float *grad_a1, const float *gamma, const float *beta,
+                         const float *mean_invstd, float *grad_gamma, float *grad_beta, void *bn_scratch,
+                         const float *xyz, const float *new_xyz, const int32_t *idx, const float *w, int ldw, float *dw,
+                         int lddw, float *grad_new_xyz, float *grad_rows, void *scratch, int b, int n, int m,
+                         int nsample, int c1, pda_stream_t stream);
 
 int64_t pda_input_stage_workspace_bytes(int batch, int64_t n_cap);
 int pda_input_stage(const float *points, const int64_t *offsets, int64_t n_total, int batch, int c, int64_t n_cap,
diff --git a/pdanet_amd/_lib.py b/pdanet_amd/_lib.py
--- a/pdanet_amd/_lib.py
+++ b/pdanet_amd/_lib.py
@@ -100,6 +100,8 @@
     "pda_bn_stats_fwd": [_vp, _vp, _vp, _vp, _vp, ctypes.c_int64, _i, _f, _f, _vp],
     "pda_bn_finalize_fwd": [_vp, _i, _i, ctypes.c_int64, _f, _f, _vp, _vp, _vp, _vp],
     "pda_bn_relu_max_pool_apply": [_vp, _vp, _vp, _vp, _vp, _vp, ctypes.c_int64, _i, _i, _vp],
+    "pda_bn_relu_max_pool_apply_zmax": [_vp] * 7 + [ctypes.c_int64, _i, _i, _vp],
+    "pda_bn_relu_max_pool_bwd_zmax": [_vp] * 11 + [ctypes.c_int64, _i, _i, _vp],
     "pda_colsum_scratch_bytes": [_i],
     "pda_colsum_bf16": [_vp, _vp, _vp, ctypes.c_int64, _i, _vp],
     "pda_assemble_tokens": [_vp, _vp, _vp, _vp, _vp, _vp, _i, _i, _i, _i, _i, _vp],
@@ -148,6 +150,8 @@
     "pda_sa_xyz_grad_scratch_bytes": [_i],
     "pda_sa_point_gather": [_vp, _vp, _vp, _vp, _vp, _i, _vp, _i, _vp, _i, _i, _i, _i, _i, _vp],
     "pda_sa_xyz_grad": [_vp, _vp, _vp, _vp, _vp, _i, _vp, _i, _vp, _vp, _i, _i, _i, _i, _i, _vp],
+    "pda_sa_point_gather_stats": [_vp] * 5 + [_i] + [_vp] * 5 + [_i] * 5 + [_f, _f, _vp],
+    "pda_sa_wide_tail_bwd": [_vp] * 12 + [_i, _vp, _i] + [_vp] * 3 + [_i] * 5 + [_vp],
     "pda_adam_onecycle_step": [_vp, _vp, _vp, _vp, ctypes.c_int64, _f, _f, _f, _f, _f, _i, _vp, _f, _vp],
     "pda_input_stage_workspace_bytes": [_i, ctypes.c_int64],
     "pda_input_stage": [_vp, _vp, ctypes.c_int64, _i, _i, ctypes.c_int64, ctypes.POINTER(_f), _i, _vp, _vp, _vp,
diff --git a/pdanet_amd/csrc/bn_partials.h b/pdanet_amd/csrc/bn_partials.h
--- /dev/null
+++ b/pdanet_amd/csrc/bn_partials.h
@@ -0,0 +1,30 @@
+#pragma once
+#include "pda_common.h"
+
+namespace pda {
+
+constexpr int BN_BLOCKS = 512;
+
+__device__ __forceinline__ void block_reduce_cols(double (&a)[4], double (&b)[4], double* lds, int cg, int rpb, double* out_a,
+                                                  double* out_b) {
+    const int tid = threadIdx.x;
+    double* la = lds;
+    double* lb = lds + 256 * 4;
+#pragma unroll
+    for (int k = 0; k < 4; ++k) { la[tid * 4 + k] = a[k]; lb[tid * 4 + k] = b[k]; }
+    __syncthreads();
+    if (tid < cg) {
+        double sa[4] = {0, 0, 0, 0}, sb[4] = {0, 0, 0, 0};
+        for (int r = 0; r < rpb; ++r)
+#pragma unroll
+            for (int k = 0; k < 4; ++k) { sa[k] += la[(r * cg + tid) * 4 + k]; sb[k] += lb[(r * cg + tid) * 4 + k]; }
+#pragma unroll
+        for (int k = 0; k < 4; ++k) { out_a[tid * 4 + k] = sa[k]; out_b[tid * 4 + k] = sb[k]; }
+    }
+}
+
+int bn_relu_bwd_sums(const float* x, const float* grad_y, const float* gamma, const float* beta, const float* mean_invstd, float* grad_gamma,
+                     float* grad_beta, void* scratch, int64_t rows, int c, hipStream_t st, const char* what);
+inline float* bn_bwd_sums(void* scratch, int c) { return reinterpret_cast<float*>(reinterpret_cast<double*>(scratch) + (size_t)BN_BLOCKS * 2 * c); }
+
+}
diff --git a/pdanet_amd/csrc/bn_relu.hip b/pdanet_amd/csrc/bn_relu.hip
--- a/pdanet_amd/csrc/bn_relu.hip
+++ b/pdanet_amd/csrc/bn_relu.hip
@@ -1,8 +1,7 @@
 #include "pda_common.h"
+#include "bn_partials.h"
 
 namespace pda {
-
-constexpr int BN_BLOCKS = 512;
 
 struct BnShape {
     int64_t rows;
@@ -19,24 +18,6 @@
     const float4 v = reinterpret_cast<const float4*>(gout)[g * s.cg + col];
     const uchar4 k = reinterpret_cast<const uchar4*>(arg)[g * s.cg + col];
     return make_float4(k.x == t ? v.x : 0.f, k.y == t ? v.y : 0.f, k.z == t ? v.z : 0.f, k.w == t ? v.w : 0.f);
-}
-
-__device__ __forceinline__ void block_reduce_cols(double (&a)[4], double (&b)[4], double* lds, int cg, int rpb, double* out_a,
-                                                  double* out_b) {
-    const int tid = threadIdx.x;
-    double* la = lds;
-    double* lb = lds + 256 * 4;
-#pragma unroll
-    for (int k = 0; k < 4; ++k) { la[tid * 4 + k] = a[k]; lb[tid * 4 + k] = b[k]; }
-    __syncthreads();
-    if (tid < cg) {
-        double sa[4] = {0, 0, 0, 0}, sb[4] = {0, 0, 0, 0};
-        for (int r = 0; r < rpb; ++r)
-#pragma unroll
-            for (int k = 0; k < 4; ++k) { sa[k] += la[(r * cg + tid) * 4 + k]; sb[k] += lb[(r * cg + tid) * 4 + k]; }
-#pragma unroll
-        for (int k = 0; k < 4; ++k) { out_a[tid * 4 + k] = sa[k]; out_b[tid * 4 + k] = sb[k]; }
-    }
 }
 
 template <bool BWD, typename TX, typename TD, bool POOL = false>
@@ -75,8 +56,10 @@
         };
         auto grad = [&](int64_t r) -> float4 {
             if constexpr (!BWD) return make_float4(0, 0, 0, 0);
-            else if constexpr (POOL) return pooled_grad(reinterpret_cast<const float*>(dy), arg, r, col, s);
-            else return load4(dy + r * s.c + 4 * col);
+            else if constexpr (POOL) {
+                if (arg == nullptr) return load4(reinterpret_cast<const float*>(dy) + r * s.c + 4 * col);
+                return pooled_grad(reinterpret_cast<const float*>(dy), arg, r, col, s);
+            } else return load4(dy + r * s.c + 4 * col);
         };
         constexpr int U = BWD ? 1 : 4;
         int64_t r = (int64_t)blockIdx.x * s.rpb + r0;
@@ -200,11 +183,11 @@
     for (; r < s.rows; r += stride) { const int64_t q = last - r; row(q, load4(x + q * s.c + 4 * col), grad(q)); }
 }
 
-template <typename TX>
+template <typename TX, bool ZMAX = false>
 __global__ __launch_bounds__(256) void bn_apply_pool_kernel(const TX* __restrict__ x, const float* __restrict__ mean_invstd,
                                                             const float* __restrict__ gamma, const float* __restrict__ beta,
                                                             float* __restrict__ out, uint8_t* __restrict__ arg, int64_t groups,
-                                                            BnShape s) {
+                                                            BnShape s, float* __restrict__ zmax = nullptr) {
     const int64_t e = (int64_t)blockIdx.x * 256 + threadIdx.x;
     if (e >= groups * s.cg) return;
     const int64_t g = e / s.cg;
@@ -213,18 +196,20 @@
     const float4 gm = reinterpret_cast<const float4*>(gamma)[col], be = reinterpret_cast<const float4*>(beta)[col];
     float4 best = make_float4(-1.f, -1.f, -1.f, -1.f);
     uchar4 bi = make_uchar4(0, 0, 0, 0);
+    float4 zb = make_float4(0.f, 0.f, 0.f, 0.f);
     const TX* px = x + (size_t)g * s.ns * s.c + 4 * col;
     for (int t = 0; t < s.ns; ++t) {
         const float4 v = load4(px + (size_t)t * s.c);
         const float y0 = fmaxf((v.x - mu.x) * is.x * gm.x + be.x, 0.f), y1 = fmaxf((v.y - mu.y) * is.y * gm.y + be.y, 0.f);
         const float y2 = fmaxf((v.z - mu.z) * is.z * gm.z + be.z, 0.f), y3 = fmaxf((v.w - mu.w) * is.w * gm.w + be.w, 0.f);
-        if (y0 > best.x) { best.x = y0; bi.x = (uint8_t)t; }
-        if (y1 > best.y) { best.y = y1; bi.y = (uint8_t)t; }
-        if (y2 > best.z) { best.z = y2; bi.z = (uint8_t)t; }
-        if (y3 > best.w) { best.w = y3; bi.w = (uint8_t)t; }
+        if (y0 > best.x) { best.x = y0; bi.x = (uint8_t)t; if (ZMAX) zb.x = v.x; }
+        if (y1 > best.y) { best.y = y1; bi.y = (uint8_t)t; if (ZMAX) zb.y = v.y; }
+        if (y2 > best.z) { best.z = y2; bi.z = (uint8_t)t; if (ZMAX) zb.z = v.z; }
+        if (y3 > best.w) { best.w = y3; bi.w = (uint8_t)t; if (ZMAX) zb.w = v.w; }
     }
     reinterpret_cast<float4*>(out)[e] = best;
     reinterpret_cast<uchar4*>(arg)[e] = bi;
+    if (ZMAX) reinterpret_cast<float4*>(zmax)[e] = zb;
 }
 
 static int bn_shape(int64_t rows, int c, BnShape& s, const char* what) {
@@ -452,3 +437,60 @@
                        mean_invstd, gamma, beta, out, arg, groups, s);
     return pda::check_launch(what);
 }
+
+PDA_API int pda_bn_relu_max_pool_apply_zmax(const float* x, const float* gamma, const float* beta, const float* mean_invstd, float* out,
+                                            uint8_t* arg, float* zmax, int64_t groups, int ns, int c, pda_stream_t stream) {
+    const char* what = "pda_bn_relu_max_pool_apply_zmax";
+    PDA_REQUIRE(groups >= 1 && ns >= 1 && ns <= 255, "%s: groups=%lld ns=%d (1..255)", what, (long long)groups, ns);
+    pda::BnShape s;
+    if (int rc = pda::bn_shape(groups * ns, c, s, what)) return rc;
+    s.ns = ns;
+    PDA_REQUIRE(x && gamma && beta && out && arg && zmax && mean_invstd, "%s: null pointer", what);
+    PDA_REQUIRE(pda::bn_aligned(x) && (((uintptr_t)out | (uintptr_t)zmax | (uintptr_t)gamma | (uintptr_t)beta | (uintptr_t)mean_invstd) & 15) == 0 &&
+                    ((uintptr_t)arg & 3) == 0, "%s: alignment", what);
+    hipLaunchKernelGGL((pda::bn_apply_pool_kernel<float, true>), dim3((unsigned)pda::divup64(groups * s.cg, 256)), dim3(256), 0, (hipStream_t)stream,
+                       x, mean_invstd, gamma, beta, out, arg, groups, s, zmax);
+    return pda::check_launch(what);
+}
+
+PDA_API int pda_bn_relu_max_pool_bwd_zmax(const float* x, const float* grad_out, const uint8_t* arg, const float* zmax, const float* gamma,
+                                          const float* beta, const float* mean_invstd, float* grad_x, float* grad_gamma, float* grad_beta,
+                                          void* scratch, int64_t groups, int ns, int c, pda_stream_t stream) {
+    using namespace pda;
+    const char* what = "pda_bn_relu_max_pool_bwd_zmax";
+    PDA_REQUIRE(groups >= 1 && ns >= 1 && ns <= 255, "%s: groups=%lld ns=%d (1..255)", what, (long long)groups, ns);
+    BnShape s, sg;
+    if (int rc = bn_shape(groups * ns, c, s, what)) return rc;
+    if (int rc = bn_shape(groups, c, sg, what)) return rc;
+    s.ns = ns;
+    PDA_REQUIRE(x && grad_out && arg && zmax && gamma && beta && mean_invstd && grad_x && grad_gamma && grad_beta && scratch, "%s: null pointer", what);
+    PDA_REQUIRE(bn_aligned(x) && bn_aligned(grad_x) &&
+                    (((uintptr_t)grad_out | (uintptr_t)zmax | (uintptr_t)gamma | (uintptr_t)beta | (uintptr_t)mean_invstd) & 15) == 0 &&
+                    ((uintptr_t)arg & 3) == 0, "%s: alignment", what);
+    hipStream_t st = (hipStream_t)stream;
+    const int rgrid = bn_grid(sg), grid = bn_grid(s);
+    float* sums = reinterpret_cast<float*>(reinterpret_cast<double*>(scratch) + (size_t)BN_BLOCKS * 2 * c);
+    hipLaunchKernelGGL((bn_reduce_kernel<true, float, float, true>), dim3(rgrid), dim3(256), 0, st, zmax, grad_out, mean_invstd, gamma, beta,
+                       (double*)scratch, sg, (const uint8_t*)nullptr);
+    hipLaunchKernelGGL(bn_finalize_bwd_kernel, dim3(divup(c, 32)), dim3(512), 0, st, (const double*)scratch, rgrid, c, s.rows, grad_gamma, grad_beta,
+                       sums);
+    hipLaunchKernelGGL((bn_apply_kernel<true, float, float, float, true>), dim3(grid), dim3(256), 0, st, x, grad_out, mean_invstd, gamma, beta, sums,
+                       grad_x, s, arg);
+    return check_launch(what);
+}
+
+namespace pda {
+int bn_relu_bwd_sums(const float* x, const float* grad_y, const float* gamma, const float* beta, const float* mean_invstd, float* grad_gamma,
+                     float* grad_beta, void* scratch, int64_t rows, int c, hipStream_t st, const char* what) {
+    BnShape s;
+    if (int rc = bn_shape(rows, c, s, what)) return rc;
+    PDA_REQUIRE(x && grad_y && gamma && beta && mean_invstd && grad_gamma && grad_beta && scratch, "%s: null pointer", what);
+    PDA_REQUIRE(bn_aligned(x) && bn_aligned(grad_y) && (((uintptr_t)gamma | (uintptr_t)beta | (uintptr_t)mean_invstd) & 15) == 0,
+                "%s: pointers must be 16-byte aligned", what);
+    const int grid = bn_grid(s);
+    hipLaunchKernelGGL((bn_reduce_kernel<true, float, float>), dim3(grid), dim3(256), 0, st, x, grad_y, mean_invstd, gamma, beta, (double*)scratch, s);
+    hipLaunchKernelGGL(bn_finalize_bwd_kernel, dim3(divup(c, 32)), dim3(512), 0, st, (const double*)scratch, grid, c, s.count, grad_gamma, grad_beta,
+                       bn_bwd_sums(scratch, c));
+    return check_launch(what);
+}
+}
diff --git a/pdanet_amd/csrc/sa_xyz_grad.hip b/pdanet_amd/csrc/sa_xyz_grad.hip
--- a/pdanet_amd/csrc/sa_xyz_grad.hip
+++ b/pdanet_amd/csrc/sa_xyz_grad.hip
@@ -1,4 +1,5 @@
 #include "pda_common.h"
+#include "bn_partials.h"
 
 namespace pda {
 
@@ -6,19 +7,36 @@
 constexpr int XG_THREADS = 256;
 constexpr int XG_MAXC = 4;
 
-template <int CPT>
+struct SaTailBn {
+    const float* z1;
+    const float* mean_invstd;
+    const float* gamma;
+    const float* beta;
+    const float* sums;
+    float* grad_rows;
+};
+
+template <int CPT, bool TAIL = false>
 __global__ __launch_bounds__(XG_THREADS) void sa_xyz_grad_kernel(const float* __restrict__ g, const float* __restrict__ xyz,
                                                                  const float* __restrict__ new_xyz, const int32_t* __restrict__ idx,
                                                                  const float* __restrict__ w, int ldw, float* __restrict__ partial,
-                                                                 float* __restrict__ grad_new, int n, int m, int ns, int c1, int64_t groups) {
+                                                                 float* __restrict__ grad_new, int n, int m, int ns, int c1, int64_t groups,
+                                                                 SaTailBn bn = SaTailBn()) {
     __shared__ float red[XG_THREADS / 64][3];
     const int tid = threadIdx.x;
     float accw[CPT][3], wx[CPT][3];
+    float mu[CPT], is[CPT], gm[CPT], be[CPT], m1[CPT], m2[CPT];
 #pragma unroll
     for (int q = 0; q < CPT; ++q) {
         const int o = tid + q * XG_THREADS;
 #pragma unroll
         for (int d = 0; d < 3; ++d) { accw[q][d] = 0.f; wx[q][d] = o < c1 ? w[(size_t)o * ldw + d] : 0.f; }
+        if (TAIL && o < c1) {
+            mu[q] = bn.mean_invstd[o]; is[q] = bn.mean_invstd[c1 + o]; gm[q] = bn.gamma[o]; be[q] = bn.beta[o];
+            m1[q] = bn.sums[o]; m2[q] = bn.sums[c1 + o];
+        } else {
+            mu[q] = is[q] = gm[q] = be[q] = m1[q] = m2[q] = 0.f;
+        }
     }
     for (int64_t grp = blockIdx.x; grp < groups; grp += gridDim.x) {
         const int bs = (int)(grp / m);
@@ -27,11 +45,13 @@
         const float* pts = xyz + (size_t)bs * n * 3;
         const int32_t* ids = idx + grp * ns;
         const float* grow = g + grp * ns * (int64_t)c1;
+        const float* zrow = TAIL ? bn.z1 + grp * ns * (int64_t)c1 : nullptr;
+        float* prow = TAIL ? bn.grad_rows + (size_t)bs * n * c1 : nullptr;
         float gs[CPT];
 #pragma unroll
         for (int q = 0; q < CPT; ++q) gs[q] = 0.f;
         for (int s0 = 0; s0 < ns; s0 += 8) {
-            float gv[8][CPT], dx[8], dy[8], dz[8];
+            float gv[8][CPT], zv[TAIL ? 8 : 1][CPT], dx[8], dy[8], dz[8];
 #pragma unroll
             for (int u = 0; u < 8; ++u) {
                 const int s = s0 + u < ns ? s0 + u : ns - 1;
@@ -41,7 +61,21 @@
                 for (int q = 0; q < CPT; ++q) {
                     const int o = tid + q * XG_THREADS;
                     gv[u][q] = (s0 + u < ns && o < c1) ? grow[(int64_t)s * c1 + o] : 0.f;
+                    if constexpr (TAIL) zv[u][q] = (s0 + u < ns && o < c1) ? zrow[(int64_t)s * c1 + o] : 0.f;
                 }
+            }
+            if constexpr (TAIL) {
+#pragma unroll
+                for (int u = 0; u < 8; ++u)
+#pragma unroll
+                    for (int q = 0; q < CPT; ++q) {
+                        const int o = tid + q * XG_THREADS;
+                        const float xh = (zv[u][q] - mu[q]) * is[q];
+                        const float dyh = (xh * gm[q] + be[q] > 0.f) ? gv[u][q] : 0.f;
+                        gv[u][q] = gm[q] * is[q] * (dyh - (m1[q] + xh * m2[q]));
+                        if (s0 + u < ns && o < c1) atomicAdd(prow + (size_t)ids[s0 + u] * c1 + o, gv[u][q]);
+                        else gv[u][q] = 0.f;
+                    }
             }
 #pragma unroll
             for (int u = 0; u < 8; ++u)
@@ -98,11 +132,14 @@
     }
 }
 
+template <bool STATS = false>
 __global__ __launch_bounds__(256) void sa_point_gather_kernel(const float* __restrict__ prow, const float* __restrict__ xyz,
                                                               const float* __restrict__ new_xyz, const int32_t* __restrict__ idx,
                                                               const float* __restrict__ w, int ldw, const float* __restrict__ bias,
                                                               int relu, float* __restrict__ z, int n, int m, int ns, int c1,
-                                                              int64_t tokens) {
+                                                              int64_t tokens, double* __restrict__ partial = nullptr) {
+    __shared__ double lds[STATS ? 2 * 256 * 4 : 1];
+    double sa[4] = {0, 0, 0, 0}, sb[4] = {0, 0, 0, 0};
     const int cq = c1 >> 2;
     const int q = threadIdx.x % cq;
     float wx[4], wy[4], wz[4];
@@ -114,22 +151,40 @@
     float bq[4] = {0.f, 0.f, 0.f, 0.f};
     if (bias) { const float4 b4 = *reinterpret_cast<const float4*>(bias + 4 * q); bq[0] = b4.x; bq[1] = b4.y; bq[2] = b4.z; bq[3] = b4.w; }
     const int tpb = 256 / cq;
-    for (int64_t tok = (int64_t)blockIdx.x * tpb + threadIdx.x / cq; tok < tokens; tok += (int64_t)gridDim.x * tpb) {
-        const int64_t grp = tok / ns;
-        const int bs = (int)(grp / m);
-        const int id = idx[tok];
-        const float* pt = xyz + ((size_t)bs * n + id) * 3;
-        const float* ct = new_xyz + grp * 3;
-        const float dx = pt[0] - ct[0], dy = pt[1] - ct[1], dz = pt[2] - ct[2];
-        const float4 p4 = *reinterpret_cast<const float4*>(prow + ((size_t)bs * n + id) * c1 + 4 * q);
-        const float pv[4] = {p4.x, p4.y, p4.z, p4.w};
-        float o[4];
-#pragma unroll
-        for (int k = 0; k < 4; ++k) {
-            o[k] = __builtin_fmaf(wz[k], dz, __builtin_fmaf(wy[k], dy, __builtin_fmaf(wx[k], dx, pv[k]))) + bq[k];
-            o[k] = relu ? fmaxf(o[k], 0.f) : o[k];
-        }
-        *reinterpret_cast<float4*>(z + tok * c1 + 4 * q) = make_float4(o[0], o[1], o[2], o[3]);
+    const int64_t stride = (int64_t)gridDim.x * tpb;
+    constexpr int U = STATS ? 4 : 1;
+    int64_t tok = (int64_t)blockIdx.x * tpb + threadIdx.x / cq;
+    for (; tok < tokens; tok += U * stride) {
+        float dx[U], dy[U], dz[U];
+        float4 p4[U];
+#pragma unroll
+        for (int u = 0; u < U; ++u) {
+            const int64_t t = tok + u * stride < tokens ? tok + u * stride : tok;
+            const int64_t grp = t / ns;
+            const int bs = (int)(grp / m);
+            const int id = idx[t];
+            const float* pt = xyz + ((size_t)bs * n + id) * 3;
+            const float* ct = new_xyz + grp * 3;
+            dx[u] = pt[0] - ct[0]; dy[u] = pt[1] - ct[1]; dz[u] = pt[2] - ct[2];
+            p4[u] = *reinterpret_cast<const float4*>(prow + ((size_t)bs * n + id) * c1 + 4 * q);
+        }
+#pragma unroll
+        for (int u = 0; u < U; ++u) {
+            if (tok + u * stride >= tokens) break;
+            const float pv[4] = {p4[u].x, p4[u].y, p4[u].z, p4[u].w};
+            float o[4];
+#pragma unroll
+            for (int k = 0; k < 4; ++k) {
+                o[k] = __builtin_fmaf(wz[k], dz[u], __builtin_fmaf(wy[k], dy[u], __builtin_fmaf(wx[k], dx[u], pv[k]))) + bq[k];
+                o[k] = relu ? fmaxf(o[k], 0.f) : o[k];
+                if (STATS) { sa[k] += o[k]; sb[k] += (double)o[k] * o[k]; }
+            }
+            *reinterpret_cast<float4*>(z + (tok + u * stride) * c1 + 4 * q) = make_float4(o[0], o[1], o[2], o[3]);
+        }
+    }
+    if constexpr (STATS) {
+        double* pa = partial + (size_t)blockIdx.x * 2 * c1;
+        block_reduce_cols(sa, sb, lds, cq, tpb, pa, pa + c1);
     }
 }
 
@@ -149,7 +204,7 @@
     }
     const int64_t total = tokens * (c1 >> 2);
     const int blocks = (int)(divup64(total, 256) < 8192 ? divup64(total, 256) : 8192);
-    hipLaunchKernelGGL(sa_point_gather_kernel, dim3(blocks), dim3(256), 0, (hipStream_t)stream, point_rows, xyz, new_xyz, idx, w, ldw, bias, relu, z,
+    hipLaunchKernelGGL(sa_point_gather_kernel<false>, dim3(blocks), dim3(256), 0, (hipStream_t)stream, point_rows, xyz, new_xyz, idx, w, ldw, bias, relu, z,
                        n, m, ns, c1, tokens);
     return check_launch("pda_sa_point_gather");
 }
@@ -179,3 +234,53 @@
     hipLaunchKernelGGL(sa_xyz_grad_reduce_kernel, dim3(divup(c1 * 3, 16)), dim3(256), 0, s, (const float*)partial, blocks, c1, dw, lddw);
     return check_launch("pda_sa_xyz_grad");
 }
+
+PDA_API int pda_sa_point_gather_stats(const float* point_rows, const float* xyz, const float* new_xyz, const int32_t* idx, const float* w, int ldw,
+                                      float* z, float* running_mean, float* running_var, float* mean_invstd, void* scratch, int b, int n, int m,
+                                      int ns, int c1, float eps, float momentum, pda_stream_t stream) {
+    using namespace pda;
+    const char* what = "pda_sa_point_gather_stats";
+    PDA_REQUIRE(b >= 1 && n >= 1 && m >= 1 && ns >= 1 && c1 >= 4 && (c1 & 3) == 0 && ldw >= 3, "%s: bad size", what);
+    const int64_t tokens = (int64_t)b * m * ns;
+    PDA_REQUIRE(point_rows && xyz && new_xyz && idx && w && z && mean_invstd && scratch &&
+                    (((uintptr_t)point_rows | (uintptr_t)z | (uintptr_t)mean_invstd | (uintptr_t)scratch) & 15) == 0,
+                "%s: null or misaligned pointer", what);
+    if (c1 > 1024 || 256 % (c1 >> 2) != 0) {
+        set_error("%s: c1 = %d (c1 / 4 must divide 256)", what, c1);
+        return PDA_ERR_UNSUPPORTED;
+    }
+    const int64_t steps = divup64(tokens, 256 / (c1 >> 2));
+    const int blocks = (int)(steps < BN_BLOCKS ? steps : BN_BLOCKS);
+    hipLaunchKernelGGL(sa_point_gather_kernel<true>, dim3(blocks), dim3(256), 0, (hipStream_t)stream, point_rows, xyz, new_xyz, idx, w, ldw,
+                       (const float*)nullptr, 0, z, n, m, ns, c1, tokens, (double*)scratch);
+    if (int rc = check_launch(what)) return rc;
+    return pda_bn_finalize_fwd((const double*)scratch, blocks, c1, tokens, eps, momentum, mean_invstd, running_mean, running_var, stream);
+}
+
+PDA_API int pda_sa_wide_tail_bwd(const float* z1, const float* grad_a1, const float* gamma, const float* beta, const float* mean_invstd,
+                                 float* grad_gamma, float* grad_beta, void* bn_scratch, const float* xyz, const float* new_xyz,
+                                 const int32_t* idx, const float* w, int ldw, float* dw, int lddw, float* grad_new_xyz, float* grad_rows,
+                                 void* scratch, int b, int n, int m, int ns, int c1, pda_stream_t stream) {
+    using namespace pda;
+    const char* what = "pda_sa_wide_tail_bwd";
+    PDA_REQUIRE(b >= 1 && n >= 1 && m >= 1 && ns >= 1 && c1 >= 1 && ldw >= 3 && lddw >= 3, "%s: bad size", what);
+    const int64_t groups = (int64_t)b * m;
+    PDA_REQUIRE(xyz && new_xyz && idx && w && dw && grad_rows && scratch, "%s: null pointer", what);
+    if (c1 > XG_THREADS * XG_MAXC) {
+        set_error("%s: c1 = %d > %d", what, c1, XG_THREADS * XG_MAXC);
+        return PDA_ERR_UNSUPPORTED;
+    }
+    const hipStream_t s = (hipStream_t)stream;
+    if (int rc = bn_relu_bwd_sums(z1, grad_a1, gamma, beta, mean_invstd, grad_gamma, grad_beta, bn_scratch, groups * ns, c1, s, what)) return rc;
+    SaTailBn bn;
+    bn.z1 = z1; bn.mean_invstd = mean_invstd; bn.gamma = gamma; bn.beta = beta; bn.sums = bn_bwd_sums(bn_scratch, c1); bn.grad_rows = grad_rows;
+    const int blocks = (int)(groups < XG_BLOCKS ? groups : XG_BLOCKS);
+    float* partial = (float*)scratch;
+    const int cpt = divup(c1, XG_THREADS);
+#define PDA_XG(CPT) hipLaunchKernelGGL((sa_xyz_grad_kernel<CPT, true>), dim3(blocks), dim3(XG_THREADS), 0, s, grad_a1, xyz, new_xyz, idx, w, ldw, \
+                                       partial, grad_new_xyz, n, m, ns, c1, groups, bn)
+    if (cpt == 1) PDA_XG(1); else if (cpt == 2) PDA_XG(2); else PDA_XG(4);
+#undef PDA_XG
+    hipLaunchKernelGGL(sa_xyz_grad_reduce_kernel, dim3(divup(c1 * 3, 16)), dim3(256), 0, s, (const float*)partial, blocks, c1, dw, lddw);
+    return check_launch(what);
+}
diff --git a/pdanet_amd/pointnet2_batch_cuda.py b/pdanet_amd/pointnet2_batch_cuda.py
--- a/pdanet_amd/pointnet2_batch_cuda.py
+++ b/pdanet_amd/pointnet2_batch_cuda.py
@@ -464,6 +464,24 @@
     _numel_ok(x, groups * ns * c, "x"); _numel_ok(out, groups * c, "out"); _numel_ok(arg, groups * c, "arg"); _numel_ok(mean_invstd, 2 * c, "mean_invstd")
     _call("pda_bn_relu_max_pool_apply", x, _chk(x, "x", F32), _chk(gamma, "gamma", F32), _chk(beta, "beta", F32),
           _chk(mean_invstd, "mean_invstd", F32), _chk(out, "out", F32), _chk(arg, "arg", torch.uint8), groups, ns, c)
+    return 1
+
+
+def bn_relu_max_pool_apply_zmax(x, gamma, beta, mean_invstd, out, arg, zmax, groups, ns, c):
+    _numel_ok(x, groups * ns * c, "x"); _numel_ok(out, groups * c, "out"); _numel_ok(arg, groups * c, "arg"); _numel_ok(zmax, groups * c, "zmax")
+    _numel_ok(mean_invstd, 2 * c, "mean_invstd")
+    _call("pda_bn_relu_max_pool_apply_zmax", x, _chk(x, "x", F32), _chk(gamma, "gamma", F32), _chk(beta, "beta", F32),
+          _chk(mean_invstd, "mean_invstd", F32), _chk(out, "out", F32), _chk(arg, "arg", torch.uint8), _chk(zmax, "zmax", F32), groups, ns, c)
+    return 1
+
+
+def bn_relu_max_pool_bwd_zmax(x, grad_out, arg, zmax, gamma, beta, mean_invstd, grad_x, grad_gamma, grad_beta, scratch, groups, ns, c):
+    _numel_ok(x, groups * ns * c, "x"); _numel_ok(grad_out, groups * c, "grad_out"); _numel_ok(arg, groups * c, "arg")
+    _numel_ok(zmax, groups * c, "zmax"); _numel_ok(grad_x, groups * ns * c, "grad_x")
+    _call("pda_bn_relu_max_pool_bwd_zmax", x, _chk(x, "x", F32), _chk(grad_out, "grad_out", F32), _chk(arg, "arg", torch.uint8),
+          _chk(zmax, "zmax", F32), _chk(gamma, "gamma", F32), _chk(beta, "beta", F32), _chk(mean_invstd, "mean_invstd", F32),
+          _chk(grad_x, "grad_x", F32), _chk(grad_gamma, "grad_gamma", F32), _chk(grad_beta, "grad_beta", F32),
+          _chk(scratch, "scratch", torch.uint8), groups, ns, c)
     return 1
 
 
@@ -820,3 +838,36 @@
           _chk(idx, "idx", I32), _chk(w, "w", F32), int(w.shape[1]), None if bias is None else _chk(bias, "bias", F32),
           1 if relu else 0, _chk(z, "z", F32), b, n, m, ns, c1)
     return 1
+
+
+def sa_point_gather_stats(point_rows, xyz, new_xyz, idx, w, z, running_mean, running_var, mean_invstd, scratch, b, n, m, ns, c1, eps, momentum):
+    _numel_ok(point_rows, b * n * c1, "point_rows"); _numel_ok(z, b * m * ns * c1, "z"); _numel_ok(idx, b * m * ns, "idx")
+    _numel_ok(xyz, b * n * 3, "xyz"); _numel_ok(new_xyz, b * m * 3, "new_xyz"); _numel_ok(mean_invstd, 2 * c1, "mean_invstd")
+    assert w.shape[0] == c1 and w.shape[1] >= 3 and scratch.numel() >= bn_relu_scratch_bytes(c1)
+    rm = None if running_mean is None else _chk(running_mean, "running_mean", F32)
+    rv = None if running_var is None else _chk(running_var, "running_var", F32)
+    _buffers_written(rm)
+    _call("pda_sa_point_gather_stats", xyz, _chk(point_rows, "point_rows", F32), _chk(xyz, "xyz", F32), _chk(new_xyz, "new_xyz", F32),
+          _chk(idx, "idx", I32), _chk(w, "w", F32), int(w.shape[1]), _chk(z, "z", F32), rm, rv, _chk(mean_invstd, "mean_invstd", F32),
+          _chk(scratch, "scratch", torch.uint8), b, n, m, ns, c1, float(eps), float(momentum))
+    return 1
+
+
+def sa_wide_tail_bwd(z1, grad_a1, gamma, beta, mean_invstd, grad_gamma, grad_beta, xyz, new_xyz, idx, w, dw, grad_new_xyz, grad_rows,
+                     b, n, m, ns, c1):
+    _numel_ok(z1, b * m * ns * c1, "z1"); _numel_ok(grad_a1, b * m * ns * c1, "grad_a1"); _numel_ok(idx, b * m * ns, "idx")
+    _numel_ok(xyz, b * n * 3, "xyz"); _numel_ok(new_xyz, b * m * 3, "new_xyz"); _numel_ok(grad_rows, b * n * c1, "grad_rows")
+    _numel_ok(mean_invstd, 2 * c1, "mean_invstd"); _numel_ok(gamma, c1, "gamma"); _numel_ok(beta, c1, "beta")
+    _numel_ok(grad_gamma, c1, "grad_gamma"); _numel_ok(grad_beta, c1, "grad_beta")
+    assert w.shape[0] == c1 and dw.shape == w.shape and w.shape[1] >= 3
+    if grad_new_xyz is not None:
+        _numel_ok(grad_new_xyz, b * m * 3, "grad_new_xyz")
+    bn_scratch = torch.empty((bn_relu_scratch_bytes(c1),), dtype=torch.uint8, device=xyz.device)
+    scratch = torch.empty((sa_xyz_grad_scratch_bytes(c1),), dtype=torch.uint8, device=xyz.device)
+    _call("pda_sa_wide_tail_bwd", xyz, _chk(z1, "z1", F32), _chk(grad_a1, "grad_a1", F32), _chk(gamma, "gamma", F32), _chk(beta, "beta", F32),
+          _chk(mean_invstd, "mean_invstd", F32), _chk(grad_gamma, "grad_gamma", F32), _chk(grad_beta, "grad_beta", F32),
+          _chk(bn_scratch, "bn_scratch", torch.uint8), _chk(xyz, "xyz", F32), _chk(new_xyz, "new_xyz", F32), _chk(idx, "idx", I32),
+          _chk(w, "w", F32), int(w.shape[1]), _chk(dw, "dw", F32), int(dw.shape[1]),
+          None if grad_new_xyz is None else _chk(grad_new_xyz, "grad_new_xyz", F32), _chk(grad_rows, "grad_rows", F32),
+          _chk(scratch, "scratch", torch.uint8), b, n, m, ns, c1)
+    return 1
diff --git a/pdanet_amd/pointnet2_utils.py b/pdanet_amd/pointnet2_utils.py
--- a/pdanet_amd/pointnet2_utils.py
+++ b/pdanet_amd/pointnet2_utils.py
@@ -1161,6 +1161,7 @@
 
 SA_WIDE_CHAIN = os.environ.get("PDA_SA_WIDE_CHAIN", "1") != "0"
 WIDE_CHAIN_DGRAD_FIRST = os.environ.get("PDA_WIDE_CHAIN_DGRAD_FIRST", "1") != "0"
+SA_WIDE_PASSES = os.environ.get("PDA_SA_WIDE_PASSES", "1") != "0"
 SA_WIDE_CHAIN_MIN_TOKENS = int(os.environ.get("PDA_SA_WIDE_CHAIN_MIN_TOKENS", "32768"))
 
 
@@ -1201,10 +1202,14 @@
         w1d = w1.detach().contiguous()
         rows = _gemm_nt(feats_pm.view(B * N, C), w1d[:, 3:].contiguous())
         z1 = torch.empty((T, c1), dtype=torch.float32, device=dev)
-        pointnet2.sa_point_gather(rows, xyz, new_xyz, idx, w1d, z1, B, N, M, ns, c1)
         mi1 = torch.empty((2 * c1,), dtype=torch.float32, device=dev)
         scratch = torch.empty((pointnet2.bn_relu_scratch_bytes(c1),), dtype=torch.uint8, device=dev)
-        pointnet2.bn_stats_fwd(z1, stats[0][0], stats[0][1], mi1, scratch, T, c1, bns[0].eps, bns[0].momentum)
+        if SA_WIDE_PASSES:
+            pointnet2.sa_point_gather_stats(rows, xyz, new_xyz, idx, w1d, z1, stats[0][0], stats[0][1], mi1, scratch, B, N, M, ns, c1,
+                                            bns[0].eps, bns[0].momentum)
+        else:
+            pointnet2.sa_point_gather(rows, xyz, new_xyz, idx, w1d, z1, B, N, M, ns, c1)
+            pointnet2.bn_stats_fwd(z1, stats[0][0], stats[0][1], mi1, scratch, T, c1, bns[0].eps, bns[0].momentum)
         tiles = pointnet2.gemm_split_bn_tiles(T)
 
         def layer(z_in, mi_in, k, w, n_out, bn, st, gi, bi):
@@ -1220,13 +1225,18 @@
         z3, mi3 = layer(z2, mi2, c2, w3, c3, bns[2], stats[2], gs[1], bs[1])
         out = torch.empty((B, M, c3), dtype=torch.float32, device=dev)
         arg = torch.empty((B, M, c3), dtype=torch.uint8, device=dev)
-        pointnet2.bn_relu_max_pool_apply(z3, gs[2], bs[2], mi3, out, arg, B * M, ns, c3)
-        ctx.save_for_backward(xyz, new_xyz, feats_pm, idx, w1, w2, w3, g1, b1, g2, b2, g3, b3, z1, z2, z3, mi1, mi2, mi3, arg)
+        zmax = None
+        if SA_WIDE_PASSES:
+            zmax = torch.empty((B, M, c3), dtype=torch.float32, device=dev)
+            pointnet2.bn_relu_max_pool_apply_zmax(z3, gs[2], bs[2], mi3, out, arg, zmax, B * M, ns, c3)
+        else:
+            pointnet2.bn_relu_max_pool_apply(z3, gs[2], bs[2], mi3, out, arg, B * M, ns, c3)
+        ctx.save_for_backward(xyz, new_xyz, feats_pm, idx, w1, w2, w3, g1, b1, g2, b2, g3, b3, z1, z2, z3, mi1, mi2, mi3, arg, zmax)
         return out
 
     @staticmethod
     def backward(ctx, grad_out):
-        xyz, new_xyz, feats_pm, idx, w1, w2, w3, g1, b1, g2, b2, g3, b3, z1, z2, z3, mi1, mi2, mi3, arg = ctx.saved_tensors
+        xyz, new_xyz, feats_pm, idx, w1, w2, w3, g1, b1, g2, b2, g3, b3, z1, z2, z3, mi1, mi2, mi3, arg, zmax = ctx.saved_tensors
         B, M, ns = idx.shape
         N, C = xyz.shape[1], feats_pm.shape[-1]
         c1, c2, c3 = w1.shape[0], w2.shape[0], w3.shape[0]
@@ -1238,9 +1248,13 @@
             gz3 = torch.empty((T, c3), dtype=torch.float32, device=dev)
             dg3, db3 = torch.empty_like(g3c), torch.empty_like(b3c)
             scratch = torch.empty((pointnet2.bn_relu_scratch_bytes(c3),), dtype=torch.uint8, device=dev)
-            pointnet2.bn_relu_max_pool_bwd(z3, grad_out.contiguous().float(), arg, g3c, b3c, mi3, gz3, dg3, db3, scratch, B * M, ns, c3)
-
-            def layer(gz, w, z_in, mi_in, gi, bi, k_in, n_out):
+            if zmax is not None:
+                pointnet2.bn_relu_max_pool_bwd_zmax(z3, grad_out.contiguous().float(), arg, zmax, g3c, b3c, mi3, gz3, dg3, db3, scratch,
+                                                    B * M, ns, c3)
+            else:
+                pointnet2.bn_relu_max_pool_bwd(z3, grad_out.contiguous().float(), arg, g3c, b3c, mi3, gz3, dg3, db3, scratch, B * M, ns, c3)
+
+            def layer(gz, w, z_in, mi_in, gi, bi, k_in, n_out, bn_bwd=True):
                 dw = torch.empty((n_out, k_in), dtype=torch.float32, device=dev)
                 ga = torch.empty((T, k_in), dtype=torch.float32, device=dev)
                 if WIDE_CHAIN_DGRAD_FIRST:
@@ -1250,19 +1264,24 @@
                     pointnet2.linear_wgrad_bn(z_in, gz, dw, T, k_in, n_out, mi_in, gi, bi)
                     _lin_cols(gz, w, ga, T, n_out, k_in, True)
                 dg, db = torch.empty_like(gi), torch.empty_like(bi)
-                scratch = torch.empty((pointnet2.bn_relu_scratch_bytes(k_in),), dtype=torch.uint8, device=dev)
-                pointnet2.bn_relu_bwd(z_in, ga, gi, bi, mi_in, ga, dg, db, scratch, T, k_in)
+                if bn_bwd:
+                    scratch = torch.empty((pointnet2.bn_relu_scratch_bytes(k_in),), dtype=torch.uint8, device=dev)
+                    pointnet2.bn_relu_bwd(z_in, ga, gi, bi, mi_in, ga, dg, db, scratch, T, k_in)
                 return dw, ga, dg, db
+            fused_tail = zmax is not None
             dw3, gz2, dg2, db2 = layer(gz3, w3, z2, mi2, g2c, b2c, c2, c3)
             del gz3
-            dw2, gz1, dg1, db1 = layer(gz2, w2, z1, mi1, g1c, b1c, c1, c2)
+            dw2, gz1, dg1, db1 = layer(gz2, w2, z1, mi1, g1c, b1c, c1, c2, bn_bwd=not fused_tail)
             del gz2
             w1c = w1.contiguous()
             dw1 = torch.empty_like(w1c)
             g_new = torch.empty_like(new_xyz) if ctx.needs_input_grad[1] else None
-            pointnet2.sa_xyz_grad(gz1, xyz, new_xyz, idx, w1c, dw1, g_new, B, N, M, ns, c1)
             g_pts = torch.zeros((B, N, c1), dtype=torch.float32, device=dev)
-            pointnet2.group_rows_grad(B, N, c1, M * ns, gz1, idx, g_pts)
+            if fused_tail:
+                pointnet2.sa_wide_tail_bwd(z1, gz1, g1c, b1c, mi1, dg1, db1, xyz, new_xyz, idx, w1c, dw1, g_new, g_pts, B, N, M, ns, c1)
+            else:
+                pointnet2.sa_xyz_grad(gz1, xyz, new_xyz, idx, w1c, dw1, g_new, B, N, M, ns, c1)
+                pointnet2.group_rows_grad(B, N, c1, M * ns, gz1, idx, g_pts)
             g_pts = g_pts.view(B * N, c1)
             dw1[:, 3:] = _wgrad(feats_pm.view(B * N, C), g_pts, torch.empty((c1, C), dtype=torch.float32, device=dev), False)[0]
             g_feats = _gemm_nn(g_pts, w1c[:, 3:].contiguous()).view(B, N, C) if ctx.needs_input_grad[2] else None
```

After: 113.9 scenes/s. -6.0%, worse.
